# marvinquiet/SpaDOT

Hardware: AMD Instinct MI355X
Metric: training steps/sec + Sinkhorn iters/sec, 50k spots x 3k genes x 5 timepoints (higher is better)
Workload: dtype bf16; 1 GPU; cfg3: 5 time points x 10000 spots x 3000 genes, batch 512, k=30, 1200 inducing points; parallelism=1 GPU, n_sub=9980, E_sub=308893, m_inducing=236, params=16136032, hip_graphs=True, staged_graphs=True, bucketed_grad_exchange=False, units_in_schedule=80

## Files before the change

### include/spadot_model.h

```cpp
#ifndef SPADOT_MODEL_H
#define SPADOT_MODEL_H

#ifdef __cplusplus
extern "C" {
#endif

enum { SPADOT_DT_F32 = 0, SPADOT_DT_BF16 = 1, SPADOT_DT_F64 = 2 };
enum { SPADOT_KERNEL_GAUSSIAN = 0, SPADOT_KERNEL_CAUCHY = 1, SPADOT_KERNEL_QUADRATIC = 2 };

const char *spadot_model_version(void);

int spadot_gat_forward(const void *h, int dtype, const float *s_src, const float *s_dst,
                       const int *rowptr, const int *col, const float *bias, int n, int H, int C,
                       int concat, int act, void *out, float *alpha_out, void *stream);

int spadot_gat_backward_target(const void *g_out, const void *out, const void *h, int dtype,
                               const float *s_src, const float *s_dst, const float *alpha,
                               const int *rowptr, const int *col, int n, int H, int C, int concat,
                               int act, void *g_pre, float *dz, float *ds_dst, void *stream);

int spadot_gat_backward_source(const void *g_pre, int dtype, const float *alpha, const float *dz,
                               const int *rowptr_t, const int *col_t, const int *eid_t, int n, int H,
                               int C, void *dh, float *ds_src, const float *ds_dst, const float *att_src,
                               const float *att_dst, void *stream);
// ... 27 lines not shown
                         void *g_mu, void *g_var, void *g_mv, void *g_tr, void *g_pm, void *g_pv,
                         void *stream);

int spadot_bn_act_forward(const void *x, int x_dtype, const float *lin_bias, const float *gamma, const float *beta,
                          float *running_mean, float *running_var, long long *num_batches_tracked, int b, int F,
                          double momentum, double eps, double slope, float *y, float *save_mean, float *save_invstd,
                          void *stream);
int spadot_bn_act_backward(const float *dy, const float *y, const void *x, int x_dtype, const float *lin_bias,
                           const float *gamma, const float *save_mean, const float *save_invstd, int b, int F,
                           double slope, void *dx, float *dgamma, float *dbeta, void *stream);
int spadot_ln_act_forward(const float *x, const float *gamma, const float *beta, int b, int F, double eps, double slope,
                          float *y, float *save_mean, float *save_invstd, void *stream);
int spadot_ln_act_backward(const float *dy, const float *y, const float *x, const float *gamma, const float *save_mean,
                           const float *save_invstd, int b, int F, double slope, float *dx, float *dgamma, float *dbeta,
                           void *stream);

int spadot_svgp_post_forward(const double *raw, const double *rd, const double *r, const double *Mr, const double *ld,
                             const double *sm, const double *mu, const double *var, const double *ktilde, int b, int L,
                             int m, double c, double kl_const, double b_over_N, double *p_m, double *mv, double *p_v,
                             double *tr, double *out4, float *skl32 , void *stream);
int spadot_svgp_post_backward(const float *g_skl, const double *out4, const double *G_pm, const double *G_pv,
                              const double *mu, const double *var, const double *mv, const double *tr, const double *p_m,
                              const double *p_v, const double *ktilde, const double *Mr, const double *M, int b, int L,
                              int m, double c, double b_over_N, double *g_mu, double *g_var, double *G1, double *G2T,
                              double *g_kl, double *gMr, double *gM, void *stream);
int spadot_svgp_q1t(const double *Ta, const double *Tb, const double *G2T, const double *m0, const double *g_kl, int L, int nh,
                    int b, double *q1, void *stream);
int spadot_svgp_post_pm_pv(const double *raw, const double *rd_a, const double *ktilde, int b, int L, double c, double *p_m,
                           double *p_v, void *stream);
int spadot_svgp_grad_tail(const double *q1, const double *q2, const double *Kdt, const double *p_v, const double *ktilde,
                          const double *p_m, const double *mu, const double *w, const double *g_kl, const double *g_mu,
                          const double *g_var, int b, int L, double c, double *dmu, double *dvar, float *dz,
                          void *stream);
int spadot_svgp_pre(const float *z, int b, int L, double *mu, double *var, double *w, double *muw, void *stream);
int spadot_svgp_pre2(const float *z, const double *Kn, int b, int L, int m, double *mu, double *var, double *w, double *muw,
                     double *A, void *stream);
int spadot_svgp_mid(const double *S, const double *t, const double *M, const double *X2, int L, int m, int rows2,
                    double *r, double *Mr, double *raw, double *sm, double *smpart, int smpart_doubles, void *stream);

int spadot_latent_head_forward(const float *zg, const double *p_m, const double *p_v, float *eps, int b, int Ls,
                               int Lg, float *latent, float *scal2, double *partials, unsigned *counter,
                               unsigned long long *rng_state, void *stream);
int spadot_latent_head_backward(const float *zg, const double *p_v, const float *eps, const float *latent,
                                const float *g_latent, const float *g_kl, const float *g_align, int b, int Ls, int Lg,
                                float *d_zg, double *d_pm, double *d_pv, void *stream);
int spadot_cluster_losses_forward(const float *z, const long long *labels_all, const long long *seed_ids,
                                  const float *centres, const float *prev_centres, const float *gamma,
                                  const long long *cluster_list, int b, int D, int K, int Kp, int Kl, int do_km,
                                  int do_ot, float *out2, float *work, void *stream);
int spadot_cluster_losses_backward(const float *z, const float *centres, const float *prev_centres, const float *gamma,
                                   const long long *cluster_list, const float *work, const float *g_km,
                                   const float *g_ot, int b, int D, int K, int Kp, int Kl, int do_km, int do_ot,
                                   float *dz, void *stream);
int spadot_cluster_losses_fb(const float *z, const long long *labels_all, const long long *seed_ids, const float *centres,
                             const float *prev_centres, const float *gamma, const long long *cluster_list, int b, int D, int K,
                             int Kp, int Kl, int do_km, int do_ot, const float *g_km, const float *g_ot, float *out2,
                             float *work, float *dz, void *stream);
int spadot_mix_losses_forward(const float *const *terms6, const float *w6, float *out7, void *stream);
int spadot_mix_losses_backward(const float *g_elbo, const float *w6, float *g6, void *stream);

int spadot_sqerr_forward(const void *y, const void *yhat, long long count, double inv_scale, int dtype,
                         double *scratch, void *out1, void *stream);
int spadot_sqerr_backward(const void *g1, const void *y, const void *yhat, long long count,
                          double inv_scale, int dtype, void *g_yhat, void *stream);

int spadot_kmeans_assign(const void *x, const void *centers, int n, int k, int d, int dtype, int *labels,
                         void *stream);

int spadot_sgemm_small(int mode, const float *A, int lda, const float *B, int ldb, float *C, int ldc, int M, int N, int K,
                       const float *bias, int batch, long long strideA, long long strideB, long long strideC, void *stream);

int spadot_enc_fused_supported(int b, int F1, int F2, int Q);
long long spadot_enc_fused_workspace(int b, int F1, int F2, int Q);
int spadot_enc_bn_map(const float *h1, const float *lin_bias, const float *gamma, const float *beta, float *running_mean,
                      float *running_var, long long *num_batches_tracked, int b, int F1, double momentum, double eps, double slope,
                      float *y1, float *save_mean, float *save_invstd, const float *W2, int F2, float *part, void *stream);
int spadot_enc_bn_fc(const float *part, int nparts, const float *lin_bias, const float *gamma, const float *beta, float *running_mean,
                     float *running_var, long long *num_batches_tracked, int b, int F2, double momentum, double eps, double slope,
                     float *h2, float *y2, float *save_mean, float *save_invstd, const float *Wfc, int Q, float *pz, void *stream);
int spadot_enc_sum_z(const float *pz, int nparts, const float *bias, int b, int Q, float *z, void *stream);
int spadot_svgp_pre2_partials(const float *pz, int nparts, const float *bias, const double *Kn, int b, int L, int m, float *z,
                              double *mu, double *var, double *w, double *muw, double *A, void *stream);

int spadot_recon_fb_supported(int b, int K, int G);
long long spadot_recon_fb_workspace(int b, int K, int G);
int spadot_recon_fb(const void *h_bf16, const void *W_bf16, const void *WT_bf16, int ldt, const float *bias, const float *y, int b, int K,
                    int G, double inv_scale, const float *grad_weight, void *g_bf16, float *workspace, double *loss_parts, float *dh,
                    void *stream);
int spadot_sum_parts(const double *part, int n, double scale, float *out, void *stream);

int spadot_stamp(unsigned long long *buf, int slot, void *stream);

int spadot_lloyd_step(const double *X, double *C, const int *xoff, const int *npts, int n_max, int R, const int *rgroup,
                      const int *Kr, int K_max, int D, const double *tol, double *part, int *done, double *inertia, int skip_done,
                      void *stream);
int spadot_kmeanspp_seed(const double *X, const int *xoff, const int *npts, int D, int P, const int *pset, const int *pK,
                         const int *pfirst, const int *puoff, const double *U, int K_max, int n_max, double *closest, int *idx,
                         double *centers, void *stream);

int spadot_knn(const double *x, int n, int d, int kk, int *out, void *stream);

int spadot_gat_mfma_supported(int dtype, int H, int C, int max_cols);

int spadot_gat_tail_supported(int dtype, int H, int K);
int spadot_gat_tail_wvec(const float *W, int ldw, const float *att_src, const float *att_dst, int H, int C, int K, float *part,
                         int slices, float *wv, void *whi, void *wlo, void *stream);
int spadot_gat_tail_logits(const void *x, int dtype, int ldx, const float *wv, const void *whi, const void *wlo, int n, int H, int K,
                           float *s, void *stream);
int spadot_gat_tail_aggregate(const void *x, int dtype, int ldx, const float *s, const int *rowptr, const int *col, int n_tgt, int H,
                              int K, void *A, float *alpha, void *stream);
int spadot_gat_tail_headmean(const void *O, int dtype, const float *bias, int n_tgt, int H, int C, void *out, void *stream);
int spadot_gat_tail_colsum_rows(const void *g, int dtype, int rows, int C, float *out, void *stream);
int spadot_gat_tail_scale_colsum(const void *g, int dtype, int rows, int C, double scale, void *gs, float *out, void *stream);
int spadot_gat_tail_edge_backward(const void *x, int dtype, int ldx, const void *dA, const float *s, const float *alpha, const int *rowptr,
                                  const int *col, int n_tgt, int H, int K, float *dz, float *ds_dst, void *stream);
int spadot_gat_tail_source_backward(const void *dA, int dtype, const float *alpha, const float *dz, const float *ds_dst, const float *wv,
                                    const int *rowptr_t, const int *col_t, const int *eid_t, int n, int n_tgt, int rows_out, int H, int K,
                                    void *dx, int lddx, float *ds_src, const void *act_out, int ldm, double slope, void *stream);
int spadot_gat_tail_dwvec_rows(int n);
int spadot_gat_tail_dwvec(const void *x, int dtype, int ldx, const float *ds_src, const float *ds_dst, int n, int n_tgt, int H, int K,
                          float *part, void *stream);
int spadot_gat_tail_wvec_backward(const float *W, int ldw, const float *att_src, const float *att_dst, const float *dwv, int H, int C, int K,
                                  float *dW, int lddw, int accumulate, float *datt_src, float *datt_dst, void *stream);
int spadot_gat_alpha(const float *s_src, const float *s_dst, const int *rowptr, const int *col, const int *cellq, int n_tgt,
                     int H, float *alpha, void *acell, const int *cellq_s, void *acell_s, void *stream);
int spadot_gat_aggregate(const void *x, int dtype, const void *acell, const int *plan_rows, const int *plan_sptr,
                         const int *plan_cols, int nb, int max_cols, int H, int C, int mode, const float *vec_a,
                         const float *vec_b, int act, const float *ds_src, const float *ds_dst, void *out,
                         const void *h_rows, float *att_part, int part_width, int pad_from, int pad_to, const float *dz,
                         const int *rowptr_t, const int *eid_t, float *ds_src_out, void *stream);
int spadot_gat_edge_dot(const void *g_out, const void *out, const void *h, int dtype, const int *plan_rows,
                        const int *plan_sptr, const int *plan_cols, const int *plan_cell, int nb, int max_cols, int H,
                        int C, int act, void *g_pre, float *dz, float *bias_part, int part_width, int part_col, void *stream);
int spadot_gat_softmax_backward(const float *alpha, const float *s_src, const float *s_dst, const int *rowptr,
                                const int *col, const int *cellq_s, int n_tgt, int n_all, int H, float *dz, float *ds_dst,
                                void *acell_s, void *stream);
int spadot_gat_ds_src(const float *dz, const int *rowptr_t, const int *eid_t, int n, int H, float *ds_src, void *stream);

int spadot_gemm_tn_bf16(const void *A, int lda, const void *B, int ldb, void *C, int ldc, int M, int N, int K, void *stream);
int spadot_gemm_nn_bf16(const void *A, int lda, const void *B, int ldb, void *C, int ldc, int M, int N, int K, void *stream);
int spadot_gemm_nn_bf16_masked(const void *A, int lda, const void *B, int ldb, void *C, int ldc, int M, int N, int K,
                               const void *act_out, int ldm, double slope, void *stream);
long long spadot_gemm_bf16_split_workspace(int M, int N, int tail_row_tiles, int slices);
int spadot_gemm_tn_bf16_split(const void *A, int lda, const void *B, int ldb, void *C, int ldc, int M, int N, int K,
                              int tail_row_tiles, int slices, float *workspace, void *stream);


long long spadot_gemm_wgrad_bf16_workspace(int M, int N, int K, int slices);
int spadot_gemm_wgrad_bf16(const void *G, int ldg, const void *X, int ldx, float *dW, int ldw, int M, int N, int K,
                           int slices, float *workspace, const void *zero_row, void *stream);
long long spadot_gemm_wgrad_bf16_workspace_tiled(int M, int N, int K, int slices, int tile_k);
int spadot_gemm_wgrad_bf16_tiled(const void *G, int ldg, const void *X, int ldx, float *dW, int ldw, int M, int N, int K,
                                 int slices, int tile_k, float *workspace, const void *zero_row, void *stream);

int spadot_mlp_chain_supported(int n_layers, const int *dims);
int spadot_mlp_chain_workspace(int b, int n_layers, const int *dims, int *n_rows, int *width);
int spadot_mlp_chain_forward(const float *x, int b, int n_layers, const int *dims, const float *const *W,
                             const float *const *bias, const float *const *gamma, const float *const *beta, const double *eps,
                             const double *slope, float *const *a, float *const *y, float *const *mean, float *const *invstd,
                             void *stream);
int spadot_mlp_chain_forward_bf16(const float *x, int b, int n_layers, const int *dims, const float *const *W,
                                  const float *const *bias, const float *const *gamma, const float *const *beta,
                                  const double *eps, const double *slope, float *const *a, float *const *y, float *const *mean,
                                  float *const *invstd, void *y_last_bf16, void *stream);
int spadot_mlp_chain_backward(const float *dy, const float *x, int b, int n_layers, const int *dims, const float *const *W,
                              const float *const *gamma, const double *slope, float *const *a, float *const *y,
                              float *const *mean, float *const *invstd, float *dx, float *workspace, float *grads, void *stream);
int spadot_mlp_chain_backward_add(const float *dy, const float *x, int b, int n_layers, const int *dims, const float *const *W,
                                  const float *const *gamma, const double *slope, float *const *a, float *const *y,
                                  float *const *mean, float *const *invstd, float *dx, const float *dx_add, float *workspace,
                                  float *grads, void *stream);

int spadot_bias_sqerr_forward(const float *o, const float *bias, const float *y, int b, int G, double inv_scale, double *scratch,
                              float *out, void *stream);
int spadot_bias_sqerr_backward(const float *g1, const float *o, const float *bias, const float *y, int b, int G,
                               double inv_scale, void *g_bf16, float *dbias, void *stream);

int spadot_headfc_backward(const float *g, const void *h_bf16, const float *W, int b, int K, int N, void *dh_bf16,
                           float *workspace , float *grads ,
                           void *stream);

int spadot_cast_rows_multi(const float *const *src, void *const *dst, const int *rows, const int *K, const int *Kp, int n,
                           void *stream);

int spadot_grad_sumsq(const float *grad, long long count, double *scratch, float *sumsq, void *stream);
int spadot_clip_adamw_dev(float *param, const float *grad, float *exp_avg, float *exp_avg_sq, long long count, double lr,
                          double beta1, double beta2, double eps, double weight_decay, double max_norm, double *scratch,
                          float *sumsq, int *step_dev, unsigned *counter, const float *grad_scale_dev, void *stream);
typedef struct spadot_weight_image {
    long long offset;
    int rows, K, Kp, reserved;
    void *image;
} spadot_weight_image;
typedef struct spadot_weight_images {
    int n, reserved;
    spadot_weight_image w[8];
} spadot_weight_images;
int spadot_clip_adamw_images_dev(float *param, const float *grad, float *exp_avg, float *exp_avg_sq, long long count, double lr,
                                 double beta1, double beta2, double eps, double weight_decay, double max_norm, double *scratch,
                                 float *sumsq, int *step_dev, const float *grad_scale_dev, const spadot_weight_images *images,
                                 void *stream);
int spadot_grad_norm_step_dev(const float *grad, long long count, double *scratch, float *sumsq, int *step_dev, void *stream);
int spadot_adamw_range_dev(float *param, const float *grad, float *exp_avg, float *exp_avg_sq, long long offset, long long count,
                           double lr, double beta1, double beta2, double eps, double weight_decay, double max_norm,
                           const float *sumsq, const int *step_dev, const float *grad_scale_dev, const spadot_weight_images *images,
                           void *stream);

int spadot_adamw_step(float *param, const float *grad, float *exp_avg, float *exp_avg_sq,
                      const float *sumsq, long long count, double lr, double beta1, double beta2,
                      double eps, double weight_decay, double max_norm, int step, void *stream);

int spadot_adamw_step_dev(float *param, const float *grad, float *exp_avg, float *exp_avg_sq,
                          const float *sumsq, long long count, double lr, double beta1, double beta2,
                          double eps, double weight_decay, double max_norm, int *step_dev, void *stream);

int spadot_pre_gene_detect(const long long *colptr, const int *ridx, const float *val, const int *tp_off, int T, int G,
                           double thr, int *cnt, double *colsum, void *stream);
int spadot_pre_row_total(const long long *indptr, const int *cidx, const float *val, const int *tp_off, int T, int G,
                         const unsigned char *mask, int nrows, double *total, void *stream);
int spadot_sparkx_moments(const long long *colptr, const int *ridx, const float *val, const int *tp_off, int P,
                          const int *pair_t, const int *pair_g, const int *rowmap, const double *xt, double *mom, void *stream);
int spadot_sparkx_pvals(const double *mom, int P, const int *pair_t, const int *nkeep, const double *inv, const double *lam,
                        int nodes, double *stat, double *pval, double *comb, void *stream);
int spadot_pre_lognorm_stats(const long long *colptr, const int *ridx, const float *val, const int *tp_off, int T, int S,
                             const int *cols, const double *total, double target, double *mean, double *stdv, void *stream);
int spadot_pre_scale_write(const long long *indptr, const int *cidx, const float *val, const int *tp_off, int T, int S,
                           const int *colpos, const double *total, double target, const double *mean, const double *stdv,
                           double clip, int nrows, float *out, void *stream);

int spadot_sct_gene_stats(const long long *colptr, const int *ridx, const float *val, const int *tp_off, int t, int Gk,
                          const int *genes, int N, double *out, void *stream);
int spadot_sct_fit(const long long *colptr, const int *ridx, const float *val, const int *tp_off, int t, int G1,
                   const int *genes, const double *lur, const double *lu, int N, double tol, int maxit, int limit, double eps,
                   double *out, void *stream);
int spadot_sct_resid_stats(const long long *colptr, const int *ridx, const float *val, const int *tp_off, int t, int Gk,
                           const int *genes, const double *lur, const double *lu, int N, const double *pars, double clip_hi,
                           double clip_lo, double *out, void *stream);
int spadot_sct_resid_write(const long long *colptr, const int *ridx, const float *val, const int *tp_off, int t, int S,
                           const int *genes, const double *lur, const double *lu, const int *krow, const int *rowmap, int N,
                           const double *pars, const double *center, double clip_lo, double *out, void *stream);
int spadot_sct_polygamma(const double *x, int n, double *psi, double *psi1, void *stream);

int spadot_mk_lds_capacity(void);
long long spadot_mk_ranksum_scratch_bytes(int T, int G, int nmax);
int spadot_mk_lognorm(const int *ridx, const float *val, const double *total, long long nnz, double target, float *v,
                      void *stream);
int spadot_mk_ranksum(const long long *colptr, const int *ridx, const float *v, const int *tp_off, const int *labels,
                      const int *nk, int T, int G, int K, int nmax, void *scratch, long long scratch_bytes, long long *r2,
                      long long *ties, int *nnz_k, double *vsum, void *stream);
int spadot_mk_finish(const long long *r2, const long long *ties, const int *tp_off, const int *nk, int T, int G, int K,
                     double *u1, double *score, double *pval, void *stream);

int spadot_silhouette(const double *x, int d, int P, const long long *prob, const int *order, const int *coff, int n_max,
                      int k_min, int k_max, double *a, double *b, int *nearest, double *s, void *stream);

int spadot_gmm_em_step(const double *x, int d, int P, const long long *prob, int K_max, int n_max, double *par, double *w,
                       double *cov, double *mom, const double *resp_init, double reg_covar, double tol, int steps, double *part,
                       int *done, int *n_iter, double *lb, void *stream);
int spadot_gmm_estep(const double *x, int d, int P, const long long *prob, int K_max, int n_max, const double *par, double *norm,
                     int *labels, double *resp, double *lp, void *stream);

int spadot_nhood_counts(const int *src, const int *dst, const unsigned char *labels, const long long *desc_host,
                        const long long *desc_dev, int G, int K_max, long long lds_limit, int *out, void *stream);

int spadot_cooccur_counts(const double *xy, const long long *desc_host, const long long *desc_dev, const double *r2_host,
                          const double *r2_dev, int P, int K_max, int B_max, long long *out, void *stream);

int spadot_cooccur_null(const double *xy, const long long *desc_host, const long long *desc_dev, const double *r2_host,
                        const double *r2_dev, int P, int K_max, int B_max, int observed, long long first, int n_perms,
                        long long seed, long long *out, void *stream);

int spadot_ripley_counts(const double *xy, const long long *desc_host, const long long *desc_dev, const double *r2_host,
                         const double *r2_dev, const double *hull_host, const double *hull_dev, const double *cum_host,
                         const double *cum_dev, long long hull_rows, int P, int K_max, int S_max, int B_max, long long seed,
                         long long *out, void *stream);

int spadot_ripley_points(const double *hull_host, const double *hull_dev, const double *cum_host, const double *cum_dev, int V,
                         long long seed, long long g, long long stream_id, long long count, double *out, void *stream);

int spadot_autocorr_sums(const int *src, const int *dst, const long long *colptr, const int *ridx, const float *v, long long nnz,
                         long long ridx_lo, long long ridx_hi, const double *centre, const long long *desc_host,
                         const long long *desc_dev, int T, int G, int g0, int ng, int observed, long long first, long long P,
                         long long seed, long long lds_limit, float *scratch, long long scratch_floats, int threads, int gs,
                         double *N, double *D, void *stream);

int spadot_ligrec_sums(const long long *colptr, const int *ridx, const float *v, long long nnz, long long ridx_lo,
                       long long ridx_hi, const unsigned char *labels, int label_hi, const long long *desc_host,
                       const long long *desc_dev, int T, int G, int K, const int *genes, int ng, int gene_lo, int gene_hi,
                       int observed, long long first, long long P, long long seed, long long lds_limit, int threads, int gc,
                       double *S, int *cnt, void *stream);

int spadot_ligrec_count(const double *S0, const double *S, const double *wk, const int *pairs, int pair_lo, int pair_hi,
                        const unsigned char *mask, int T, int M, int ns, int K, long long L, int skip, int *ge, void *stream);

int spadot_local_lag(const int *rowptr, const int *col, const long long *colptr, const int *ridx, const float *v, long long nnz,
                     long long ridx_lo, long long ridx_hi, const double *centre, const long long *desc_host,
                     const long long *desc_dev, int T, int G, const int *genes, int ng, int gene_lo, int gene_hi, long long first,
                     long long P, long long seed, long long lds_limit, void *scratch, long long scratch_bytes, int threads, int gs,
                     long long perm_chunk, long long rows, double *lag, int *ge, int *le, void *stream);

int spadot_cross_dense(const int *rowptr, const int *col, const long long *colptr, const int *ridx, const float *v, long long nnz,
                       long long ridx_lo, long long ridx_hi, const double *centre, const long long *desc_host,
                       const long long *desc_dev, int T, int G, const int *genes, int ng, int gene_lo, int gene_hi, int GP,
                       long long zrows, double *Z, double *Y, void *stream);
int spadot_cross_sums(const double *Z, const double *Y, long long zrows, int GP, const long long *desc_host,
                      const long long *desc_dev, int T, int ng, int observed, long long first, long long P, long long seed,
                      double *M, void *stream);

int spadot_corr_sums(const double *xy, const int *order, const double *Z, long long zrows, int GP, const long long *desc_host,
                     const long long *desc_dev, const double *r2_host, const double *r2_dev, int T, int ng, int B_max, int observed,
                     long long first, long long P, long long seed, int cull, int cs, double *scratch, long long scratch_doubles,
                     long long *W, long long *S2c, double *N, double *Q, long long *skipped, void *stream);

int spadot_latent_knn(const double *x, int d, int P, const long long *prob_host, const long long *prob_dev, int *idx, double *d2,
                      void *stream);
int spadot_tsne_affinities(const double *d2, int P, const long long *prob_host, const long long *prob_dev, const double *perp_host,
                           const double *perp_dev, double *cond, double *beta, void *stream);
int spadot_tsne_steps(const long long *prob_host, const long long *prob_dev, int P, const long long *rowptr, const int *col,
                      const double *val, double *Y0, double *Y1, double *upd, double *gains, const double *lr, double *part,
                      double *zr, double *att, double *blk, double *grad, double *Z, double *kl, long long kl_stride, long long it0,
                      int steps, long long early, double exaggeration, int two, void *stream);

int spadot_weighted_moments_chunk(void);
int spadot_weighted_moments(const long long *colptr, const int *ridx, const float *v, const int *tp_off, int T, int G,
                            const double *W, long long n, int C, double *S0, double *S1, double *S2, void *stream);

#ifdef __cplusplus
}
#endif
#endif
```

### spadot_amd/_lib.py

```python
import ctypes
import os

_CSRC = os.path.join(os.path.dirname(os.path.abspath(__file__)), "csrc")
_CACHE = {}


class NativeLibraryMissing(RuntimeError):
    pass


def _load(name):
    if name in _CACHE:
        return _CACHE[name]
    import torch

    path = os.path.join(_CSRC, name)
    if not os.path.exists(path):
        raise NativeLibraryMissing(
            f"{path} is missing: build the HIP extension with `python -m spadot_amd.csrc.build` "
            "(needs hipcc; cross-compiles for gfx950 without a GPU). There is no CPU fallback.")
    lib = ctypes.CDLL(path)
    _CACHE[name] = lib
    return lib


class _Checked:
    __slots__ = ("fn", "n", "name")

    def __init__(self, fn, name):
        self.fn, self.n, self.name = fn, len(fn.argtypes), name

    @property
    def argtypes(self):
        return self.fn.argtypes

    @property
    def restype(self):
        return self.fn.restype

    def __call__(self, *args):
        if len(args) != self.n:
            raise TypeError(f"{self.name} takes {self.n} arguments (include/*.h), {len(args)} given")
        return self.fn(*args)


def _seal(lib):
    for name, fn in list(vars(lib).items()):
        if name.startswith("spadot_") and not isinstance(fn, _Checked):
            if fn.argtypes is None and name not in ("spadot_ot_version", "spadot_model_version"):
                raise RuntimeError(f"{name}: no argtypes declared in spadot_amd/_lib.py")
            if fn.argtypes is not None:
                setattr(lib, name, _Checked(fn, name))


class OTConfig(ctypes.Structure):
    _fields_ = [("lambda1", ctypes.c_double), ("lambda2", ctypes.c_double), ("epsilon", ctypes.c_double),
                ("epsilon0", ctypes.c_double), ("tolerance", ctypes.c_double), ("tau", ctypes.c_double),
                ("batch_size", ctypes.c_int), ("max_iter", ctypes.c_int)]


class OTInfo(ctypes.Structure):
    _fields_ = [("gap", ctypes.c_double), ("stage_iters", ctypes.c_int * 6), ("absorbs", ctypes.c_int),
                ("gap_checks", ctypes.c_int)]


class OTSmallProblem(ctypes.Structure):
    _fields_ = [("x_dev", ctypes.c_void_p), ("y_dev", ctypes.c_void_p), ("C_dev", ctypes.c_void_p),
                ("G_dev", ctypes.c_void_p), ("plan_dev", ctypes.c_void_p), ("gamma_rownorm_dev", ctypes.c_void_p),
                ("I", ctypes.c_int), ("J", ctypes.c_int)]


class OTSmallInfo(ctypes.Structure):
    _fields_ = [("gap", ctypes.c_double), ("stage_iters", ctypes.c_int * 6), ("absorbs", ctypes.c_int),
                ("gap_checks", ctypes.c_int), ("status", ctypes.c_int), ("reserved", ctypes.c_int)]


class WeightImage(ctypes.Structure):
    _fields_ = [("offset", ctypes.c_longlong), ("rows", ctypes.c_int), ("K", ctypes.c_int), ("Kp", ctypes.c_int),
                ("reserved", ctypes.c_int), ("image", ctypes.c_void_p)]


class WeightImages(ctypes.Structure):
    _fields_ = [("n", ctypes.c_int), ("reserved", ctypes.c_int), ("w", WeightImage * 8)]


def ot_lib():
    lib = _load("libspadot_ot.so")
    if getattr(lib, "_spadot_ready", False):
        return lib
    vp, ci, cd = ctypes.c_void_p, ctypes.c_int, ctypes.c_double
    lib.spadot_ot_version.restype = ctypes.c_char_p
    lib.spadot_ot_create.argtypes = [ctypes.POINTER(vp), ci, ci, ci, vp]
    lib.spadot_ot_create.restype = ci
    lib.spadot_ot_destroy.argtypes = [vp]
    lib.spadot_ot_destroy.restype = None
    lib.spadot_ot_ld.argtypes = [vp]
    lib.spadot_ot_ld.restype = ci
    lib.spadot_ot_fused_geometry.argtypes = [vp, ctypes.POINTER(ci)]
    lib.spadot_ot_fused_geometry.restype = None
    lib.spadot_ot_matrix_dev.argtypes = [vp, ci]
    lib.spadot_ot_matrix_dev.restype = vp
    lib.spadot_ot_vector_dev.argtypes = [vp, ci]
    lib.spadot_ot_vector_dev.restype = vp
    lib.spadot_ot_vector_host.argtypes = [vp, ci, vp]
    lib.spadot_ot_vector_host.restype = ci
    lib.spadot_ot_matrix_host.argtypes = [vp, ci, vp]
    lib.spadot_ot_matrix_host.restype = ci
    lib.spadot_ot_set_cost_dev.argtypes = [vp, vp, ci, ci]
    lib.spadot_ot_set_cost_dev.restype = ci
    lib.spadot_ot_set_cost_host.argtypes = [vp, vp]
    lib.spadot_ot_set_cost_host.restype = ci
    lib.spadot_ot_set_cost_from_latents_dev.argtypes = [vp, vp, vp, ci, ci]
    lib.spadot_ot_set_cost_from_latents_dev.restype = ci
    lib.spadot_ot_solve.argtypes = [vp, vp, ctypes.POINTER(OTConfig), ctypes.POINTER(OTInfo)]
    lib.spadot_ot_solve.restype = ci
    lib.spadot_ot_plan_dev.argtypes = [vp, vp, ci, ci]
    lib.spadot_ot_plan_dev.restype = ci
    lib.spadot_ot_plan_group_sums_dev.argtypes = [vp, vp, ci, vp]
    lib.spadot_ot_plan_group_sums_dev.restype = ci
    lib.spadot_ot_plan_apply_dev.argtypes = [vp, ci, vp, ci, vp]
    lib.spadot_ot_plan_apply_dev.restype = ci
    lib.spadot_ot_plan_host.argtypes = [vp, vp]
    lib.spadot_ot_plan_host.restype = ci
    lib.spadot_ot_plan_rowsums_host.argtypes = [vp, vp]
    lib.spadot_ot_plan_rowsums_host.restype = ci
    lib.spadot_ot_run_iterations.argtypes = [vp, ctypes.POINTER(OTConfig), cd, ci, ctypes.POINTER(ctypes.c_float)]
    lib.spadot_ot_run_iterations.restype = ci
    lib.spadot_ot_run_tau_flag.argtypes = [vp, ci]
    lib.spadot_ot_run_tau_flag.restype = ci
    lib.spadot_ot_run_checked.argtypes = [vp, ctypes.POINTER(OTConfig), cd, ci, ci, ctypes.POINTER(ci), ctypes.POINTER(ctypes.c_float)]
    lib.spadot_ot_run_checked.restype = ci
    lib.spadot_ot_time_kernels.argtypes = [vp, ctypes.POINTER(OTConfig), cd, ci, ctypes.POINTER(ctypes.c_float)]
    lib.spadot_ot_time_kernels.restype = ci
    lib.spadot_ot_small_max.argtypes = []
    lib.spadot_ot_small_max.restype = ci
    lib.spadot_ot_small_solve.argtypes = [ci, ctypes.POINTER(OTSmallProblem), ci, ci, ctypes.POINTER(OTConfig), vp, vp]
    lib.spadot_ot_small_solve.restype = ci
    _seal(lib)
    lib._spadot_ready = True
    return lib


def model_lib():
    lib = _load("libspadot_model.so")
    if getattr(lib, "_spadot_ready", False):
        return lib
    vp, ci, cd, ll = ctypes.c_void_p, ctypes.c_int, ctypes.c_double, ctypes.c_longlong
    lib.spadot_model_version.restype = ctypes.c_char_p
    sig = {
        "spadot_gat_forward": [vp, ci, vp, vp, vp, vp, vp, ci, ci, ci, ci, ci, vp, vp, vp],
        "spadot_gat_backward_target": [vp, vp, vp, ci, vp, vp, vp, vp, vp, ci, ci, ci, ci, ci, vp, vp, vp, vp],
        "spadot_gat_backward_source": [vp, ci, vp, vp, vp, vp, vp, ci, ci, ci, vp, vp, vp, vp, vp, vp],
        "spadot_gat_logits": [vp, ci, vp, vp, ci, ci, ci, vp, vp, vp],
        "spadot_gat_att_grad": [vp, ci, vp, vp, ci, ci, ci, vp, ci, vp, vp, vp, ci, vp],
        "spadot_gat_alpha": [vp, vp, vp, vp, vp, ci, ci, vp, vp, vp, vp, vp],
        "spadot_gat_softmax_backward": [vp, vp, vp, vp, vp, vp, ci, ci, ci, vp, vp, vp, vp],
        "spadot_gat_ds_src": [vp, vp, vp, ci, ci, vp, vp],
        "spadot_gat_mfma_supported": [ci, ci, ci, ci],
        "spadot_gat_tail_supported": [ci, ci, ci],
        "spadot_gat_tail_wvec": [vp, ci, vp, vp, ci, ci, ci, vp, ci, vp, vp, vp, vp],
        "spadot_gat_tail_logits": [vp, ci, ci, vp, vp, vp, ci, ci, ci, vp, vp],
        "spadot_gat_tail_aggregate": [vp, ci, ci, vp, vp, vp, ci, ci, ci, vp, vp, vp],
        "spadot_gat_tail_headmean": [vp, ci, vp, ci, ci, ci, vp, vp],
        "spadot_gat_tail_colsum_rows": [vp, ci, ci, ci, vp, vp],
        "spadot_gat_tail_scale_colsum": [vp, ci, ci, ci, cd, vp, vp, vp],
        "spadot_gat_tail_edge_backward": [vp, ci, ci, vp, vp, vp, vp, vp, ci, ci, ci, vp, vp, vp],
        "spadot_gat_tail_source_backward": [vp, ci, vp, vp, vp, vp, vp, vp, vp, ci, ci, ci, ci, ci, vp, ci, vp, vp, ci, cd, vp],
        "spadot_gat_tail_dwvec_rows": [ci],
        "spadot_gat_tail_dwvec": [vp, ci, ci, vp, vp, ci, ci, ci, ci, vp, vp],
        "spadot_gat_tail_wvec_backward": [vp, ci, vp, vp, vp, ci, ci, ci, vp, ci, ci, vp, vp, vp],
        "spadot_gat_aggregate": [vp, ci, vp, vp, vp, vp, ci, ci, ci, ci, ci, vp, vp, ci, vp, vp, vp, vp, vp, ci, ci, ci, vp, vp, vp, vp, vp],
        "spadot_gat_edge_dot": [vp, vp, vp, ci, vp, vp, vp, vp, ci, ci, ci, ci, ci, vp, vp, vp, ci, ci, vp],
        "spadot_gemm_tn_bf16": [vp, ci, vp, ci, vp, ci, ci, ci, ci, vp],
        "spadot_gemm_nn_bf16": [vp, ci, vp, ci, vp, ci, ci, ci, ci, vp],
        "spadot_enc_fused_supported": [ci, ci, ci, ci],
        "spadot_recon_fb_supported": [ci, ci, ci],
        "spadot_recon_fb": [vp, vp, vp, ci, vp, vp, ci, ci, ci, cd, vp, vp, vp, vp, vp, vp],
        "spadot_sum_parts": [vp, ci, cd, vp, vp],
        "spadot_enc_bn_map": [vp, vp, vp, vp, vp, vp, vp, ci, ci, cd, cd, cd, vp, vp, vp, vp, ci, vp, vp],
        "spadot_enc_bn_fc": [vp, ci, vp, vp, vp, vp, vp, vp, ci, ci, cd, cd, cd, vp, vp, vp, vp, vp, ci, vp, vp],
        "spadot_enc_sum_z": [vp, ci, vp, ci, ci, vp, vp],
        "spadot_svgp_pre2_partials": [vp, ci, vp, vp, ci, ci, ci, vp, vp, vp, vp, vp, vp, vp],
        "spadot_gemm_nn_bf16_masked": [vp, ci, vp, ci, vp, ci, ci, ci, ci, vp, ci, cd, vp],
        "spadot_gemm_tn_bf16_split": [vp, ci, vp, ci, vp, ci, ci, ci, ci, ci, ci, vp, vp],
        "spadot_gemm_wgrad_bf16": [vp, ci, vp, ci, vp, ci, ci, ci, ci, ci, vp, vp, vp],
        "spadot_gemm_wgrad_bf16_tiled": [vp, ci, vp, ci, vp, ci, ci, ci, ci, ci, ci, vp, vp, vp],
        "spadot_mlp_chain_supported": [ci, vp],
        "spadot_headfc_backward": [vp, vp, vp, ci, ci, ci, vp, vp, vp, vp],
        "spadot_bias_sqerr_forward": [vp, vp, vp, ci, ci, cd, vp, vp, vp],
        "spadot_bias_sqerr_backward": [vp, vp, vp, vp, ci, ci, cd, vp, vp, vp],
        "spadot_mlp_chain_workspace": [ci, ci, vp, vp, vp],
        "spadot_mlp_chain_forward": [vp, ci, ci, vp, vp, vp, vp, vp, vp, vp, vp, vp, vp, vp, vp],
        "spadot_mlp_chain_forward_bf16": [vp, ci, ci, vp, vp, vp, vp, vp, vp, vp, vp, vp, vp, vp, vp, vp],
        "spadot_mlp_chain_backward": [vp, vp, ci, ci, vp, vp, vp, vp, vp, vp, vp, vp, vp, vp, vp, vp],
        "spadot_mlp_chain_backward_add": [vp, vp, ci, ci, vp, vp, vp, vp, vp, vp, vp, vp, vp, vp, vp, vp, vp],
        "spadot_kernel_matrix": [vp, vp, ci, ci, ci, cd, ci, ci, vp, vp],
        "spadot_spd_inverse_logdet": [vp, ci, ci, vp, vp, vp],
        "spadot_rowdot_forward": [vp, vp, ci, ci, ci, ci, vp, vp],
        "spadot_rowdot_backward": [vp, vp, ci, ci, ci, ci, vp, vp],
        "spadot_elbo_forward": [vp, vp, vp, vp, vp, vp, vp, ci, ci, ci, vp, vp],
        "spadot_elbo_backward": [vp, vp, vp, vp, vp, vp, vp, vp, ci, ci, ci, vp, vp, vp, vp, vp, vp, vp],
        "spadot_bn_act_forward": [vp, ci, vp, vp, vp, vp, vp, vp, ci, ci, cd, cd, cd, vp, vp, vp, vp],
        "spadot_bn_act_backward": [vp, vp, vp, ci, vp, vp, vp, vp, ci, ci, cd, vp, vp, vp, vp],
        "spadot_ln_act_forward": [vp, vp, vp, ci, ci, cd, cd, vp, vp, vp, vp],
        "spadot_ln_act_backward": [vp, vp, vp, vp, vp, vp, ci, ci, cd, vp, vp, vp, vp],
        "spadot_svgp_post_forward": [vp] * 9 + [ci, ci, ci, cd, cd, cd] + [vp] * 7,
        "spadot_svgp_post_backward": [vp] * 13 + [ci, ci, ci, cd, cd] + [vp] * 8,
        "spadot_svgp_grad_tail": [vp] * 11 + [ci, ci, cd] + [vp] * 4,
        "spadot_svgp_q1t": [vp, vp, vp, vp, vp, ci, ci, ci, vp, vp],
        "spadot_svgp_post_pm_pv": [vp, vp, vp, ci, ci, cd, vp, vp, vp],
        "spadot_svgp_pre": [vp, ci, ci, vp, vp, vp, vp, vp],
        "spadot_svgp_pre2": [vp, vp, ci, ci, ci, vp, vp, vp, vp, vp, vp],
        "spadot_svgp_mid": [vp, vp, vp, vp, ci, ci, ci, vp, vp, vp, vp, vp, ci, vp],
        "spadot_spd_inverse_logdet2": [vp, ci, ci, ci, vp, vp, vp, vp, vp],
        "spadot_latent_head_forward": [vp, vp, vp, vp, ci, ci, ci, vp, vp, vp, vp, vp, vp],
        "spadot_latent_head_backward": [vp, vp, vp, vp, vp, vp, vp, ci, ci, ci, vp, vp, vp, vp],
        "spadot_cluster_losses_forward": [vp, vp, vp, vp, vp, vp, vp, ci, ci, ci, ci, ci, ci, ci, vp, vp, vp],
        "spadot_cluster_losses_backward": [vp, vp, vp, vp, vp, vp, vp, vp, ci, ci, ci, ci, ci, ci, ci, vp, vp],
        "spadot_cluster_losses_fb": [vp, vp, vp, vp, vp, vp, vp, ci, ci, ci, ci, ci, ci, ci, vp, vp, vp, vp, vp, vp],
        "spadot_mix_losses_forward": [vp, vp, vp, vp],
        "spadot_mix_losses_backward": [vp, vp, vp, vp],
        "spadot_sqerr_forward": [vp, vp, ll, cd, ci, vp, vp, vp],
        "spadot_sqerr_backward": [vp, vp, vp, ll, cd, ci, vp, vp],
        "spadot_kmeans_assign": [vp, vp, ci, ci, ci, ci, vp, vp],
        "spadot_sgemm_small": [ci, vp, ci, vp, ci, vp, ci, ci, ci, ci, vp, ci, ll, ll, ll, vp],
        "spadot_lloyd_step": [vp, vp, vp, vp, ci, ci, vp, vp, ci, ci, vp, vp, vp, vp, ci, vp],
        "spadot_kmeanspp_seed": [vp, vp, vp, ci, ci, vp, vp, vp, vp, vp, ci, ci, vp, vp, vp, vp],
        "spadot_colsum": [vp, ci, ci, vp, vp],
        "spadot_cast_rows_multi": [vp, vp, vp, vp, vp, ci, vp],
        "spadot_knn": [vp, ci, ci, ci, vp, vp],
        "spadot_stamp": [vp, ci, vp],
        "spadot_grad_sumsq": [vp, ll, vp, vp, vp],
        "spadot_clip_adamw_dev": [vp, vp, vp, vp, ll, cd, cd, cd, cd, cd, cd, vp, vp, vp, vp, vp, vp],
        "spadot_clip_adamw_images_dev": [vp, vp, vp, vp, ll, cd, cd, cd, cd, cd, cd, vp, vp, vp, vp, ctypes.POINTER(WeightImages), vp],
        "spadot_grad_norm_step_dev": [vp, ll, vp, vp, vp, vp],
        "spadot_adamw_range_dev": [vp, vp, vp, vp, ll, ll, cd, cd, cd, cd, cd, cd, vp, vp, vp, ctypes.POINTER(WeightImages), vp],
        "spadot_adamw_step": [vp, vp, vp, vp, vp, ll, cd, cd, cd, cd, cd, cd, ci, vp],
        "spadot_adamw_step_dev": [vp, vp, vp, vp, vp, ll, cd, cd, cd, cd, cd, cd, vp, vp],
        "spadot_pre_gene_detect": [vp, vp, vp, vp, ci, ci, cd, vp, vp, vp],
        "spadot_pre_row_total": [vp, vp, vp, vp, ci, ci, vp, ci, vp, vp],
        "spadot_sparkx_moments": [vp, vp, vp, vp, ci, vp, vp, vp, vp, vp, vp],
        "spadot_sparkx_pvals": [vp, ci, vp, vp, vp, vp, ci, vp, vp, vp, vp],
        "spadot_pre_lognorm_stats": [vp, vp, vp, vp, ci, ci, vp, vp, cd, vp, vp, vp],
        "spadot_pre_scale_write": [vp, vp, vp, vp, ci, ci, vp, vp, cd, vp, vp, cd, ci, vp, vp],
        "spadot_sct_gene_stats": [vp, vp, vp, vp, ci, ci, vp, ci, vp, vp],
        "spadot_sct_fit": [vp, vp, vp, vp, ci, ci, vp, vp, vp, ci, cd, ci, ci, cd, vp, vp],
        "spadot_sct_resid_stats": [vp, vp, vp, vp, ci, ci, vp, vp, vp, ci, vp, cd, cd, vp, vp],
        "spadot_sct_resid_write": [vp, vp, vp, vp, ci, ci, vp, vp, vp, vp, vp, ci, vp, vp, cd, vp, vp],
        "spadot_sct_polygamma": [vp, ci, vp, vp, vp],
        "spadot_mk_lognorm": [vp, vp, vp, ll, cd, vp, vp],
        "spadot_mk_ranksum": [vp, vp, vp, vp, vp, vp, ci, ci, ci, ci, vp, ll, vp, vp, vp, vp, vp],
        "spadot_mk_finish": [vp, vp, vp, vp, ci, ci, ci, vp, vp, vp, vp],
        "spadot_silhouette": [vp, ci, ci, vp, vp, vp, ci, ci, ci, vp, vp, vp, vp, vp],
        "spadot_weighted_moments": [vp, vp, vp, vp, ci, ci, vp, ll, ci, vp, vp, vp, vp],
        "spadot_gmm_em_step": [vp, ci, ci, vp, ci, ci, vp, vp, vp, vp, vp, cd, cd, ci, vp, vp, vp, vp, vp],
        "spadot_gmm_estep": [vp, ci, ci, vp, ci, ci, vp, vp, vp, vp, vp, vp],
        "spadot_nhood_counts": [vp, vp, vp, vp, vp, ci, ci, ll, vp, vp],
        "spadot_cooccur_counts": [vp, vp, vp, vp, vp, ci, ci, ci, vp, vp],
        "spadot_cooccur_null": [vp, vp, vp, vp, vp, ci, ci, ci, ci, ll, ci, ll, vp, vp],
        "spadot_ripley_counts": [vp, vp, vp, vp, vp, vp, vp, vp, vp, ll, ci, ci, ci, ci, ll, vp, vp],
        "spadot_ripley_points": [vp, vp, vp, vp, ci, ll, ll, ll, ll, vp, vp],
        "spadot_autocorr_sums": [vp, vp, vp, vp, vp, ll, ll, ll, vp, vp, vp, ci, ci, ci, ci, ci, ll, ll, ll, ll, vp, ll, ci, ci,
                                 vp, vp, vp],
        "spadot_ligrec_sums": [vp, vp, vp, ll, ll, ll, vp, ci, vp, vp, ci, ci, ci, vp, ci, ci, ci, ci, ll, ll, ll, ll, ci, ci, vp, vp,
                               vp],
        "spadot_ligrec_count": [vp, vp, vp, vp, ci, ci, vp, ci, ci, ci, ci, ll, ci, vp, vp],
        "spadot_local_lag": [vp, vp, vp, vp, vp, ll, ll, ll, vp, vp, vp, ci, ci, vp, ci, ci, ci, ll, ll, ll, ll, vp, ll, ci, ci, ll,
                             ll, vp, vp, vp, vp],
        "spadot_cross_dense": [vp, vp, vp, vp, vp, ll, ll, ll, vp, vp, vp, ci, ci, vp, ci, ci, ci, ci, ll, vp, vp, vp],
        "spadot_cross_sums": [vp, vp, ll, ci, vp, vp, ci, ci, ci, ll, ll, ll, vp, vp],
        "spadot_corr_sums": [vp, vp, vp, ll, ci, vp, vp, vp, vp, ci, ci, ci, ci, ll, ll, ll, ci, ci, vp, ll, vp, vp, vp, vp, vp, vp],
        "spadot_latent_knn": [vp, ci, ci, vp, vp, vp, vp, vp],
        "spadot_tsne_affinities": [vp, ci, vp, vp, vp, vp, vp, vp, vp],
        "spadot_tsne_steps": [vp, vp, ci, vp, vp, vp, vp, vp, vp, vp, vp, vp, vp, vp, vp, vp, vp, vp, ll, ll, ci, ll, cd, ci, vp],
    }
    for name, args in sig.items():
        fn = getattr(lib, name)
        fn.argtypes = args
        fn.restype = ci
    lib.spadot_recon_fb_workspace.argtypes = [ci, ci, ci]
    lib.spadot_recon_fb_workspace.restype = ll
    lib.spadot_enc_fused_workspace.argtypes = [ci, ci, ci, ci]
    lib.spadot_enc_fused_workspace.restype = ll
    lib.spadot_gemm_bf16_split_workspace.argtypes = [ci, ci, ci, ci]
    lib.spadot_gemm_bf16_split_workspace.restype = ll
    lib.spadot_gemm_wgrad_bf16_workspace.argtypes = [ci, ci, ci, ci]
    lib.spadot_gemm_wgrad_bf16_workspace.restype = ll
    lib.spadot_gemm_wgrad_bf16_workspace_tiled.argtypes = [ci, ci, ci, ci, ci]
    lib.spadot_gemm_wgrad_bf16_workspace_tiled.restype = ll
    lib.spadot_mk_lds_capacity.argtypes = []
    lib.spadot_mk_lds_capacity.restype = ci
    lib.spadot_mk_ranksum_scratch_bytes.argtypes = [ci, ci, ci]
    lib.spadot_mk_ranksum_scratch_bytes.restype = ll
    lib.spadot_weighted_moments_chunk.argtypes = []
    lib.spadot_weighted_moments_chunk.restype = ci
    _seal(lib)
    lib._spadot_ready = True
    return lib
```

### spadot_amd/csrc/gemm_wgrad_bf16.hip

```cpp
#include <hip/hip_runtime.h>
#include <cstdint>

#include "../../include/spadot_model.h"
#include "per_device.h"

namespace {

typedef __bf16 bf8 __attribute__((ext_vector_type(8)));
typedef short s4v __attribute__((ext_vector_type(4)));
typedef float f16v __attribute__((ext_vector_type(16)));

constexpr int TN = 256, TK = 256, CH = 64, NT = 512;
constexpr int ROWB = 512;
constexpr int OPB = CH * ROWB;
constexpr int STAGEB = 2 * OPB;
constexpr int LDS_BYTES = 2 * STAGEB;
constexpr int PIECES = 8;

template <int WGN, int WGK, int TI, int TJ>
__global__ __launch_bounds__(NT, 1) void k_gemm_wgrad_bf16(const __bf16 *__restrict__ G, int ldg, const __bf16 *__restrict__ X,
                                                          int ldx, float *__restrict__ dW, int ldw, int M, int N, int K,
                                                          int ktiles, int S, int chunks_per_slice,
                                                          const __bf16 *__restrict__ zrow, float *__restrict__ part) {
    extern __shared__ __attribute__((aligned(16))) unsigned char smem[];
// ... 23 lines not shown
        poff[u] = u < 4 ? ((size_t)row * ldg + n0) * 2 + chunk * 16 : ((size_t)row * ldx + k0) * 2 + chunk * 16;
        if (u >= 4 && chunk * 8 >= TKE) pzero = true;
    }
    auto request = [&](int ks) __attribute__((always_inline)) {
#ifdef WGRAD_PROBE_NO_DMA
        return;
#endif
        const int m0 = (c_begin + ks) * CH;
        const unsigned base = lds0 + (unsigned)(ks & 1) * STAGEB + (unsigned)wave * 1024u;
#pragma unroll
        for (int u = 0; u < PIECES; u++) {
            const char *src = (u < 4 ? reinterpret_cast<const char *>(G) + (size_t)m0 * ldg * 2
                                     : reinterpret_cast<const char *>(X) + (size_t)m0 * ldx * 2) + poff[u];
            if (m0 + prow[u] >= M || (u >= 4 && pzero)) src = reinterpret_cast<const char *>(zrow) + (lane & 31) * 16;
            const unsigned dst = __builtin_amdgcn_readfirstlane(base + (unsigned)(u & 3) * 8192u + (u < 4 ? 0u : (unsigned)OPB));
            unsigned keep;
            asm volatile("s_mov_b32 %0, m0\n\ts_mov_b32 m0, %2\n\ts_nop 0\n\tglobal_load_lds_dwordx4 %1, off\n\ts_mov_b32 m0, %0"
                         : "=&s"(keep) : "v"(src), "s"(dst) : "memory");
        }
    };

    f16v acc[TI][TJ];
#pragma unroll
    for (int i = 0; i < TI; i++)
#pragma unroll
        for (int j = 0; j < TJ; j++)
#pragma unroll
            for (int e = 0; e < 16; e++) acc[i][j][e] = 0.f;

    const int hh = lane >> 5, g16 = (lane >> 4) & 1, qq = (lane & 15) >> 2, pp = lane & 3;
    unsigned ga[TI], xb[TJ];
#pragma unroll
    for (int i = 0; i < TI; i++) {
        const int g = wn * TI + i;
        ga[i] = lds0 + (unsigned)((8 * hh + qq) * ROWB + (g & ~3) * 64 + ((g ^ qq) & 3) * 64 + 32 * g16 + 8 * pp);
    }
#pragma unroll
    for (int j = 0; j < TJ; j++) {
        const int g = wk * TJ + j;
        xb[j] = lds0 + (unsigned)OPB + (unsigned)((8 * hh + qq) * ROWB + (g & ~3) * 64 + ((g ^ qq) & 3) * 64 + 32 * g16 + 8 * pp);
    }
    auto read_frags = [&](unsigned stage_off, int ss, s4v (&a)[TI][2], s4v (&b)[TJ][2]) __attribute__((always_inline)) {
        const unsigned so = stage_off + (unsigned)ss * (16 * ROWB);
#ifdef WGRAD_PROBE_NO_READS
#pragma unroll
        for (int j = 0; j < TJ; j++) b[j][0] = b[j][1] = s4v{(short)so, 1, 2, 3};
#pragma unroll
        for (int i = 0; i < TI; i++) a[i][0] = a[i][1] = s4v{(short)so, 1, 2, 3};
        return;
#endif
#pragma unroll
        for (int j = 0; j < TJ; j++) {
            asm volatile("ds_read_b64_tr_b16 %0, %1" : "=v"(b[j][0]) : "v"(xb[j] + so));
            asm volatile("ds_read_b64_tr_b16 %0, %1 offset:2048" : "=v"(b[j][1]) : "v"(xb[j] + so));
        }
#pragma unroll
        for (int i = 0; i < TI; i++) {
            asm volatile("ds_read_b64_tr_b16 %0, %1" : "=v"(a[i][0]) : "v"(ga[i] + so));
            asm volatile("ds_read_b64_tr_b16 %0, %1 offset:2048" : "=v"(a[i][1]) : "v"(ga[i] + so));
        }
    };
    auto mma = [&](const s4v (&a)[TI][2], const s4v (&b)[TJ][2]) __attribute__((always_inline)) {
        __builtin_amdgcn_s_setprio(1);
        bf8 bf[TJ];
#pragma unroll
        for (int j = 0; j < TJ; j++) bf[j] = __builtin_bit_cast(bf8, __builtin_shufflevector(b[j][0], b[j][1], 0, 1, 2, 3, 4, 5, 6, 7));
#pragma unroll
        for (int i = 0; i < TI; i++) {
            const bf8 af = __builtin_bit_cast(bf8, __builtin_shufflevector(a[i][0], a[i][1], 0, 1, 2, 3, 4, 5, 6, 7));
#pragma unroll
            for (int j = 0; j < TJ; j++) {
#ifdef WGRAD_PROBE_NO_MFMA
                asm volatile("" ::"v"(af), "v"(bf[j]));
#else
                acc[i][j] = __builtin_amdgcn_mfma_f32_32x32x16_bf16(af, bf[j], acc[i][j], 0, 0, 0);
#endif
            }
        }
        __builtin_amdgcn_s_setprio(0);
    };
    auto frags_ready = [&]() __attribute__((always_inline)) {
#ifdef WGRAD_PROBE_NO_READS
        return;
#endif
        asm volatile("s_waitcnt lgkmcnt(%0)" ::"n"(RD) : "memory");
        __builtin_amdgcn_sched_barrier(0);
    };

    if (nk > 0) {
        request(0);
        if (1 < nk) {
            request(1);
            asm volatile("s_waitcnt vmcnt(%0)" ::"n"(PIECES) : "memory");
        } else {
            asm volatile("s_waitcnt vmcnt(0)" ::: "memory");
        }
        __builtin_amdgcn_s_barrier();
        s4v a0[TI][2], b0[TJ][2], a1[TI][2], b1[TJ][2];
        read_frags(0u, 0, a0, b0);
        for (int P = 0; P < nk; P++) {
            const unsigned so = (unsigned)(P & 1) * STAGEB;
            read_frags(so, 1, a1, b1);
            frags_ready();
            mma(a0, b0);
            read_frags(so, 2, a0, b0);
            frags_ready();
            mma(a1, b1);
            read_frags(so, 3, a1, b1);
            frags_ready();
            mma(a0, b0);
            if (P + 1 < nk) {
                asm volatile("s_waitcnt vmcnt(0)" ::: "memory");
                asm volatile("s_waitcnt lgkmcnt(0)" ::: "memory");
                __builtin_amdgcn_sched_barrier(0);
                __builtin_amdgcn_s_barrier();
                if (P + 2 < nk) request(P + 2);
                read_frags((unsigned)((P + 1) & 1) * STAGEB, 0, a0, b0);
                asm volatile("s_waitcnt lgkmcnt(%0)" ::"n"(RD) : "memory");
            } else {
                asm volatile("s_waitcnt lgkmcnt(0)" ::: "memory");
            }
            __builtin_amdgcn_sched_barrier(0);
            mma(a1, b1);
        }
    }

    const int lk = (wk * TJ) * 32 + (lane & 31);
    if (S == 1) {
#pragma unroll
        for (int i = 0; i < TI; i++)
#pragma unroll
            for (int j = 0; j < TJ; j++)
#pragma unroll
                for (int e = 0; e < 16; e++) {
                    const int n = n0 + (wn * TI + i) * 32 + (e & 3) + 8 * (e >> 2) + 4 * hh, k = k0 + lk + 32 * j;
                    if (n < N && k < K) dW[(size_t)n * ldw + k] = acc[i][j][e];
                }
        return;
    }
    float *mine = part + ((size_t)slice * gridDim.x / S + tile) * (size_t)(TN * TKE);
#pragma unroll
    for (int i = 0; i < TI; i++)
#pragma unroll
        for (int j = 0; j < TJ; j++)
#pragma unroll
            for (int e = 0; e < 16; e++) {
                const int ln = (wn * TI + i) * 32 + (e & 3) + 8 * (e >> 2) + 4 * hh;
                mine[(size_t)ln * TKE + lk + 32 * j] = acc[i][j][e];
            }
}

template <int TKE>
__global__ __launch_bounds__(256) void k_wgrad_reduce(const float *__restrict__ part, int S, int tiles, int ktiles,
                                                      float *__restrict__ dW, int ldw, int N, int K) {
    constexpr int RP = TKE / 4;
    constexpr int BPT = RP / 4;
    constexpr int Q = 64 * RP;
    typedef float f32x4 __attribute__((ext_vector_type(4)));
    const int tile = blockIdx.x / BPT;
    const int p0 = (blockIdx.x - tile * BPT) * 256 + threadIdx.x;
    const int tn = tile / ktiles, tk = tile - tn * ktiles;
    f32x4 v[8][4];
#pragma unroll
    for (int s_ = 0; s_ < 8; s_++)
        if (s_ < S) {
            const f32x4 *src = reinterpret_cast<const f32x4 *>(part + ((size_t)s_ * tiles + tile) * (size_t)(TN * TKE));
#pragma unroll
            for (int j = 0; j < 4; j++) v[s_][j] = src[p0 + j * Q];
        }
#pragma unroll
    for (int j = 0; j < 4; j++) {
        f32x4 sum = v[0][j];
#pragma unroll
        for (int s_ = 1; s_ < 8; s_++)
            if (s_ < S) sum += v[s_][j];
        const int idx4 = p0 + j * Q, ln = idx4 / RP, c4 = idx4 - ln * RP;
        const int n = tn * TN + ln, k = tk * TKE + 4 * c4;
        if (n < N && k + 3 < K) *reinterpret_cast<f32x4 *>(dW + (size_t)n * ldw + k) = sum;
        else if (n < N) {
            for (int e = 0; e < 4; e++)
                if (k + e < K) dW[(size_t)n * ldw + k + e] = sum[e];
        }
    }
}

static int effective_slices(int M, int slices, int *cps_out) {
    const int nchunk = (M + CH - 1) / CH;
    int S = slices > 0 ? slices : 1;
    if (S > nchunk) S = nchunk;
    if (S > 8) S = 8;
    const int cps = (nchunk + S - 1) / S;
    S = (nchunk + cps - 1) / cps;
    if (cps_out) *cps_out = cps;
    return S;
}

}

extern "C" long long spadot_gemm_wgrad_bf16_workspace_tiled(int M, int N, int K, int slices, int tile_k) {
    if (M <= 0 || N <= 0 || K <= 0 || N % TN != 0 || (tile_k != 256 && tile_k != 192)) return -22;
    const int S = effective_slices(M, slices, nullptr);
    const long long tiles = (long long)(N / TN) * ((K + tile_k - 1) / tile_k);
    return S > 1 ? (long long)S * tiles * TN * tile_k : 0;
}

extern "C" long long spadot_gemm_wgrad_bf16_workspace(int M, int N, int K, int slices) {
    return spadot_gemm_wgrad_bf16_workspace_tiled(M, N, K, slices, 256);
}

template <int WGN, int WGK, int TI, int TJ>
static int launch_wgrad(const void *G, int ldg, const void *X, int ldx, float *dW, int ldw, int M, int N, int K, int ktiles, int ntiles,
                        int S, int cps, float *workspace, const void *zero_row, hipStream_t stream) {
    constexpr int TKE = 32 * WGK * TJ;
    static PerDeviceFlag attr_set;     
    auto kern = k_gemm_wgrad_bf16<WGN, WGK, TI, TJ>;
    if (!attr_set) {
        if (hipFuncSetAttribute((const void *)kern, hipFuncAttributeMaxDynamicSharedMemorySize, LDS_BYTES) != hipSuccess) return -5;
        attr_set = true;
    }
    const int tiles = ntiles * ktiles;
    hipLaunchKernelGGL(kern, dim3((unsigned)(tiles * S)), dim3(NT), LDS_BYTES, stream, (const __bf16 *)G, ldg, (const __bf16 *)X, ldx, dW,
                       ldw, M, N, K, ktiles, S, cps, (const __bf16 *)zero_row, workspace);
    if (S > 1)
        hipLaunchKernelGGL(k_wgrad_reduce<TKE>, dim3((unsigned)tiles * (unsigned)(TKE / 16)), dim3(256), 0, stream, (const float *)workspace, S,
                           tiles, ktiles, dW, ldw, N, K);
    return hipGetLastError() == hipSuccess ? 0 : -5;
}

extern "C" int spadot_gemm_wgrad_bf16_tiled(const void *G, int ldg, const void *X, int ldx, float *dW, int ldw, int M, int N, int K,
                                            int slices, int tile_k, float *workspace, const void *zero_row, void *stream) {
    if (M <= 0 || N <= 0 || K <= 0 || N % TN != 0 || ldg < N || ldx < K || ldw < K || ldg % 8 || ldx % 8) return -22;
    if (tile_k != 256 && tile_k != 192) return -22;
    if (((uintptr_t)G & 15) || ((uintptr_t)X & 15) || ((uintptr_t)dW & 15) || (ldw % 4)) return -22;
    if (!zero_row || ((uintptr_t)zero_row & 15)) return -22;
    const int ktiles = (K + tile_k - 1) / tile_k, ntiles = N / TN;
    if (ldx < ktiles * tile_k) return -22;
    if ((size_t)M * ldg * 2 >= ((size_t)1 << 32) || (size_t)M * ldx * 2 >= ((size_t)1 << 32)) return -22;
    int cps = 0;
    const int S = effective_slices(M, slices, &cps);
    if (ntiles * ktiles > 4096) return -22;
    if (S > 1 && (!workspace || ((uintptr_t)workspace & 15))) return -22;
    if (tile_k == 256)
        return launch_wgrad<2, 4, 4, 2>(G, ldg, X, ldx, dW, ldw, M, N, K, ktiles, ntiles, S, cps, workspace, zero_row, (hipStream_t)stream);
    return launch_wgrad<4, 2, 2, 3>(G, ldg, X, ldx, dW, ldw, M, N, K, ktiles, ntiles, S, cps, workspace, zero_row, (hipStream_t)stream);
}

extern "C" int spadot_gemm_wgrad_bf16(const void *G, int ldg, const void *X, int ldx, float *dW, int ldw, int M, int N, int K,
                                      int slices, float *workspace, const void *zero_row, void *stream) {
    return spadot_gemm_wgrad_bf16_tiled(G, ldg, X, ldx, dW, ldw, M, N, K, slices, 256, workspace, zero_row, stream);
}
```

### spadot_amd/csrc/model_kernels.hip

```cpp
#include <hip/hip_runtime.h>
#include <cmath>
#include <climits>
#include <cstdint>
#include <cstdio>
#include <cstdlib>

#include "../../include/spadot_model.h"
#include "per_device.h"

namespace {

constexpr int WAVE = 64;
constexpr float ATT_SLOPE = 0.2f;
constexpr float ACT_SLOPE = 0.01f;

template <typename T> __device__ __forceinline__ float ld(const T *p);
template <> __device__ __forceinline__ float ld<float>(const float *p) { return *p; }
template <> __device__ __forceinline__ float ld<__bf16>(const __bf16 *p) { return (float)*p; }
template <typename T> __device__ __forceinline__ void st(T *p, float v);
template <> __device__ __forceinline__ void st<float>(float *p, float v) { *p = v; }
template <> __device__ __forceinline__ void st<__bf16>(__bf16 *p, float v) { *p = (__bf16)v; }

__device__ __forceinline__ unsigned bf16_pack2(float lo, float hi) {
    const unsigned short a = __builtin_bit_cast(unsigned short, (__bf16)lo), b = __builtin_bit_cast(unsigned short, (__bf16)hi);
// ... 1174 lines not shown
    for (int c = 1; c < K; c++) {
        if (t < KPP_MAXTR) s_cand[t] = INT_MAX;
        double ssum = 0.0;
        for (int i = lo; i < hi; i++) ssum += cl[i];
        s_scan[t] = ssum;
        __syncthreads();
        for (int off = 1; off < KPP_T; off <<= 1) {
            const double v = t >= off ? s_scan[t - off] : 0.0;
            __syncthreads();
            s_scan[t] += v;
            __syncthreads();
        }
        double run = t > 0 ? s_scan[t - 1] : 0.0;
        double rv[KPP_MAXTR];
        int found[KPP_MAXTR];
#pragma unroll
        for (int j = 0; j < KPP_MAXTR; j++) {
            rv[j] = j < trials ? Up[(size_t)(c - 1) * trials + j] * pot : 0.0;
            found[j] = INT_MAX;
        }
        for (int i = lo; i < hi; i++) {
            run += cl[i];
#pragma unroll
            for (int j = 0; j < KPP_MAXTR; j++)
                if (j < trials && found[j] == INT_MAX && run >= rv[j]) found[j] = i;
        }
#pragma unroll
        for (int j = 0; j < KPP_MAXTR; j++)
            if (j < trials && found[j] != INT_MAX) atomicMin(&s_cand[j], found[j]);
        __syncthreads();
        for (int e = t; e < trials * D; e += KPP_T) {
            const int j = e / D;
            s_c[e] = Xg[(size_t)min(s_cand[j], n - 1) * D + (e - j * D)];
        }
        __syncthreads();
        if (t < trials) {
            double q = 0.0;
            for (int e = 0; e < D; e++) q += s_c[t * D + e] * s_c[t * D + e];
            s_csq[t] = q;
        }
        __syncthreads();
        double lp[KPP_MAXTR];
#pragma unroll
        for (int j = 0; j < KPP_MAXTR; j++) lp[j] = 0.0;
        for (int i = t; i < n; i += KPP_T) {
            const double ci = cl[i];
            const double *xr = Xg + (size_t)i * D;
#pragma unroll
            for (int j = 0; j < KPP_MAXTR; j++)
                if (j < trials) lp[j] += fmin(kpp_d2(xr, s_c + j * D, s_csq[j], D), ci);
        }
        int best = 0;
        double bpot = 0.0;
#pragma unroll
        for (int j = 0; j < KPP_MAXTR; j++) {
            if (j < trials) {
                const double pj = block_sum_d(lp[j], s_red);
                if (j == 0 || pj < bpot) { bpot = pj; best = j; }
            }
        }
        pot = bpot;
        const double *cb = s_c + best * D;
        const double csqb = s_csq[best];
        for (int i = t; i < n; i += KPP_T) cl[i] = fmin(cl[i], kpp_d2(Xg + (size_t)i * D, cb, csqb, D));
        for (int e = t; e < D; e += KPP_T) cp[(size_t)c * D + e] = cb[e];
        if (t == 0) ip[c] = min(s_cand[best], n - 1);
        __syncthreads();
    }
}

__global__ __launch_bounds__(256) void k_sumsq_part(const float *__restrict__ g, long long count,
                                                    double *__restrict__ part) {
    __shared__ double sh[16];
    double acc = 0.0;
    const long long n4 = count / 4;
    const float4 *g4 = reinterpret_cast<const float4 *>(g);
    for (long long k = (long long)blockIdx.x * 256 + threadIdx.x; k < n4; k += (long long)gridDim.x * 256) {
        const float4 v = g4[k];
        acc += (double)v.x * v.x + (double)v.y * v.y + (double)v.z * v.z + (double)v.w * v.w;
    }
    if (blockIdx.x == 0)
        for (long long k = n4 * 4 + threadIdx.x; k < count; k += 256) acc += (double)g[k] * g[k];
    acc = block_sum_d(acc, sh);
    if (threadIdx.x == 0) part[blockIdx.x] = acc;
}

template <int U>
__global__ __launch_bounds__(256) void k_sumsq_last(const float *__restrict__ g, long long count, double *__restrict__ part,
                                                    float *__restrict__ sumsq, int *__restrict__ step_dev,
                                                    unsigned *__restrict__ counter) {
    __shared__ double sh[16];
    __shared__ bool last;
    double acc = 0.0;
    const long long n4 = count / 4;
    const float4 *g4 = reinterpret_cast<const float4 *>(g);
    const long long stride = (long long)gridDim.x * 256;
    for (long long k = (long long)blockIdx.x * 256 + threadIdx.x; k < n4; k += U * stride) {
        float4 v[U];
#pragma unroll
        for (int u = 0; u < U; u++)
            v[u] = (k + u * stride < n4) ? g4[k + u * stride] : make_float4(0.f, 0.f, 0.f, 0.f);
#pragma unroll
        for (int u = 0; u < U; u++)
            acc += ((double)v[u].x * v[u].x + (double)v[u].y * v[u].y) + ((double)v[u].z * v[u].z + (double)v[u].w * v[u].w);
    }
    if (blockIdx.x == 0)
        for (long long k = n4 * 4 + threadIdx.x; k < count; k += 256) acc += (double)g[k] * g[k];
    acc = block_sum_d(acc, sh);
    if (threadIdx.x == 0) {
        part[blockIdx.x] = acc;
        __threadfence();
        last = atomicAdd(counter, 1u) == gridDim.x - 1;
    }
    __syncthreads();
    if (!last) return;
    __threadfence();
    double t = 0.0;
    {
        double q[8];
#pragma unroll
        for (int u = 0; u < 8; u++) {
            const int b = threadIdx.x + u * 256;
            q[u] = b < (int)gridDim.x ? __builtin_nontemporal_load(part + b) : 0.0;
        }
        t = ((q[0] + q[1]) + (q[2] + q[3])) + ((q[4] + q[5]) + (q[6] + q[7]));
    }
    t = block_sum_d(t, sh);
    if (threadIdx.x == 0) { sumsq[0] = (float)t; if (step_dev) step_dev[0] += 1; *counter = 0u; }
}

__global__ void k_step_inc(int *step) { step[0] += 1; }

template <int U>
__global__ __launch_bounds__(256) void k_sumsq_part_u(const float *__restrict__ g, long long count, double *__restrict__ part) {
    __shared__ double sh[16];
    double acc = 0.0;
    const long long n4 = count / 4;
    const float4 *g4 = reinterpret_cast<const float4 *>(g);
    const long long stride = (long long)gridDim.x * 256;
    for (long long k = (long long)blockIdx.x * 256 + threadIdx.x; k < n4; k += U * stride) {
        float4 v[U];
#pragma unroll
        for (int u = 0; u < U; u++)
            v[u] = (k + u * stride < n4) ? g4[k + u * stride] : make_float4(0.f, 0.f, 0.f, 0.f);
#pragma unroll
        for (int u = 0; u < U; u++)
            acc += ((double)v[u].x * v[u].x + (double)v[u].y * v[u].y) + ((double)v[u].z * v[u].z + (double)v[u].w * v[u].w);
    }
    if (blockIdx.x == 0)
        for (long long k = n4 * 4 + threadIdx.x; k < count; k += 256) acc += (double)g[k] * g[k];
    acc = block_sum_d(acc, sh);
    if (threadIdx.x == 0) part[blockIdx.x] = acc;
}
__global__ __launch_bounds__(1024) void k_final_sum_step(const double *__restrict__ part, int nparts, float *__restrict__ out,
                                                         int *__restrict__ step_dev) {
    __shared__ double sh[16];
    double acc = 0.0;
    for (int k = threadIdx.x; k < nparts; k += 1024) acc += part[k];
    acc = block_sum_d(acc, sh);
    if (threadIdx.x == 0) { out[0] = (float)acc; if (step_dev) step_dev[0] += 1; }
}

__device__ __forceinline__ void adamw_element(float g_, float &pp, float &mm, float &vv, float coef, float lr, float wd,
                                              float b1, float b2, float eps, float bc1, float bc2_sqrt) {
#pragma clang fp contract(off)
    const float gg = g_ * coef;
    float pn = pp * (1.f - lr * wd);
    const float mn = mm + (gg - mm) * (1.f - b1);
    const float vn = vv * b2 + gg * gg * (1.f - b2);
    const float denom = sqrtf(vn) / bc2_sqrt + eps;
    pn -= (lr / bc1) * (mn / denom);
    pp = pn; mm = mn; vv = vn;
}

__device__ __forceinline__ float adamw_clip_coef(float sumsq, float gs, float max_norm) {
#pragma clang fp contract(off)
    const float total = sqrtf(sumsq) * gs;
    return fminf(1.f, max_norm / (total + 1e-6f)) * gs;
}

__global__ __launch_bounds__(256) void k_adamw(float *__restrict__ p, const float *__restrict__ g,
                                               float *__restrict__ m, float *__restrict__ v,
                                               const float *__restrict__ sumsq, long long count, float lr,
                                               float b1, float b2, float eps, float wd, float max_norm,
                                               float bc1, float bc2_sqrt, const int *__restrict__ step_dev,
                                               const float *__restrict__ grad_scale) {
    if (step_dev) {
        const double t = (double)step_dev[0];
        bc1 = (float)(1.0 - pow((double)b1, t));
        bc2_sqrt = (float)sqrt(1.0 - pow((double)b2, t));
    }
    const float gs = grad_scale ? grad_scale[0] : 1.f;
    const float coef = adamw_clip_coef(sumsq[0], gs, max_norm);
    for (long long k = (long long)blockIdx.x * 256 + threadIdx.x; k < count; k += (long long)gridDim.x * 256) {
        float pp = p[k], mm = m[k], vv = v[k];
        adamw_element(g[k], pp, mm, vv, coef, lr, wd, b1, b2, eps, bc1, bc2_sqrt);
        p[k] = pp; m[k] = mm; v[k] = vv;
    }
}

__global__ __launch_bounds__(256) void k_adamw_img(float *__restrict__ p, const float *__restrict__ g,
                                                   float *__restrict__ m, float *__restrict__ v,
                                                   const float *__restrict__ sumsq, long long count, float lr,
                                                   float b1, float b2, float eps, float wd, float max_norm,
                                                   const int *__restrict__ step_dev, const float *__restrict__ grad_scale,
                                                   spadot_weight_images imgs, long long base) {
    const double t = (double)step_dev[0];
    const float bc1 = (float)(1.0 - pow((double)b1, t));
    const float bc2_sqrt = (float)sqrt(1.0 - pow((double)b2, t));
    const float gs = grad_scale ? grad_scale[0] : 1.f;
    const float coef = adamw_clip_coef(sumsq[0], gs, max_norm);
    const long long n4 = count >> 2;
    for (long long q = (long long)blockIdx.x * 256 + threadIdx.x; q < n4; q += (long long)gridDim.x * 256) {
        const long long k = q << 2;
        const float4 g4 = *reinterpret_cast<const float4 *>(g + k);
        const float4 p4 = *reinterpret_cast<const float4 *>(p + k);
        const float4 m4 = *reinterpret_cast<const float4 *>(m + k);
        const float4 v4 = *reinterpret_cast<const float4 *>(v + k);
        const float gi[4] = {g4.x, g4.y, g4.z, g4.w}, pi[4] = {p4.x, p4.y, p4.z, p4.w};
        const float mi[4] = {m4.x, m4.y, m4.z, m4.w}, vi[4] = {v4.x, v4.y, v4.z, v4.w};
        float po[4], mo[4], vo[4];
#pragma unroll
        for (int e = 0; e < 4; e++) {
            po[e] = pi[e]; mo[e] = mi[e]; vo[e] = vi[e];
            adamw_element(gi[e], po[e], mo[e], vo[e], coef, lr, wd, b1, b2, eps, bc1, bc2_sqrt);
        }
        *reinterpret_cast<float4 *>(p + k) = make_float4(po[0], po[1], po[2], po[3]);
        *reinterpret_cast<float4 *>(m + k) = make_float4(mo[0], mo[1], mo[2], mo[3]);
        *reinterpret_cast<float4 *>(v + k) = make_float4(vo[0], vo[1], vo[2], vo[3]);
#pragma unroll
        for (int s_ = 0; s_ < 8; s_++) {
            if (s_ >= imgs.n) break;
            const spadot_weight_image W = imgs.w[s_];
            const unsigned long long d = (unsigned long long)(k + base - W.offset);
            if (d < (unsigned long long)W.rows * (unsigned long long)W.K) {
                const unsigned row = (unsigned)d / (unsigned)W.K;
                const unsigned col = (unsigned)d - row * (unsigned)W.K;
                __bf16 *dst = reinterpret_cast<__bf16 *>(W.image) + (size_t)row * W.Kp + col;
                const unsigned lo = (unsigned)__builtin_bit_cast(unsigned short, (__bf16)po[0]) |
                                    ((unsigned)__builtin_bit_cast(unsigned short, (__bf16)po[1]) << 16);
                const unsigned hi = (unsigned)__builtin_bit_cast(unsigned short, (__bf16)po[2]) |
                                    ((unsigned)__builtin_bit_cast(unsigned short, (__bf16)po[3]) << 16);
                *reinterpret_cast<uint2 *>(dst) = make_uint2(lo, hi);
                break;
            }
        }
    }
}

#ifndef BN_RG_DEF
#define BN_RG_DEF 16
#endif
constexpr int BN_RPT = 512 / BN_RG_DEF;
#ifndef BN_COLS_DEF
#define BN_COLS_DEF 16
#endif
constexpr int BN_COLS = BN_COLS_DEF, BN_RG = BN_RG_DEF, BN_NT = BN_COLS * BN_RG;
constexpr int LN_RG = 64, LN_NT = BN_COLS * LN_RG;

template <int RG = BN_RG>
__device__ __forceinline__ float bn_col_sum(float v, float (*sh)[BN_COLS + 1], int cl, int rg) {
    __syncthreads();
    sh[rg][cl] = v;
    __syncthreads();
    float t = 0.f;
#pragma unroll 8
    for (int g = 0; g < RG; g++) t += sh[g][cl];
    return t;
}

template <typename TX>
__global__ __launch_bounds__(BN_NT) void k_bn_act_fwd(const TX *__restrict__ x, const float *__restrict__ lb,
                                                    const float *__restrict__ gamma, const float *__restrict__ beta,
                                                    float *__restrict__ run_mean, float *__restrict__ run_var,
                                                    long long *__restrict__ nbt, int b, int F, float momentum, float eps,
                                                    float slope, float *__restrict__ y, float *__restrict__ save_mean,
                                                    float *__restrict__ save_invstd) {
    __shared__ float sh[BN_RG][BN_COLS + 1];
    const int cl = threadIdx.x & (BN_COLS - 1), rg = threadIdx.x / BN_COLS;
    const int c = blockIdx.x * BN_COLS + cl;
    const bool on = c < F;
    const int c1 = min(c, F - 1);
    const float add_r = (lb ? lb : gamma)[c1];
    const float add = (on && lb) ? add_r : 0.f;
    if (b <= BN_RG * BN_RPT) {
        float v[BN_RPT];
        const int cc = min(c, F - 1);
#pragma unroll
        for (int r = 0; r < BN_RPT; r++) v[r] = ld<TX>(x + (size_t)min(rg + r * BN_RG, b - 1) * F + cc);
        const float gam_r = gamma[cc], bet_r = beta[cc], rm_r = run_mean[cc], rv_r = run_var[cc];
#pragma unroll
        for (int r = 0; r < BN_RPT; r++) v[r] = (on && rg + r * BN_RG < b) ? v[r] + add : 0.f;
        float s = 0.f;
#pragma unroll
        for (int r = 0; r < BN_RPT; r++)
            if (rg + r * BN_RG < b) s += v[r];
        const float mean = bn_col_sum(s, sh, cl, rg) / (float)b;
        float ss = 0.f;
#pragma unroll
        for (int r = 0; r < BN_RPT; r++)
            if (rg + r * BN_RG < b) { const float d = v[r] - mean; ss += d * d; }
        const float var = bn_col_sum(ss, sh, cl, rg) / (float)b;
        const float invstd = rsqrtf(var + eps);
        if (on) {
            const float g = gam_r * invstd, o = bet_r;
#pragma unroll
            for (int r = 0; r < BN_RPT; r++) {
                const int i = rg + r * BN_RG;
                if (i < b) {
                    const float u = (v[r] - mean) * g + o;
                    y[(size_t)i * F + c] = u > 0.f ? u : slope * u;
                }
            }
            if (rg == 0) {
                save_mean[c] = mean; save_invstd[c] = invstd;
                run_mean[c] = (1.f - momentum) * rm_r + momentum * mean;
                run_var[c] = (1.f - momentum) * rv_r + momentum * var * ((float)b / (float)(b > 1 ? b - 1 : 1));
            }
        }
        if (nbt && blockIdx.x == 0 && threadIdx.x == 0) nbt[0] += 1;
        return;
    }
    float s = 0.f;
    if (on)
#pragma unroll 4
        for (int i = rg; i < b; i += BN_RG) s += ld<TX>(x + (size_t)i * F + c) + add;
    const float mean = bn_col_sum(s, sh, cl, rg) / (float)b;
    float ss = 0.f;
    if (on)
#pragma unroll 4
        for (int i = rg; i < b; i += BN_RG) { const float d = ld<TX>(x + (size_t)i * F + c) + add - mean; ss += d * d; }
    const float var = bn_col_sum(ss, sh, cl, rg) / (float)b;
    const float invstd = rsqrtf(var + eps);
    if (on) {
        const float g = gamma[c] * invstd, o = beta[c];
#pragma unroll 4
        for (int i = rg; i < b; i += BN_RG) {
            const float v = (ld<TX>(x + (size_t)i * F + c) + add - mean) * g + o;
            y[(size_t)i * F + c] = v > 0.f ? v : slope * v;
        }
        if (rg == 0) {
            save_mean[c] = mean; save_invstd[c] = invstd;
            run_mean[c] = (1.f - momentum) * run_mean[c] + momentum * mean;
            run_var[c] = (1.f - momentum) * run_var[c] + momentum * var * ((float)b / (float)(b > 1 ? b - 1 : 1));
        }
    }
    if (nbt && blockIdx.x == 0 && threadIdx.x == 0) nbt[0] += 1;
}

template <typename TX>
__global__ __launch_bounds__(BN_NT) void k_bn_act_bwd(const float *__restrict__ dy, const float *__restrict__ y,
                                                    const TX *__restrict__ x, const float *__restrict__ lb,
                                                    const float *__restrict__ gamma, const float *__restrict__ save_mean,
                                                    const float *__restrict__ save_invstd, int b, int F, float slope,
                                                    TX *__restrict__ dx, float *__restrict__ dgamma,
                                                    float *__restrict__ dbeta) {
    __shared__ float sh[BN_RG][BN_COLS + 1];
    const int cl = threadIdx.x & (BN_COLS - 1), rg = threadIdx.x / BN_COLS;
    const int c = blockIdx.x * BN_COLS + cl;
    const bool on = c < F;
    const int c1 = min(c, F - 1);
    const float add_r = (lb ? lb : gamma)[c1], mean_r = save_mean[c1], invstd_r = save_invstd[c1], gamma_r = gamma[c1];
    const float add = (on && lb) ? add_r : 0.f;
    const float mean = on ? mean_r : 0.f, invstd = on ? invstd_r : 0.f;
    if (b <= BN_RG * BN_RPT) {
        float dzv[BN_RPT], xh[BN_RPT];
        const int cc = min(c, F - 1);
#pragma unroll
        for (int r = 0; r < BN_RPT; r++) dzv[r] = dy[(size_t)min(rg + r * BN_RG, b - 1) * F + cc];
#pragma unroll
        for (int r = 0; r < BN_RPT; r++) {
            const float yv = y[(size_t)min(rg + r * BN_RG, b - 1) * F + cc];
            dzv[r] = (on && rg + r * BN_RG < b) ? dzv[r] * (yv > 0.f ? 1.f : slope) : 0.f;
        }
#pragma unroll
        for (int r = 0; r < BN_RPT; r++) {
            const float xv = ld<TX>(x + (size_t)min(rg + r * BN_RG, b - 1) * F + cc);
            xh[r] = (xv + add - mean) * invstd;
        }
        float sb = 0.f, sg = 0.f;
#pragma unroll
        for (int r = 0; r < BN_RPT; r++)
            if (on && rg + r * BN_RG < b) { sb += dzv[r]; sg += dzv[r] * xh[r]; }
        sb = bn_col_sum(sb, sh, cl, rg);
        sg = bn_col_sum(sg, sh, cl, rg);
        if (on) {
            const float g = gamma_r * invstd, mb = sb / (float)b, mg = sg / (float)b;
#pragma unroll
            for (int r = 0; r < BN_RPT; r++) {
                const int i = rg + r * BN_RG;
                if (i < b) st<TX>(dx + (size_t)i * F + c, g * (dzv[r] - mb - xh[r] * mg));
            }
            if (rg == 0) { dgamma[c] = sg; dbeta[c] = sb; }
        }
        return;
    }
// ... 929 lines not shown
    return hipGetLastError() == hipSuccess ? 0 : -5;
}

int spadot_sqerr_forward(const void *y, const void *yhat, long long count, double inv_scale, int dtype,
                         double *scratch, void *out1, void *stream) {
    if (count <= 0 || !scratch) return -22;
    hipStream_t st_ = (hipStream_t)stream;
    const int nb = (int)((count + 255) / 256 < 2048 ? (count + 255) / 256 : 2048);
    FP_DISPATCH(dtype,
                { hipLaunchKernelGGL(k_sqerr_part<float>, dim3(nb), dim3(256), 0, st_, (const float *)y, (const float *)yhat, count, scratch);
                  hipLaunchKernelGGL(k_final_sum<float>, dim3(1), dim3(1024), 0, st_, scratch, nb, inv_scale, (float *)out1); },
                { hipLaunchKernelGGL(k_sqerr_part<double>, dim3(nb), dim3(256), 0, st_, (const double *)y, (const double *)yhat, count, scratch);
                  hipLaunchKernelGGL(k_final_sum<double>, dim3(1), dim3(1024), 0, st_, scratch, nb, inv_scale, (double *)out1); });
    return hipGetLastError() == hipSuccess ? 0 : -5;
}

int spadot_sqerr_backward(const void *g1, const void *y, const void *yhat, long long count, double inv_scale,
                          int dtype, void *g_yhat, void *stream) {
    if (count <= 0) return -22;
    hipStream_t st_ = (hipStream_t)stream;
    const int nb = (int)((count + 255) / 256 < 4096 ? (count + 255) / 256 : 4096);
    FP_DISPATCH(dtype,
                hipLaunchKernelGGL(k_sqerr_bwd<float>, dim3(nb), dim3(256), 0, st_, (const float *)g1, (const float *)y, (const float *)yhat, count, inv_scale, (float *)g_yhat),
                hipLaunchKernelGGL(k_sqerr_bwd<double>, dim3(nb), dim3(256), 0, st_, (const double *)g1, (const double *)y, (const double *)yhat, count, inv_scale, (double *)g_yhat));
    return hipGetLastError() == hipSuccess ? 0 : -5;
}

int spadot_kmeans_assign(const void *x, const void *centers, int n, int k, int d, int dtype, int *labels,
                         void *stream) {
    if (n <= 0 || k <= 0 || d <= 0) return -22;
    hipStream_t st_ = (hipStream_t)stream;
    dim3 g((n + 255) / 256);
    FP_DISPATCH(dtype,
                hipLaunchKernelGGL(k_kmeans_assign<float>, g, dim3(256), 0, st_, (const float *)x, (const float *)centers, n, k, d, labels),
                hipLaunchKernelGGL(k_kmeans_assign<double>, g, dim3(256), 0, st_, (const double *)x, (const double *)centers, n, k, d, labels));
    return hipGetLastError() == hipSuccess ? 0 : -5;
}

int spadot_sgemm_small(int mode, const float *A, int lda, const float *B, int ldb, float *C, int ldc, int M, int N, int K,
                       const float *bias, int batch, long long strideA, long long strideB, long long strideC, void *stream) {
    if (mode < 0 || mode > 2 || !A || !B || !C || M <= 0 || N <= 0 || K <= 0 || ldc < N) return -22;
    if ((mode == 2 ? lda < M : lda < K) || (mode == 1 ? ldb < K : ldb < N)) return -22;
    if (batch < 1 || batch > 65535 || strideA < 0 || strideB < 0 || strideC < 0) return -22;
    const dim3 grid((unsigned)((N + 31) / 32), (unsigned)((M + 31) / 32), (unsigned)batch);
    if (grid.y > 65535u) return -22;
    hipStream_t st_ = (hipStream_t)stream;
    if (mode == 0) hipLaunchKernelGGL(k_sgemm_small<0>, grid, dim3(256), 0, st_, A, lda, B, ldb, C, ldc, M, N, K, bias, strideA, strideB, strideC);
    else if (mode == 1) hipLaunchKernelGGL(k_sgemm_small<1>, grid, dim3(256), 0, st_, A, lda, B, ldb, C, ldc, M, N, K, bias, strideA, strideB, strideC);
    else hipLaunchKernelGGL(k_sgemm_small<2>, grid, dim3(256), 0, st_, A, lda, B, ldb, C, ldc, M, N, K, bias, strideA, strideB, strideC);
    return hipGetLastError() == hipSuccess ? 0 : -5;
}

int spadot_stamp(unsigned long long *buf, int slot, void *stream) {
    if (!buf || slot < 0) return -22;
    hipLaunchKernelGGL(k_stamp, dim3(1), dim3(64), 0, (hipStream_t)stream, buf, slot);
    return hipGetLastError() == hipSuccess ? 0 : -5;
}

int spadot_knn(const double *x, int n, int d, int kk, int *out, void *stream) {
    if (n <= 0 || d <= 0 || d > KNN_MAXD || kk <= 0 || kk > n || kk > 128) return -22;
    const size_t lds = sizeof(double) * KNN_T * KNN_MAXD + (sizeof(double) + sizeof(int)) * (size_t)kk * KNN_T;
    static PerDeviceFlag attr_set;     
    if (!attr_set) { (void)hipFuncSetAttribute((const void *)k_knn, hipFuncAttributeMaxDynamicSharedMemorySize, 160 * 1024); attr_set = true; }
    hipLaunchKernelGGL(k_knn, dim3((n + KNN_T - 1) / KNN_T), dim3(KNN_T), lds, (hipStream_t)stream, x, n, d, kk, out);
    return hipGetLastError() == hipSuccess ? 0 : -5;
}

int spadot_lloyd_step(const double *X, double *C, const int *xoff, const int *npts, int n_max, int R, const int *rgroup,
                      const int *Kr, int K_max, int D, const double *tol, double *part, int *done, double *inertia, int skip_done,
                      void *stream) {
    if (n_max <= 0 || R <= 0 || R > 65535 || D <= 0 || D > LL_MAXD || K_max <= 0 || K_max > LL_MAXK) return -22;
    if (!X || !C || !xoff || !npts || !rgroup || !Kr || !tol || !part || !done || !inertia) return -22;
    if ((size_t)K_max * D + (size_t)LL_PTS * D > 7936) return -22;
    hipStream_t st_ = (hipStream_t)stream;
    const int nchunk = (n_max + LL_PTS - 1) / LL_PTS;
    const size_t lds = sizeof(double) * ((size_t)K_max * D + (size_t)LL_PTS * D);
    hipLaunchKernelGGL(k_lloyd_assign, dim3(nchunk, R), dim3(LL_PTS), lds, st_, X, (const double *)C, D, K_max, part, xoff, npts,
                       skip_done ? (const int *)done : (const int *)nullptr, Kr, rgroup);
    hipLaunchKernelGGL(k_lloyd_update, dim3(R), dim3(256), 0, st_, (const double *)part, nchunk, D, K_max, C, done, inertia, npts,
                       tol, skip_done, Kr, rgroup);
    return hipGetLastError() == hipSuccess ? 0 : -5;
}

int spadot_kmeanspp_seed(const double *X, const int *xoff, const int *npts, int D, int P, const int *pset, const int *pK,
                         const int *pfirst, const int *puoff, const double *U, int K_max, int n_max, double *closest, int *idx,
                         double *centers, void *stream) {
    if (P <= 0 || D <= 0 || D > LL_MAXD || K_max <= 0 || K_max > LL_MAXK || n_max <= 0) return -22;
    if (!X || !xoff || !npts || !pset || !pK || !pfirst || !puoff || !U || !closest || !idx || !centers) return -22;
    hipLaunchKernelGGL(k_kmeanspp_seed, dim3(P), dim3(KPP_T), 0, (hipStream_t)stream, X, xoff, npts, D, pset, pK, pfirst, puoff,
                       U, K_max, n_max, closest, idx, centers);
    return hipGetLastError() == hipSuccess ? 0 : -5;
}

int spadot_grad_sumsq(const float *grad, long long count, double *scratch, float *sumsq, void *stream) {
    if (count <= 0 || !scratch) return -22;
    if (((uintptr_t)grad & 15) != 0) return -22;
    hipStream_t st_ = (hipStream_t)stream;
    const long long want = (count / 4 + 255) / 256;
    const int nb = (int)(want < 1 ? 1 : (want < 2048 ? want : 2048));
    hipLaunchKernelGGL(k_sumsq_part, dim3(nb), dim3(256), 0, st_, grad, count, scratch);
    hipLaunchKernelGGL(k_final_sum<float>, dim3(1), dim3(1024), 0, st_, scratch, nb, 1.0, sumsq);
    return hipGetLastError() == hipSuccess ? 0 : -5;
}

int spadot_adamw_step_dev(float *param, const float *grad, float *exp_avg, float *exp_avg_sq, const float *sumsq,
                          long long count, double lr, double beta1, double beta2, double eps, double weight_decay,
                          double max_norm, int *step_dev, void *stream) {
    if (count <= 0 || !step_dev) return -22;
    hipStream_t st_ = (hipStream_t)stream;
    const long long want = (count + 255) / 256;
    const int nb = (int)(want < 4096 ? want : 4096);
    hipLaunchKernelGGL(k_step_inc, dim3(1), dim3(1), 0, st_, step_dev);
    hipLaunchKernelGGL(k_adamw, dim3(nb), dim3(256), 0, st_, param, grad, exp_avg, exp_avg_sq, sumsq, count,
                       (float)lr, (float)beta1, (float)beta2, (float)eps, (float)weight_decay, (float)max_norm,
                       1.f, 1.f, (const int *)step_dev, (const float *)nullptr);
    return hipGetLastError() == hipSuccess ? 0 : -5;
}

int spadot_clip_adamw_dev(float *param, const float *grad, float *exp_avg, float *exp_avg_sq, long long count, double lr,
                          double beta1, double beta2, double eps, double weight_decay, double max_norm, double *scratch,
                          float *sumsq, int *step_dev, unsigned *counter, const float *grad_scale_dev, void *stream) {
    if (count <= 0 || !step_dev || !scratch || !sumsq || !counter) return -22;
    if (((uintptr_t)grad & 15) != 0) return -22;
    hipStream_t st_ = (hipStream_t)stream;
    const long long want4 = (count / 4 + 255) / 256;
    const int nbs = (int)(want4 < 1 ? 1 : (want4 < 512 ? want4 : 512));
    constexpr int split = 2048;
    if (split > 0) {
        const int nb2 = (int)(want4 < 1 ? 1 : (want4 < split ? want4 : split));
        hipLaunchKernelGGL(k_sumsq_part_u<4>, dim3(nb2), dim3(256), 0, st_, grad, count, scratch);
        hipLaunchKernelGGL(k_final_sum_step, dim3(1), dim3(1024), 0, st_, (const double *)scratch, nb2, sumsq, step_dev);
    } else
        hipLaunchKernelGGL(k_sumsq_last<4>, dim3(nbs), dim3(256), 0, st_, grad, count, scratch, sumsq, step_dev, counter);
    const long long want = (count + 255) / 256;
    const int nb = (int)(want < 4096 ? want : 4096);
    hipLaunchKernelGGL(k_adamw, dim3(nb), dim3(256), 0, st_, param, grad, exp_avg, exp_avg_sq, (const float *)sumsq, count,
                       (float)lr, (float)beta1, (float)beta2, (float)eps, (float)weight_decay, (float)max_norm,
                       1.f, 1.f, (const int *)step_dev, grad_scale_dev);
    return hipGetLastError() == hipSuccess ? 0 : -5;
}

int spadot_clip_adamw_images_dev(float *param, const float *grad, float *exp_avg, float *exp_avg_sq, long long count, double lr,
                                 double beta1, double beta2, double eps, double weight_decay, double max_norm, double *scratch,
                                 float *sumsq, int *step_dev, const float *grad_scale_dev, const spadot_weight_images *images,
                                 void *stream) {
    if (count <= 0 || (count & 3) || !step_dev || !scratch || !sumsq || !images) return -22;
    if (((uintptr_t)grad & 15) || ((uintptr_t)param & 15) || ((uintptr_t)exp_avg & 15) || ((uintptr_t)exp_avg_sq & 15)) return -22;
    if (images->n < 0 || images->n > 8) return -22;
    for (int s_ = 0; s_ < images->n; s_++) {
        const spadot_weight_image &W = images->w[s_];
        if (!W.image || ((uintptr_t)W.image & 7) || W.rows <= 0 || W.K <= 0 || (W.K & 3) || W.Kp < W.K || (W.Kp & 3) || (W.offset & 3) ||
            W.offset < 0 || W.offset + (long long)W.rows * W.K > count || (long long)W.rows * W.K >= (1ll << 31))
            return -22;
    }
    hipStream_t st_ = (hipStream_t)stream;
    const long long want4 = (count / 4 + 255) / 256;
    const int nb2 = (int)(want4 < 1 ? 1 : (want4 < 2048 ? want4 : 2048));
    hipLaunchKernelGGL(k_sumsq_part_u<4>, dim3(nb2), dim3(256), 0, st_, grad, count, scratch);
    hipLaunchKernelGGL(k_final_sum_step, dim3(1), dim3(1024), 0, st_, (const double *)scratch, nb2, sumsq, step_dev);
    const int nb = (int)(want4 < 4096 ? want4 : 4096);
    hipLaunchKernelGGL(k_adamw_img, dim3(nb), dim3(256), 0, st_, param, grad, exp_avg, exp_avg_sq, (const float *)sumsq, count,
                       (float)lr, (float)beta1, (float)beta2, (float)eps, (float)weight_decay, (float)max_norm,
                       (const int *)step_dev, grad_scale_dev, *images, 0ll);
    return hipGetLastError() == hipSuccess ? 0 : -5;
}

int spadot_grad_norm_step_dev(const float *grad, long long count, double *scratch, float *sumsq, int *step_dev, void *stream) {
    if (count <= 0 || !scratch || !sumsq || !step_dev || ((uintptr_t)grad & 15)) return -22;
    hipStream_t st_ = (hipStream_t)stream;
    const long long want4 = (count / 4 + 255) / 256;
    const int nb2 = (int)(want4 < 1 ? 1 : (want4 < 2048 ? want4 : 2048));
    hipLaunchKernelGGL(k_sumsq_part_u<4>, dim3(nb2), dim3(256), 0, st_, grad, count, scratch);
    hipLaunchKernelGGL(k_final_sum_step, dim3(1), dim3(1024), 0, st_, (const double *)scratch, nb2, sumsq, step_dev);
    return hipGetLastError() == hipSuccess ? 0 : -5;
}

int spadot_adamw_range_dev(float *param, const float *grad, float *exp_avg, float *exp_avg_sq, long long offset, long long count,
                           double lr, double beta1, double beta2, double eps, double weight_decay, double max_norm,
                           const float *sumsq, const int *step_dev, const float *grad_scale_dev, const spadot_weight_images *images,
                           void *stream) {
    if (offset < 0 || count <= 0 || (offset & 3) || (count & 3) || !step_dev || !sumsq) return -22;
    if (((uintptr_t)grad & 15) || ((uintptr_t)param & 15) || ((uintptr_t)exp_avg & 15) || ((uintptr_t)exp_avg_sq & 15)) return -22;
    spadot_weight_images none;
    none.n = 0;
    const spadot_weight_images *tab = images ? images : &none;
    if (tab->n < 0 || tab->n > 8) return -22;
    for (int s_ = 0; s_ < tab->n; s_++) {
        const spadot_weight_image &W = tab->w[s_];
        if (!W.image || ((uintptr_t)W.image & 7) || W.rows <= 0 || W.K <= 0 || (W.K & 3) || W.Kp < W.K || (W.Kp & 3) || (W.offset & 3) ||
            W.offset < 0 || (long long)W.rows * W.K >= (1ll << 31))
            return -22;
    }
    hipStream_t st_ = (hipStream_t)stream;
    constexpr long long max_wgs = 512;
    const long long want4 = (count / 4 + 255) / 256;
    const int nb = (int)(want4 < max_wgs ? want4 : max_wgs);
    hipLaunchKernelGGL(k_adamw_img, dim3(nb), dim3(256), 0, st_, param + offset, grad + offset, exp_avg + offset, exp_avg_sq + offset,
                       sumsq, count, (float)lr, (float)beta1, (float)beta2, (float)eps, (float)weight_decay, (float)max_norm,
                       step_dev, grad_scale_dev, *tab, offset);
    return hipGetLastError() == hipSuccess ? 0 : -5;
}

int spadot_adamw_step(float *param, const float *grad, float *exp_avg, float *exp_avg_sq, const float *sumsq,
                      long long count, double lr, double beta1, double beta2, double eps, double weight_decay,
                      double max_norm, int step, void *stream) {
    if (count <= 0 || step < 1) return -22;
    hipStream_t st_ = (hipStream_t)stream;
    const long long want = (count + 255) / 256;
    const int nb = (int)(want < 4096 ? want : 4096);
    const double bc1 = 1.0 - pow(beta1, (double)step);
    const double bc2 = 1.0 - pow(beta2, (double)step);
    hipLaunchKernelGGL(k_adamw, dim3(nb), dim3(256), 0, st_, param, grad, exp_avg, exp_avg_sq, sumsq, count,
                       (float)lr, (float)beta1, (float)beta2, (float)eps, (float)weight_decay, (float)max_norm,
                       (float)bc1, (float)sqrt(bc2), (const int *)nullptr, (const float *)nullptr);
    return hipGetLastError() == hipSuccess ? 0 : -5;
}

}
```

### spadot_amd/model/decoder.py

```python
import torch
import torch.nn as nn
import torch.nn.functional as F

from ..ops import (grad_bias, linear_bias, ln_act, mlp_chain, mlp_chain_ok, recon_fb_ok, recon_sqerr, recon_sqerr_fb, recon_sqerr_ok,
                   sqerr_sum, weight_image)


def _hidden_stage(fan_in, fan_out):
    dense = nn.Linear(fan_in, fan_out)
    nn.init.xavier_uniform_(dense.weight)
    return dense, nn.LayerNorm(fan_out), nn.LeakyReLU()


class Decoder(nn.Module):
    def __init__(self, input_dim, z_dim, decoder_layers, compute_dtype=torch.float32):
        super().__init__()
        self.compute_dtype = compute_dtype
        widths = [z_dim, *decoder_layers]
        stages = []
        for fan_in, fan_out in zip(widths[:-1], widths[1:]):
            stages.extend(_hidden_stage(fan_in, fan_out))
        stages.append(nn.Linear(widths[-1], input_dim))
        self.decoder_net = nn.Sequential(*stages)

    def forward(self, latent_sample):
        h, last, _ = self._hidden(latent_sample)
        return linear_bias(h, last.weight, last.bias, self.compute_dtype)

    def recon_loss(self, latent_sample, y, inv_scale, dz_extra=None, grad_weight=None):
        bf = self.compute_dtype == torch.bfloat16
        nocast = bf
        h, last, hb = self._hidden(latent_sample, bf16_out=nocast, dx_add=dz_extra)
        if bf and grad_weight is not None:
            wim = self._output_image(last.weight)
            wimT = self._output_image_T(wim) if wim is not None else None
            if recon_fb_ok(h, last.weight, last.bias, y, hb, wim, wimT, grad_weight):
                return recon_sqerr_fb(h, last.weight, last.bias, y, inv_scale, hb, wim, wimT, grad_weight)
        if bf and recon_sqerr_ok(h, last.weight, last.bias, y):
            return recon_sqerr(h, last.weight, last.bias, y, inv_scale, hb, self._output_image(last.weight) if nocast else None)
        return sqerr_sum(y, linear_bias(h, last.weight, last.bias, self.compute_dtype), inv_scale)

    def _output_image(self, W):
        opt = getattr(self, "_image_optimizer", None)
        if opt is None or not self.training or not W.is_cuda:
            return None
        if not opt.owns(W):
            object.__setattr__(self, "_image_optimizer", None)
            return None
        im = weight_image(W, W.shape[1], torch.bfloat16, self, tag="_wout")
        if not opt.maintain_image(W, im):
            return None
        opt.sync_images()
        return im

    def _output_image_T(self, wim, refresh=None):
        G, K = wim.shape
        Gp = (G + 127) // 128 * 128
        t = getattr(self, "_wout_T", None)
        if t is None or t.shape != (K, Gp) or t.device != wim.device:
            t = torch.zeros((K, Gp), dtype=torch.bfloat16, device=wim.device)
            object.__setattr__(self, "_wout_T", t)
            object.__setattr__(self, "_wout_T_fresh", False)
        if refresh is True or (refresh is None and not getattr(self, "_wout_T_fresh", False)):
            with torch.no_grad():
                t[:, :G].copy_(wim.t())
        object.__setattr__(self, "_wout_T_fresh", bool(refresh))
        return t

    def step_begin(self):
        if self.compute_dtype != torch.bfloat16 or not self.training:
            return
        wim = self._output_image(list(self.decoder_net)[-1].weight)
        if wim is not None:
            self._output_image_T(wim, refresh=True)

    def _hidden(self, latent_sample, bf16_out=False, dx_add=None):
        stages = list(self.decoder_net)
        h, hb = latent_sample, None
        hidden = [(stages[i], stages[i + 1], stages[i + 2].negative_slope) for i in range(0, len(stages) - 1, 3)]
        if hidden and mlp_chain_ok(h, hidden):
            if bf16_out:
                h, hb = mlp_chain(h, hidden, bf16_out=True, dx_add=dx_add)
            else:
                h = mlp_chain(h, hidden, dx_add=dx_add)
        else:
            if dx_add is not None:
                h = grad_bias(h, dx_add)
            for dense, norm, slope in hidden:
                h = ln_act(linear_bias(h, dense.weight, dense.bias), norm, slope)
        return h, stages[-1], hb
```

### spadot_amd/ops.py

```python
import ctypes

import torch

from ._call import launched as _check, need_cuda as _need_cuda, ptr as _p, stream as _stream
from ._lib import model_lib

DT_F32, DT_BF16, DT_F64 = 0, 1, 2
_DT = {torch.float32: DT_F32, torch.bfloat16: DT_BF16, torch.float64: DT_F64}
KERNEL_KINDS = {"Gaussian": 0, "Cauchy": 1, "Quadratic": 2}



class BatchGraph:

    def __init__(self, n, rowptr, col, rowptr_t, col_t, eid_t, n_tgt=None):
        self.n = int(n)
        self.n_tgt = self.n if n_tgt is None else int(n_tgt)
        self.rowptr, self.col = rowptr, col
        self.rowptr_t, self.col_t, self.eid_t = rowptr_t, col_t, eid_t
        self.E = int(col.numel())
        assert rowptr.numel() == self.n_tgt + 1 and rowptr_t.numel() == self.n + 1
        self.seed_graph = None
        self.layer_graphs = None
        self.plan_t = None
# ... 293 lines not shown
        dev = x.device
        g = g.contiguous()
        dbias = torch.empty(C, dtype=torch.float32, device=dev)
        if g.dtype == x.dtype:
            gs = torch.empty_like(g)
            _check(lib.spadot_gat_tail_scale_colsum(_p(g), dt, nt, C, 1.0 / H, _p(gs), _p(dbias), _stream()), "spadot_gat_tail_scale_colsum")
        else:
            _check(lib.spadot_gat_tail_colsum_rows(_p(g), _DT[g.dtype], nt, C, _p(dbias), _stream()), "spadot_gat_tail_colsum_rows")
            gs = (g * (1.0 / H)).to(x.dtype)
        dA = torch.bmm(gs.unsqueeze(0).expand(H, nt, C), Wg)
        direct = ctx.wgrad is not None and _DIRECT_GRAD[0]
        dW = ctx.wgrad if direct else torch.empty((H * C, K), dtype=torch.float32, device=dev)
        defer = direct and _deferring() and ctx.agrad[0] is not None and ctx.agrad[1] is not None
        if not defer:
            _bmm_f32(gs.t().unsqueeze(0).expand(H, C, nt), A, out=dW.view(H, C, K))
        dz = torch.empty((graph.E, H), dtype=torch.float32, device=dev)
        ds_dst = torch.empty((nt, H), dtype=torch.float32, device=dev)
        _check(lib.spadot_gat_tail_edge_backward(_p(x), dt, Kp, _p(dA), _p(s), _p(alpha), _p(graph.rowptr), _p(graph.col), nt, H, K,
                                                 _p(dz), _p(ds_dst), _stream()), "spadot_gat_tail_edge_backward")
        dx = torch.empty_like(x) if Kp == K else torch.zeros_like(x)
        ds_src = torch.empty((n, H), dtype=torch.float32, device=dev)
        _check(lib.spadot_gat_tail_source_backward(_p(dA), dt, _p(alpha), _p(dz), _p(ds_dst), _p(wv), _p(graph.rowptr_t), _p(graph.col_t),
                                                   _p(graph.eid_t), n, nt, x.shape[0], H, K, _p(dx), Kp, _p(ds_src),
                                                   _p(x) if ctx.in_cell is not None else None, Kp,
                                                   float(ctx.in_cell["slope"]) if ctx.in_cell is not None else 1.0, _stream()),
               "spadot_gat_tail_source_backward")
        if ctx.in_cell is not None:
            ctx.in_cell["premasked"] = True
        R = int(lib.spadot_gat_tail_dwvec_rows(n))

        def weight_side(datt_src_ptr, datt_dst_ptr, with_dw):
            if with_dw:
                _bmm_f32(gs.t().unsqueeze(0).expand(H, C, nt), A, out=dW.view(H, C, K))
            part = torch.empty((R, 2 * H * K), dtype=torch.float32, device=dev)
            _check(lib.spadot_gat_tail_dwvec(_p(x), dt, Kp, _p(ds_src), _p(ds_dst), n, nt, H, K, _p(part), _stream()), "spadot_gat_tail_dwvec")
            dwv = torch.empty(2 * H * K, dtype=torch.float32, device=dev)
            _check(lib.spadot_colsum(_p(part), R, 2 * H * K, _p(dwv), _stream()), "spadot_colsum")
            _check(lib.spadot_gat_tail_wvec_backward(_p(Wd), K, _p(a_s), _p(a_d), _p(dwv), H, C, K, _p(dW), K, 1, datt_src_ptr, datt_dst_ptr,
                                                     _stream()), "spadot_gat_tail_wvec_backward")

        if defer:
            ga_s, ga_d = ctx.agrad
            DEFERRED[0].append(lambda: weight_side(_p(ga_s), _p(ga_d), True))
            return dx, dW, None, ga_s, ga_d, dbias.to(ctx.bias_dtype), None, None, None, None
        datt = torch.empty((2, H * C), dtype=torch.float32, device=dev)
        weight_side(_p(datt), ctypes.c_void_p(datt.data_ptr() + 4 * H * C), False)
        return (dx, dW, None, datt[0].view(ctx.att_shape).to(ctx.att_dtype), datt[1].view(ctx.att_shape).to(ctx.att_dtype),
                dbias.to(ctx.bias_dtype), None, None, None, None)


def gat_tail(x, W, wimg, att_src, att_dst, bias, graph, heads, channels, in_cell=None):
    return _GATTail.apply(x, W, wimg, att_src, att_dst, bias, graph, heads, channels, in_cell)



_DIRECT_GRAD = [False]

DEFERRED = [None]
POST_CHAIN = [None]
_UNIT_SEEDS = set()
_UNIT_ONES = {}


def unit_seed(device):
    key = (device.type, device.index if device.index is not None else torch.cuda.current_device())
    one = _UNIT_ONES.get(key)
    if one is None:
        one = _UNIT_ONES[key] = torch.ones((), dtype=torch.float32, device=device)
        _UNIT_SEEDS.add(one.data_ptr())
    return one


def _deferring():
    return DEFERRED[0] is not None and _DIRECT_GRAD[0]


def cast_rows(pairs):
    ok = all(s_.dtype == torch.float32 and d_.dtype == torch.bfloat16 and s_.is_contiguous() and d_.is_contiguous()
             and s_.dim() == 2 and s_.shape[1] % 4 == 0 and d_.shape[1] % 4 == 0 and s_.is_cuda
             and s_.data_ptr() % 16 == 0 and d_.data_ptr() % 8 == 0 for s_, d_ in pairs)
    if not ok:
        for s_, d_ in pairs:
            d_[:, :s_.shape[1]].copy_(s_)
        return
    lib = model_lib()
    for k0 in range(0, len(pairs), 4):
        grp = pairs[k0:k0 + 4]
        n = len(grp)
        src = (ctypes.c_void_p * n)(*(s_.data_ptr() for s_, _ in grp))
        dst = (ctypes.c_void_p * n)(*(d_.data_ptr() for _, d_ in grp))
        rows = (ctypes.c_int * n)(*(s_.shape[0] for s_, _ in grp))
        K = (ctypes.c_int * n)(*(s_.shape[1] for s_, _ in grp))
        Kp = (ctypes.c_int * n)(*(d_.shape[1] for _, d_ in grp))
        _check(lib.spadot_cast_rows_multi(src, dst, rows, K, Kp, n, _stream()), "spadot_cast_rows_multi")


GEMM_DGRAD_MIN_WGS = 240
GEMM_MAX_WGS = 256
GEMM_OWN = [True]
GEMM_BUSY_CUS = 40
GEMM_FWD_SHAPES = ((2048, 9000),)


def _own_forward(M, Kp):
    return any(t[0] == Kp and M >= t[1] for t in GEMM_FWD_SHAPES)


def gemm_tn(x, w):
    M, K = x.shape
    N = w.shape[0]
    if (GEMM_OWN[0] and x.is_cuda and x.dtype == torch.bfloat16 and w.dtype == torch.bfloat16 and x.is_contiguous()
            and w.is_contiguous() and N % 256 == 0 and K % 64 == 0 and w.shape[1] == K and M >= 2560 and N >= 1024
            and ((M + 319) // 320) * (N // 256) <= GEMM_MAX_WGS):
        out = torch.empty((M, N), dtype=torch.bfloat16, device=x.device)
        lib = model_lib()
        mt, nt_ = (M + 319) // 320, N // 256
        tail = mt - (256 - GEMM_BUSY_CUS) // nt_ if GEMM_BUSY_CUS > 0 else 0
        if 0 < tail < mt and mt * nt_ > 256 - GEMM_BUSY_CUS and K >= 4 * 64:
            need = int(lib.spadot_gemm_bf16_split_workspace(M, N, tail, 4))
            if need > 0:
                ws = torch.empty(need, dtype=torch.float32, device=x.device)
                rc = lib.spadot_gemm_tn_bf16_split(x.data_ptr(), K, w.data_ptr(), K, out.data_ptr(), N, M, N, K, tail, 4,
                                                   ws.data_ptr(), _stream())
                if rc == 0:
                    return out
                if rc != -22:
                    _check(rc, "spadot_gemm_tn_bf16_split")
        rc = lib.spadot_gemm_tn_bf16(x.data_ptr(), K, w.data_ptr(), K, out.data_ptr(), N, M, N, K, _stream())
        if rc == 0:
            return out
        if rc != -22:
            _check(rc, "spadot_gemm_tn_bf16")
    return torch.nn.functional.linear(x, w)


WGRAD_MIN_WGS = 200


_ZERO_ROWS = {}


def _zero_row(device):
    key = (device.type, device.index)
    z = _ZERO_ROWS.get(key)
    if z is None:
        z = torch.zeros(256, dtype=torch.bfloat16, device=device)
        if not torch.cuda.is_current_stream_capturing():
            _ZERO_ROWS[key] = z
    return z




def wgrad_plan(N, K, Kp):
    best = None
    for tk in (256, 192):
        kt = (K + tk - 1) // tk
        if Kp < kt * tk:
            continue
        tiles = (N // 256) * kt
        if tiles == 0 or tiles > 256:
            wgs, slices = tiles, 1
        else:
            slices = min(8, max(1, 256 // tiles))
            wgs = tiles * slices
        fill = wgs / (256.0 * ((wgs + 255) // 256)) if wgs else 0.0
        score = fill * (1.0 if tk == 256 else 0.85)
        if best is None or score > best[0]:
            best = (score, tk, slices, wgs)
    if best is None or best[3] < WGRAD_MIN_WGS:
        return None
    return best[1], best[2], best[3]


def wgrad_bf16(g, x, K, out=None):
    M, N = g.shape
    Kp = x.shape[1]
    if (g.is_cuda and g.dtype == torch.bfloat16 and x.dtype == torch.bfloat16 and g.is_contiguous()
            and x.is_contiguous() and N % 256 == 0 and Kp % 8 == 0 and M >= 1024 and N >= 1024 and K >= 1024):
        if out is None:
            out = torch.empty((N, K), dtype=torch.float32, device=g.device)
        plan = wgrad_plan(N, K, Kp) if (out.is_contiguous() and out.dtype == torch.float32 and out.shape == (N, K)) else None
        if plan is not None:
            tile_k, slices, _ = plan
            lib = model_lib()
            need = int(lib.spadot_gemm_wgrad_bf16_workspace_tiled(M, N, K, slices, tile_k))
            ws = torch.empty(max(need, 4), dtype=torch.float32, device=g.device) if need >= 0 else None
            rc = -22 if ws is None else lib.spadot_gemm_wgrad_bf16_tiled(g.data_ptr(), N, x.data_ptr(), Kp, out.data_ptr(), K, M, N, K,
                                                                        slices, tile_k, ws.data_ptr(), _zero_row(g.device).data_ptr(),
                                                                        _stream())
            if rc == 0:
                return out
            if rc != -22:
                _check(rc, "spadot_gemm_wgrad_bf16_tiled")
    if out is not None:
        return torch.mm(g.t(), x[:, :K], out_dtype=torch.float32, out=out)
    return torch.mm(g.t(), x[:, :K], out_dtype=torch.float32)


class _DenseCD(torch.autograd.Function):

    @staticmethod
    def forward(ctx, x, W, wbuf, fresh, defer=False, in_cell=None):
        N, K = W.shape
        Kp = x.shape[1]
        ctx.defer = bool(defer)
        ctx.in_cell = in_cell if (in_cell is not None and in_cell.get("armed") and in_cell.get("rows") == x.shape[0]
                                  and x.dtype == torch.bfloat16 and x.is_contiguous()) else None
        assert Kp >= K and wbuf.shape == (N, Kp) and wbuf.dtype == x.dtype
        if not fresh:
            wbuf[:, :K].copy_(W)
        ctx.save_for_backward(x, wbuf)
        ctx.K = K
        g = W.grad
        ctx.wgrad = g if (g is not None and g.dtype == torch.float32 and g.is_contiguous() and g.shape == W.shape) else None
        return gemm_tn(x, wbuf) if _own_forward(x.shape[0], Kp) else torch.nn.functional.linear(x, wbuf)

    @staticmethod
    def backward(ctx, g):
        x, wbuf = ctx.saved_tensors
        g_final = g.is_contiguous() and g.dtype == x.dtype
        g = g.contiguous()
        dx = None
        if ctx.needs_input_grad[0]:
            dx = None
            M_, Kp_ = g.shape[0], wbuf.shape[1]
            if (GEMM_OWN[0] and g.is_cuda and g.dtype == torch.bfloat16 and M_ >= 2560 and Kp_ % 256 == 0
                    and wbuf.shape[0] % 64 == 0 and wbuf.is_contiguous() and ((M_ + 319) // 320) * (Kp_ // 256) >= GEMM_DGRAD_MIN_WGS):
                dx = torch.empty((M_, Kp_), dtype=torch.bfloat16, device=g.device)
                if ctx.in_cell is not None and x.shape == (M_, Kp_):
                    rc = model_lib().spadot_gemm_nn_bf16_masked(g.data_ptr(), g.shape[1], wbuf.data_ptr(), Kp_, dx.data_ptr(), Kp_, M_,
                                                                Kp_, g.shape[1], x.data_ptr(), Kp_, float(ctx.in_cell["slope"]), _stream())
                    if rc == 0:
                        ctx.in_cell["premasked"] = True
                else:
                    rc = model_lib().spadot_gemm_nn_bf16(g.data_ptr(), g.shape[1], wbuf.data_ptr(), Kp_, dx.data_ptr(), Kp_, M_, Kp_,
                                                         g.shape[1], _stream())
                if rc == -22:
                    dx = None
                elif rc != 0:
                    _check(rc, "spadot_gemm_nn_bf16")
            if dx is None:
                dx = g @ wbuf
        dW = None
        if ctx.needs_input_grad[1]:
            if ctx.defer and ctx.wgrad is not None and _deferring() and g_final:
                DEFERRED[0].append(lambda g=g, x=x, K=ctx.K, out=ctx.wgrad: wgrad_bf16(g, x, K, out))
                dW = ctx.wgrad
            else:
                dW = wgrad_bf16(g, x, ctx.K, ctx.wgrad if (ctx.wgrad is not None and _DIRECT_GRAD[0]) else None)
        return dx, dW, None, None, None, None


class _FirstMapSeeds(torch.autograd.Function):

    @staticmethod
    def forward(ctx, x32, W, xbf):
        K = W.shape[1]
        ctx.save_for_backward(x32, xbf)
        ctx.K = K
        g = W.grad
        ctx.wgrad = g if (g is not None and g.dtype == torch.float32 and g.is_contiguous() and g.shape == W.shape) else None
        return torch.nn.functional.linear(x32[:, :K], W)

    @staticmethod
    def backward(ctx, g):
        x32, xbf = ctx.saved_tensors
        K = ctx.K
        M, N = g.shape
        lib = model_lib()
        gb = g.contiguous().to(torch.bfloat16)
        out = ctx.wgrad if (ctx.wgrad is not None and _DIRECT_GRAD[0]) else torch.empty((N, K), dtype=torch.float32, device=g.device)
        S_ = 1
        need = int(lib.spadot_gemm_wgrad_bf16_workspace(M, N, K, S_))
        rc = -22
        if need >= 0:
            ws = torch.empty(max(need, 4), dtype=torch.float32, device=g.device)
            rc = lib.spadot_gemm_wgrad_bf16(gb.data_ptr(), N, xbf.data_ptr(), xbf.shape[1], out.data_ptr(), K, M, N, K, S_,
                                            ws.data_ptr(), _zero_row(g.device).data_ptr(), _stream())
        if rc == -22:
            return None, torch.mm(g.t(), x32[:, :K]), None
        _check(rc, "spadot_gemm_wgrad_bf16")
        return None, out, None


def first_map_seeds_ok(x32, W, xbf):
    if xbf is None or not (x32.is_cuda and x32.dtype == torch.float32 and xbf.dtype == torch.bfloat16 and xbf.is_contiguous()):
        return False
    N, K = W.shape
    return (N % 256 == 0 and K % 4 == 0 and xbf.shape[0] == x32.shape[0] and xbf.shape[1] >= (K + 255) // 256 * 256
            and xbf.shape[1] % 8 == 0 and xbf.data_ptr() % 16 == 0 and x32.shape[0] >= 64 and not x32.requires_grad)


def first_map_seeds(x32, W, xbf):
    return _FirstMapSeeds.apply(x32, W, xbf)


def _small_weight_grad(g, x):
    M, N = g.shape
    K = x.shape[1]
    if M >= 256 and M % 8 == 0 and min(N, K) >= 64 and N * K <= 65536:
        return torch.bmm(g.view(8, M // 8, N).transpose(1, 2), x.view(8, M // 8, K)).sum(0)
    return g.t() @ x


def sgemm_small_ok(*ts):
    return all(t.is_cuda and t.dtype == torch.float32 and t.dim() == 2 and t.is_contiguous() for t in ts)


def sgemm_small(mode, A, B, bias=None):
    _need_cuda(A, B, bias)
    if mode == 0:
        (M, K), N = A.shape, B.shape[1]
    elif mode == 1:
        (M, K), N = A.shape, B.shape[0]
    else:
        (K, M), N = A.shape, B.shape[1]
    C = torch.empty((M, N), dtype=torch.float32, device=A.device)
    _check(model_lib().spadot_sgemm_small(mode, _p(A), A.shape[1], _p(B), B.shape[1], _p(C), N, M, N, K,
                                          _p(bias) if bias is not None else None, 1, 0, 0, 0, _stream()), "spadot_sgemm_small")
    return C


def wgrad_small(g, x, slices=8):
    _need_cuda(g, x)
    M, N = g.shape
    K = x.shape[1]
    S = slices if (M % slices == 0 and M // slices >= 32) else 1
    Ms = M // S
    part = torch.empty((S, N, K), dtype=torch.float32, device=g.device)
    _check(model_lib().spadot_sgemm_small(2, _p(g), N, _p(x), K, _p(part), K, N, K, Ms, None, S, Ms * N, Ms * K, N * K, _stream()),
           "spadot_sgemm_small")
    return part.sum(0) if S > 1 else part[0]


_SMALL_WORK = 1 << 27


class _HiddenMap(torch.autograd.Function):

    @staticmethod
    def forward(ctx, x, W):
        ctx.save_for_backward(x, W)
        return torch.nn.functional.linear(x, W)

    @staticmethod
    def backward(ctx, g):
        x, W = ctx.saved_tensors
# ... 793 lines not shown
        db = ctx.bgrad if (direct and ctx.bgrad is not None) else torch.empty(G, dtype=torch.float32, device=y.device)
        _check(model_lib().spadot_bias_sqerr_backward(_p(g1), _p(o), _p(bias), _p(y), b, G, ctx.inv_scale, _p(gc), _p(db),
                                                      _stream()), "spadot_bias_sqerr_backward")
        dh = torch.mm(gc, Wc, out_dtype=torch.float32) if ctx.needs_input_grad[0] else None
        if direct and ctx.wgrad is not None and _deferring():
            DEFERRED[0].append(lambda gc=gc, hc=hc, out=ctx.wgrad: torch.mm(gc.t(), hc, out_dtype=torch.float32, out=out))
            dW = ctx.wgrad
        elif direct and ctx.wgrad is not None:
            dW = torch.mm(gc.t(), hc, out_dtype=torch.float32, out=ctx.wgrad)
        else:
            dW = torch.mm(gc.t(), hc, out_dtype=torch.float32)
        return dh, dW, db, None, None, None, None


class _ReconFB(torch.autograd.Function):

    @staticmethod
    def forward(ctx, h, W, bias, y, inv_scale, hc, Wc, WcT, gw):
        lib = model_lib()
        b, K = h.shape
        G = W.shape[0]
        dev = h.device
        nfl = int(lib.spadot_recon_fb_workspace(b, K, G))
        GB, RB = (G + 127) // 128, (b + 63) // 64
        ws = torch.empty(nfl, dtype=torch.float32, device=dev)
        lossp = torch.empty(GB * RB, dtype=torch.float64, device=dev)
        gc = torch.empty((b, G), dtype=torch.bfloat16, device=dev)
        dh = torch.empty((b, K), dtype=torch.float32, device=dev)
        _check(lib.spadot_recon_fb(_p(hc), _p(Wc), _p(WcT), WcT.shape[1], _p(bias), _p(y), b, K, G, float(inv_scale), _p(gw), _p(gc), _p(ws),
                                   _p(lossp), _p(dh), _stream()), "spadot_recon_fb")
        out = torch.empty(1, dtype=torch.float32, device=dev)

        def value(lossp=lossp, out=out):
            _check(lib.spadot_sum_parts(_p(lossp), GB * RB, float(inv_scale), _p(out), _stream()), "spadot_sum_parts")

        if DEFERRED[0] is not None:
            DEFERRED[0].append(value)
        else:
            value()
        ctx.save_for_backward(hc, gc, dh)
        ctx.dbp = ws[GB * b * K:].view(RB, G)
        ctx.seed = gw.data_ptr()
        ok = lambda g_, p_: g_ if (g_ is not None and g_.dtype == torch.float32 and g_.is_contiguous() and g_.shape == p_.shape) else None
        ctx.wgrad, ctx.bgrad = ok(W.grad, W), ok(bias.grad, bias)
        return out[0]

    @staticmethod
    def backward(ctx, g):
        if g is None or g.data_ptr() != ctx.seed:
            raise RuntimeError("recon_sqerr_fb: backward seeded with something other than the weight its gradient was formed for "
                               "(the forward launch already holds d loss / d h for THAT seed)")
        hc, gc, dh = ctx.saved_tensors
        lib = model_lib()
        dbp = ctx.dbp
        direct = _DIRECT_GRAD[0]
        db = ctx.bgrad if (direct and ctx.bgrad is not None) else torch.empty(dbp.shape[1], dtype=torch.float32, device=dh.device)
        dW = ctx.wgrad if (direct and ctx.wgrad is not None) else torch.empty((gc.shape[1], hc.shape[1]), dtype=torch.float32, device=dh.device)

        def rest(dbp=dbp, db=db, dW=dW, gc=gc, hc=hc):
            _check(lib.spadot_colsum(_p(dbp), dbp.shape[0], dbp.shape[1], _p(db), _stream()), "spadot_colsum")
            torch.mm(gc.t(), hc, out_dtype=torch.float32, out=dW)

        if direct and ctx.wgrad is not None and ctx.bgrad is not None and _deferring():
            DEFERRED[0].append(rest)
        else:
            with torch.no_grad():
                rest()
        return dh, dW, db, None, None, None, None, None, None


def recon_fb_ok(h, W, bias, y, hc, Wc, WcT, gw):
    ok = lambda t_, like: (t_ is not None and t_.dtype == torch.bfloat16 and t_.is_contiguous() and t_.shape == like.shape)
    okT = (WcT is not None and WcT.dtype == torch.bfloat16 and WcT.is_contiguous() and WcT.dim() == 2 and WcT.shape[0] == W.shape[1]
           and WcT.shape[1] >= (W.shape[0] + 127) // 128 * 128 and WcT.shape[1] % 8 == 0 and WcT.data_ptr() % 16 == 0)
    return bool(okT and gw is not None and gw.is_cuda and gw.dtype == torch.float32 and h.is_cuda and h.dtype == torch.float32 and h.dim() == 2
                and y.dtype == torch.float32 and y.is_contiguous() and y.shape == (h.shape[0], W.shape[0]) and bias is not None
                and bias.dtype == torch.float32 and bias.is_contiguous() and bias.data_ptr() % 16 == 0 and y.data_ptr() % 16 == 0
                and ok(hc, h) and ok(Wc, W) and model_lib().spadot_recon_fb_supported(h.shape[0], h.shape[1], W.shape[0]))


def recon_sqerr_fb(h, W, bias, y, inv_scale, h_bf16, W_image, W_image_T, grad_weight):
    return _ReconFB.apply(h, W, bias, y, inv_scale, h_bf16, W_image, W_image_T, grad_weight)


def recon_sqerr_ok(h, W, bias, y):
    return bool(h.is_cuda and h.dtype == torch.float32 and y.dtype == torch.float32 and h.dim() == 2
                and y.dim() == 2 and h.shape[1] % 4 == 0 and W.shape[1] % 4 == 0 and y.shape == (h.shape[0], W.shape[0])
                and h.shape[0] <= 4096
                and bias is not None)


def recon_sqerr(h, W, bias, y, inv_scale, h_bf16=None, W_image=None):
    ok = lambda t_, like: (t_ is not None and t_.dtype == torch.bfloat16 and t_.is_contiguous() and t_.shape == like.shape)
    return _LinearSqErr.apply(h.contiguous(), W, bias, y.contiguous(), inv_scale, h_bf16 if ok(h_bf16, h) else None,
                              W_image if ok(W_image, W) else None)



def kmeans_assign(x, centers):
    _need_cuda(x, centers)
    x = x.contiguous()
    centers = centers.contiguous().to(x.dtype)
    labels = torch.empty(x.shape[0], dtype=torch.int32, device=x.device)
    _check(model_lib().spadot_kmeans_assign(_p(x), _p(centers), x.shape[0], centers.shape[0], x.shape[1],
                                            _DT[x.dtype], _p(labels), _stream()), "spadot_kmeans_assign")
    return labels


def lloyd_steps(X, C, xoff, npts, n_max, rgroup, Kr, tol, done, inertia, part, steps, skip_done=False):
    D = X.shape[1]
    R, K_max = C.shape[0], C.shape[1]
    lib = model_lib()
    for _ in range(steps):
        _check(lib.spadot_lloyd_step(_p(X), _p(C), _p(xoff), _p(npts), int(n_max), R, _p(rgroup), _p(Kr), K_max, D, _p(tol),
                                     _p(part), _p(done), _p(inertia), 1 if skip_done else 0, _stream()), "spadot_lloyd_step")


def kmeanspp_seed(X, xoff, npts, n_max, pset, pK, pfirst, puoff, U, K_max, out=None):
    _need_cuda(X)
    P, D = int(pset.shape[0]), int(X.shape[1])
    dev = X.device
    idx, centers, closest = out if out is not None else (
        torch.empty((P, K_max), dtype=torch.int32, device=dev), torch.empty((P, K_max, D), dtype=torch.float64, device=dev),
        torch.empty((P, int(n_max)), dtype=torch.float64, device=dev))
    _check(model_lib().spadot_kmeanspp_seed(_p(X), _p(xoff), _p(npts), D, P, _p(pset), _p(pK), _p(pfirst), _p(puoff), _p(U),
                                            int(K_max), int(n_max), _p(closest), _p(idx), _p(centers), _stream()),
           "spadot_kmeanspp_seed")
    return idx, centers


def knn(coords, kk):
    _need_cuda(coords)
    x = coords.contiguous().double()
    n, d = x.shape
    out = torch.empty((n, kk), dtype=torch.int32, device=x.device)
    _check(model_lib().spadot_knn(_p(x), n, d, int(kk), _p(out), _stream()), "spadot_knn")
    return out



STAMP_BUF = [None]


def stamp_if(slot):
    if STAMP_BUF[0] is not None:
        stamp(STAMP_BUF[0], slot)


def stamp(buf, slot):
    _check(model_lib().spadot_stamp(_p(buf), int(slot), _stream()), "spadot_stamp")



class FlatAdamW:

    def __init__(self, params, lr=3e-4, betas=(0.9, 0.999), eps=1e-8, weight_decay=1e-2, max_norm=0.3, last=None, first=None):
        params = [p for p in params if p.requires_grad]
        tail_ids = {id(p) for p in (last or [])}
        head_ids = {id(p) for p in (first or [])} - tail_ids
        params = ([p for p in params if id(p) in head_ids] + [p for p in params if id(p) not in tail_ids and id(p) not in head_ids]
                  + [p for p in params if id(p) in tail_ids])
        n_tail = sum(1 for p in params if id(p) in tail_ids)
        n_head = sum(1 for p in params if id(p) in head_ids)
        assert params and all(p.is_cuda and p.dtype == torch.float32 for p in params), \
            "FlatAdamW needs fp32 parameters on the MI355X"
        dev = params[0].device
        sizes = [p.numel() for p in params]
        offs, tot = [], 0
        for s in sizes:
            offs.append(tot)
            tot += (s + 3) // 4 * 4
        self.flat_param = torch.zeros(tot, dtype=torch.float32, device=dev)
        self.flat_grad = torch.zeros(tot, dtype=torch.float32, device=dev)
        self.exp_avg = torch.zeros(tot, dtype=torch.float32, device=dev)
        self.exp_avg_sq = torch.zeros(tot, dtype=torch.float32, device=dev)
        self.sumsq = torch.zeros(1, dtype=torch.float32, device=dev)
        self.scratch = torch.empty(4096, dtype=torch.float64, device=dev)
        for p, o, s in zip(params, offs, sizes):
            self.flat_param[o:o + s].copy_(p.data.reshape(-1))
            p.data = self.flat_param[o:o + s].view_as(p.data)
            p.grad = self.flat_grad[o:o + s].view_as(p.data)
        self.params, self.count = params, tot
        self.tail_offset = offs[len(params) - n_tail] if n_tail else None
        self.tail_params = params[len(params) - n_tail:] if n_tail else []
        self.head_count = (offs[n_head] if n_head < len(params) else tot) if n_head else 0
        self.lr, self.betas, self.eps, self.weight_decay, self.max_norm = lr, betas, eps, weight_decay, max_norm
        self.t = 0
        self.step_dev = torch.zeros(1, dtype=torch.int32, device=dev)
        self.grad_scale = torch.ones(1, dtype=torch.float32, device=dev)
        self._counter = torch.zeros(1, dtype=torch.int32, device=dev)
        self._images, self._image_table, self.images_version = [], None, 0
        self._image_stamps = {}

    def owns(self, param):
        lo = self.flat_param.data_ptr()
        return param.is_cuda and lo <= param.data_ptr() < lo + 4 * self.count

    def _stamp(self, param):
        return (self.flat_param._version, param._version)

    def maintain_image(self, param, image):
        if not self.owns(param):
            return False
        if any(im.data_ptr() == image.data_ptr() and p is param for p, im in self._images):
            return True
        idx = next((i for i, p in enumerate(self.params) if p is param), None)
        rows, K = (int(param.shape[0]), int(param.shape[1])) if param.dim() == 2 else (0, 0)
        ok = (idx is not None and param.dim() == 2 and image.dtype == torch.bfloat16 and image.is_contiguous()
              and image.dim() == 2 and image.shape[0] == rows and image.shape[1] >= K and K % 4 == 0 and image.shape[1] % 4 == 0
              and rows * K < 2 ** 31 and image.data_ptr() % 8 == 0 and len(self._images) < 8 and self.count % 4 == 0
              and not any(im.data_ptr() == image.data_ptr() for _, im in self._images))
        if not ok:
            return False
        self._images.append((param, image))
        self._image_table = None
        self.images_version += 1
        self.refresh_images([image])
        return True

    def maintains(self, image):
        return any(im.data_ptr() == image.data_ptr() for _, im in self._images)

    def refresh_images(self, only=None):
        pairs = [(p.detach(), im) for p, im in self._images if only is None or any(im is o for o in only)]
        if pairs:
            with torch.no_grad():
                cast_rows(pairs)
        for p, im in self._images:
            if only is None or any(im is o for o in only):
                self._image_stamps[im.data_ptr()] = self._stamp(p)

    def sync_images(self):
        stale = [im for p, im in self._images if self._image_stamps.get(im.data_ptr()) != self._stamp(p)]
        if stale:
            self.refresh_images(stale)
        return len(stale)

    def _images_struct(self):
        if self._image_table is None:
            from ._lib import WeightImages
            tab = WeightImages()
            tab.n = len(self._images)
            for k, (p, im) in enumerate(self._images):
                off = (p.data_ptr() - self.flat_param.data_ptr()) // 4
                tab.w[k].offset, tab.w[k].rows, tab.w[k].K, tab.w[k].Kp = off, p.shape[0], p.shape[1], im.shape[1]
                tab.w[k].image = im.data_ptr()
            self._image_table = tab
        return self._image_table

    def zero_grad(self):
        self.flat_grad.zero_()

    def backward(self, loss):
        _DIRECT_GRAD[0] = True
        post = POST_CHAIN[0] = []
        try:
            grads = torch.autograd.grad(loss, self.params, allow_unused=True)
        finally:
            _DIRECT_GRAD[0] = False
            POST_CHAIN[0] = None
        with torch.no_grad():
            for job in post:
                job()
        pairs = [(p.grad, g) for p, g in zip(self.params, grads) if g is not None and g.data_ptr() != p.grad.data_ptr()]
        dst = [d for d, _ in pairs]
        src = [s for _, s in pairs]
        self._zero_unreached(self.params, grads)
        torch._foreach_copy_(dst, src)

    def backward_partial(self, outputs, grad_outputs, params, extra_inputs=()):
        ins = list(params) + list(extra_inputs)
        if grad_outputs is None and torch.is_tensor(outputs) and outputs.dim() == 0 and outputs.dtype == torch.float32:
            grad_outputs = unit_seed(outputs.device)
        _DIRECT_GRAD[0] = True
        post = POST_CHAIN[0] = []
        try:
            grads = torch.autograd.grad(outputs, ins, grad_outputs=grad_outputs, allow_unused=True)
        finally:
            _DIRECT_GRAD[0] = False
            POST_CHAIN[0] = None
        with torch.no_grad():
            for job in post:
                job()
        pg = grads[:len(params)]
        pairs = [(p.grad, g) for p, g in zip(params, pg) if g is not None and g.data_ptr() != p.grad.data_ptr()]
        self._zero_unreached(params, pg)
        if pairs:
            try:
                torch._foreach_copy_([d for d, _ in pairs], [s for _, s in pairs])
            except RuntimeError as ex:
                bad = [(tuple(d.shape), d.requires_grad, d.is_leaf, d.data_ptr() - self.flat_grad.data_ptr()) for d, _ in pairs
                       if d.requires_grad or not (0 <= d.data_ptr() - self.flat_grad.data_ptr() < 4 * self.count)]
                raise RuntimeError(f"{ex}; offending gradient slots (shape, requires_grad, is_leaf, byte offset in flat_grad): {bad}") from ex
        return grads[len(params):]

    def _zero_unreached(self, params, grads):
        for p, g in zip(params, grads):
            if g is None:
                p.grad.zero_()

    def grad_norm_sq(self):
        _check(model_lib().spadot_grad_sumsq(_p(self.flat_grad), self.count, _p(self.scratch), _p(self.sumsq),
                                             _stream()), "spadot_grad_sumsq")
        return self.sumsq

    def step(self):
        self.t += 1
        if self._images:
            _check(model_lib().spadot_clip_adamw_images_dev(_p(self.flat_param), _p(self.flat_grad), _p(self.exp_avg),
                                                            _p(self.exp_avg_sq), self.count, self.lr, self.betas[0], self.betas[1],
                                                            self.eps, self.weight_decay, self.max_norm, _p(self.scratch),
                                                            _p(self.sumsq), _p(self.step_dev), _p(self.grad_scale),
                                                            ctypes.byref(self._images_struct()), _stream()),
                   "spadot_clip_adamw_images_dev")
            return
        _check(model_lib().spadot_clip_adamw_dev(_p(self.flat_param), _p(self.flat_grad), _p(self.exp_avg),
                                                 _p(self.exp_avg_sq), self.count, self.lr, self.betas[0], self.betas[1],
                                                 self.eps, self.weight_decay, self.max_norm, _p(self.scratch), _p(self.sumsq),
                                                 _p(self.step_dev), _p(self._counter), _p(self.grad_scale), _stream()),
               "spadot_clip_adamw_dev")

    def _update_range(self, lo, hi):
        tab = ctypes.byref(self._images_struct()) if self._images else None
        _check(model_lib().spadot_adamw_range_dev(_p(self.flat_param), _p(self.flat_grad), _p(self.exp_avg), _p(self.exp_avg_sq),
                                                  lo, hi - lo, self.lr, self.betas[0], self.betas[1], self.eps, self.weight_decay,
                                                  self.max_norm, _p(self.sumsq), _p(self.step_dev), _p(self.grad_scale), tab,
                                                  _stream()), "spadot_adamw_range_dev")

    def step_sharded(self, group=None):
        from . import parallel as _par
        assert self.count % 4 == 0
        self.t += 1

        def local_sumsq(lo, hi):
            if hi <= lo:
                self.sumsq.zero_()
                self.step_dev += 1
                return self.sumsq
            _check(model_lib().spadot_grad_norm_step_dev(self.flat_grad[lo:hi].data_ptr(), hi - lo, _p(self.scratch), _p(self.sumsq),
                                                         _p(self.step_dev), _stream()), "spadot_grad_norm_step_dev")
            return self.sumsq

        def update_range(lo, hi, sumsq):
            if sumsq.data_ptr() != self.sumsq.data_ptr():
                self.sumsq.copy_(sumsq)
            self._update_range(lo, hi)

        _par.sharded_update(self.flat_grad, self.flat_param, local_sumsq, update_range, group=group)
        if self._images:
            self.refresh_images()

    def step_head(self):
        assert self.head_count > 0 and self.count % 4 == 0
        self.t += 1
        _check(model_lib().spadot_grad_norm_step_dev(_p(self.flat_grad), self.count, _p(self.scratch), _p(self.sumsq),
                                                     _p(self.step_dev), _stream()), "spadot_grad_norm_step_dev")
        self._update_range(0, self.head_count)

    def step_rest(self):
        if self.head_count < self.count:
            self._update_range(self.head_count, self.count)
```

### spadot_amd/utils/_train_utils.py

```python
import contextlib
import os
import random
from collections import OrderedDict
from collections.abc import Mapping
from time import time

import numpy as np
import torch

from ..graph import build_batch_graph, knn_graph, precompute_batches
from ..model import SpaDOT
from ..ops import FlatAdamW, cluster_losses, cluster_losses_fb, mix_losses
from .OT_loss.ot_solvers import compute_transport_map, compute_transport_maps

LOSS_NAMES = ["elbo", "Recon", "SVGP_KL", "GAT_KL", "alignment", "KMeans", "OT"]


def _obtain_tp_loc_info(adata):
    tps = np.asarray(adata.obs["timepoint"])
    uniq = sorted(set(tps.tolist()))
    code = np.array([uniq.index(t) for t in tps.tolist()], dtype=int)
    tp_mat = np.zeros((code.size, len(uniq)))
    tp_mat[np.arange(code.size), code] = 1
    loc = np.asarray(adata.obsm["spatial"], dtype=np.float64)
# ... 177 lines not shown
    with torch.no_grad():
        if backend == "device":
            from ..kmeans import fit_many
            lat = []
            for tp in tps:
                loc, Y, ix = dataloader_dict["datasets"][tp]
                lat.append(model.all_latent_samples(loc, Y, dataloader_dict["graphs"][tp], tp, as_numpy=False))
            fits = fit_many(lat, model_config["n_clusters"], random_state=model_config["seed"], n_init=10) if lat else []
            for tp, km in zip(tps, fits):
                _set_kmeans_state(model, tp, km.cluster_centers_, km.labels_, dataloader_dict["datasets"][tp][2], device)
            return
        for tp in tps:
            loc, Y, ix = dataloader_dict["datasets"][tp]
            from sklearn.cluster import KMeans
            latent = model.all_latent_samples(loc, Y, dataloader_dict["graphs"][tp], tp)
            km = KMeans(n_clusters=model_config["n_clusters"], random_state=model_config["seed"], n_init=10).fit(latent)
            _set_kmeans_state(model, tp, km.cluster_centers_, km.labels_, ix, device)


def _set_gamma(model, key, gamma, device):
    model.gammas[key] = gamma
    with np.errstate(divide="ignore", invalid="ignore"):
        g = gamma / gamma.sum(axis=1, keepdims=True)
    g = np.nan_to_num(g, nan=0.0, posinf=0.0, neginf=0.0)
    if _assign_or_copy(model._gamma_dev, key, torch.as_tensor(g, dtype=torch.float32).to(device)):
        model._state_version = getattr(model, "_state_version", 0) + 1


def _update_OT_matrix(model, model_config):
    model.eval()
    device = torch.device(model_config["device"])
    timepoints = model_config["timepoints"]
    keys, pairs = [], []
    for tp_i, tp in enumerate(timepoints[:-1]):
        nxt = timepoints[tp_i + 1]
        if tp not in model.kmeans_center_dict or nxt not in model.kmeans_center_dict:
            continue
        keys.append(f"{tp}_{nxt}")
        pairs.append((np.asarray(model.kmeans_center_dict[tp]), np.asarray(model.kmeans_center_dict[nxt])))
    if not pairs:
        return
    if not hasattr(model, "_gamma_dev"):
        model._kmeans_dev, model._gamma_dev = getattr(model, "_kmeans_dev", {}), {}
    outs = []
    for key, (a, b) in zip(keys, pairs):
        cur = model._gamma_dev.get(key)
        if cur is None or tuple(cur.shape) != (a.shape[0], b.shape[0]):
            if cur is not None:
                model._state_version = getattr(model, "_state_version", 0) + 1
            cur = model._gamma_dev[key] = torch.zeros((a.shape[0], b.shape[0]), dtype=torch.float32, device=device)
        outs.append(cur)
    plans = compute_transport_maps(pairs, model_config["ot_config"], gamma_out=outs, device=device)
    if plans is not None:
        for key, gamma in zip(keys, plans):
            model.gammas[key] = gamma
        return
    for key, (a, b) in zip(keys, pairs):
        gamma = compute_transport_map(a, b, model_config["ot_config"], G=None, device=device, skip_small=True)
        _set_gamma(model, key, gamma, device)



def _cluster_terms(model, model_config, tp, tp_i, seed_ids, z, do_km, do_ot, weights=None):
    if not (do_km or do_ot):
        zero = torch.zeros((), dtype=torch.float32, device=z.device)
        return zero, zero
    st = _device_state(model, tp)
    prev = gamma = None
    if do_ot:
        prev_tp = model_config["timepoints"][tp_i - 1]
        prev = _device_state(model, prev_tp)["centers"]
        gamma = model._gamma_dev[f"{prev_tp}_{tp}"]
    if weights is not None:
        return cluster_losses_fb(z, st["labels"], seed_ids, st["centers"], prev, gamma, st["cluster_list"], do_km, do_ot,
                                 weights[4], weights[5])
    return cluster_losses(z, st["labels"], seed_ids, st["centers"], prev, gamma, st["cluster_list"], do_km, do_ot)


def _loss_weights(model, model_config, beta1):
    if isinstance(beta1, torch.Tensor) and beta1.numel() == 6:
        return beta1
    return torch.tensor([model_config["lambda1"], -float(beta1), model_config["beta2"], model_config["omiga1"],
                         model_config["omiga2"], model_config["omiga3"]], dtype=torch.float32,
                        device=next(model.parameters()).device)


def forward_backward(model, model_config, dataloader_dict, tp_i, tp, bi, epoch, beta1, optimizer=None, noise=None,
                     latent_out=None):
    batch = dataloader_dict["dataloaders"][tp][bi]
    loc, Y, _ = dataloader_dict["datasets"][tp]
    if batch.y is not None:
        x_b, y_b = batch.x, batch.y
    else:
        x_b, y_b = loc[batch.n_id], Y[batch.n_id]
    seeds = batch.n_id[:batch.batch_size]
    recon, svgp_kl, gat_kl, align, z = model.forward(x=x_b, y=y_b, edge_index=batch.graph, tp=tp,
                                                     batch_size=batch.batch_size, batch_key=(tp, bi), noise=noise,
                                                     y_seed32=batch.y_seed32 if batch.y is not None else None)
    if latent_out is not None:
        latent_out.append(z.detach())
    do_km = epoch >= 1
    do_ot = bool(epoch >= model_config["ot_epoch"] and tp_i != 0)
    km, ot = _cluster_terms(model, model_config, tp, tp_i, seeds, z, do_km, do_ot)
    elbo, losses = mix_losses(_loss_weights(model, model_config, beta1), (recon, svgp_kl, gat_kl, align, km, ot))
    if optimizer is not None and hasattr(optimizer, "backward"):
        optimizer.backward(elbo)
    else:
        elbo.backward()
    return losses


def _ranks_share_a_device(device):
    import socket
    import torch.distributed as dist
    if not (dist.is_available() and dist.is_initialized()) or dist.get_world_size() < 2:
        return False
    idx = device.index if device.index is not None else torch.cuda.current_device()
    prop = torch.cuda.get_device_properties(idx)
    me = (socket.gethostname(), getattr(prop, "pci_domain_id", 0), getattr(prop, "pci_bus_id", idx), getattr(prop, "pci_device_id", 0))
    everyone = [None] * dist.get_world_size()
    dist.all_gather_object(everyone, me)
    return len(set(everyone)) < len(everyone)


class GraphedStepper:

    STAGES = ("gat_fwd", "svgp_fwd", "tail", "svgp_bwd", "gat_bwd_a", "gat_bwd_b", "late", "svgp_pre")
    SIDE_STAGES = (1, 3, 6, 7)

    def __init__(self, model, optimizer, model_config, dataloader_dict, grad_sync=None, grad_sync_async=None):
        self.model, self.opt, self.cfg, self.dd = model, optimizer, model_config, dataloader_dict
        self.grad_sync, self.grad_sync_async = grad_sync, grad_sync_async
        self.beta1_t = _loss_weights(model, model_config, 0.0)
        self.graphs, self.seen = {}, set()
        self.opt_graph = None
        self.pool = self.pool_side = None
        self._groups = None
        import torch.distributed as dist
        multi = grad_sync is not None or (dist.is_available() and dist.is_initialized() and dist.get_world_size() > 1)
        shared = multi and _ranks_share_a_device(torch.device(model_config["device"]))
        self.staged = bool(model_config.get("staged_graphs", not shared))
        first = {id(p) for p in model.GATEncoder.first_layer_parameters()}
        self.overlap = bool(self.staged and grad_sync_async is not None and optimizer.tail_offset is not None
                            and {id(p) for p in optimizer.tail_params} == first
                            and model_config.get("overlap_grad_sync", True))
        self.capturable = True
        self._beta1 = None
        self.clone_output = True
        self.version = getattr(model, "_state_version", 0)
        self.keep_latents, self.latents = False, {}
        if model_config.get("optimizer_weight_images", True) and hasattr(optimizer, "maintain_image"):
            object.__setattr__(model.GATEncoder, "_image_optimizer", optimizer)
            object.__setattr__(model.decoder, "_image_optimizer", optimizer)
            if not getattr(model, "_image_refresh_hook", False):
                def _refresh(mod, incompatible):
                    o = getattr(mod.GATEncoder, "_image_optimizer", None)
                    if o is not None:
                        o.refresh_images()
                model.register_load_state_dict_post_hook(_refresh)
                object.__setattr__(model, "_image_refresh_hook", True)
        self._images_version = getattr(optimizer, "images_version", 0)
        self._head_event, self._head_ready, self._chain = None, False, False
        if self.staged:
            object.__setattr__(model.GATEncoder.gat2, "defer_wgrad", True)
        self._late_event = None
        self.stamps = (torch.zeros(32, dtype=torch.int64, device=next(model.parameters()).device)
                       if os.environ.get("SPADOT_STAMPS") == "1" else None)
        if self.stamps is not None:
            from .. import ops as _ops
            _ops.STAMP_BUF[0] = self.stamps
        import weakref
        reg = getattr(model, "_steppers", None)
        if reg is None:
            reg = weakref.WeakSet()
            object.__setattr__(model, "_steppers", reg)
        reg.add(self)

    def _body(self, tp_i, tp, bi, epoch, with_update=True):
        losses = forward_backward(self.model, self.cfg, self.dd, tp_i, tp, bi, epoch, self.beta1_t,
                                  optimizer=self.opt)
        if with_update:
            self.opt.step()
        return losses

    def _capture(self, fn):
        torch.cuda.synchronize()
        g = torch.cuda.CUDAGraph()
        if self.pool is None:
            self.pool = torch.cuda.graph_pool_handle()
        with torch.cuda.graph(g, pool=self.pool, capture_error_mode="thread_local"):
            out = fn()
        return g, out

    def update(self):
        if getattr(self.opt, "images_version", 0) != self._images_version:
            self._images_version = self.opt.images_version
            self.opt_graph = None if self.opt_graph in (None, False) else False
        if getattr(self.opt, "head_count", 0) <= 0:
            if self.opt_graph is None:
                self.opt.step()
                self.opt_graph = False
            elif self.opt_graph is False:
                self.opt_graph, _ = self._capture(self.opt.step)
                self.opt_graph.replay()
            else:
                self.opt_graph.replay()
            return
        if self._head_event is None:
            self._head_event = torch.cuda.Event()
        main = torch.cuda.current_stream()
        if self.opt_graph is None:
            self.opt.step_head()
            self._head_event.record(main)
            self.opt.step_rest()
            self.opt_graph = False
        else:
            if self.opt_graph is False:
                head, rest = self.opt.step_head, self.opt.step_rest
                if self.stamps is not None:
                    from ..ops import stamp

                    def head():
                        stamp(self.stamps, 24)
                        self.opt.step_head()
                        stamp(self.stamps, 25)

                    def rest():
                        stamp(self.stamps, 26)
                        self.opt.step_rest()
                        stamp(self.stamps, 27)
                ga, _ = self._capture(head)
                gb, _ = self._capture(rest)
                self.opt_graph = (ga, gb)
            self.opt_graph[0].replay()
            self._head_event.record(main)
            self.opt_graph[1].replay()
        self._head_ready = True

    @contextlib.contextmanager
    def chained(self):
        prev = self._chain
        self._chain, self._head_ready = True, False
        try:
            yield self
        finally:
            self._chain, self._head_ready = prev, False

    def barrier(self):
        self._head_ready = False

    def _run(self, tp_i, tp, bi, epoch, beta1, with_update):
        if getattr(self.model.GATEncoder, "_image_optimizer", None) is self.opt:
            self.opt.sync_images()
        if getattr(self.model, "_state_version", 0) != self.version:
            self.graphs.clear()
            self.version = getattr(self.model, "_state_version", 0)
        if self._beta1 != float(beta1):
            self.beta1_t[1].fill_(-float(beta1))
            self._beta1 = float(beta1)
        if self.staged:
            return self._run_staged(tp_i, tp, bi, epoch, with_update)
        key = (tp, bi, epoch >= 1, epoch >= self.cfg["ot_epoch"] and tp_i != 0, with_update)
        if key in self.graphs:
            g, out = self.graphs[key]
            g.replay()
            return out.clone() if self.clone_output else out
        if key not in self.seen:
            self.seen.add(key)
            return self._body(tp_i, tp, bi, epoch, with_update=with_update)
        g, out = self._capture(lambda: self._body(tp_i, tp, bi, epoch, with_update=with_update))
        self.graphs[key] = (g, out)
        g.replay()
        return out.clone() if self.clone_output else out

    def _stages(self, tp_i, tp, bi, epoch):
        model, cfg, dd, opt = self.model, self.cfg, self.dd, self.opt
        batch = dd["dataloaders"][tp][bi]
        b = batch.batch_size
        seeds = batch.n_id[:b]
        cached = batch.y is not None
        loc, Y, _ = dd["datasets"][tp]
        do_km = epoch >= 1
        do_ot = bool(epoch >= cfg["ot_epoch"] and tp_i != 0)
        P = self._param_groups()
        st = {}
        from .. import ops as _ops
        from ..model import svgp as _svgp

        def gat_fwd():
            model.decoder.step_begin()
            y_all = batch.y if cached else Y[batch.n_id]
            st["zg"] = model.branch_gat(y_all, batch.graph, b, taps=st)

        def svgp_fwd():
            st["xs"] = batch.x[:b] if cached else loc[seeds]
            st["ys"] = batch.y[:b] if cached else Y[seeds]
            _svgp.ELBO_LATE[0] = st.setdefault("svgp_late", [])
            try:
                st["pm"], st["pv"], st["skl"] = model.branch_svgp(st["xs"], st["ys"], tp, b, batch_key=(tp, bi),
                                                                  y_seed32=getattr(batch, "y_seed32", None) if cached else None)
            finally:
                _svgp.ELBO_LATE[0] = None
            st["svgp_holder"] = _svgp.holder_of(st["pm"])

        def svgp_pre():
            with torch.no_grad():
                for job in st.pop("svgp_late", []):
                    job()
            _svgp.precompute_backward(st["svgp_holder"])

        def tail():
            leaves = [st[k].detach().requires_grad_(True) for k in ("zg", "pm", "pv", "skl")]
            box = {}

            def hook(z):
                if not (do_km or do_ot):
                    return None
                res = _cluster_terms(model, cfg, tp, tp_i, seeds, z, do_km, do_ot, weights=self.beta1_t)
                if res is None:
                    return None
                box["km"], box["ot"] = res[0], res[1]
                return res[2]

            recon, gkl, align, z = model.tail(leaves[0], leaves[1], leaves[2], st["ys"], b,
                                              y_seed32=getattr(batch, "y_seed32", None) if cached else None, z_hook=hook,
                                              recon_weight=self.beta1_t[0])
            km, ot = (box["km"], box["ot"]) if "km" in box else _cluster_terms(model, cfg, tp, tp_i, seeds, z, do_km, do_ot)
            elbo, losses = mix_losses(self.beta1_t, (recon, leaves[3], gkl, align, km, ot))
            st["g"] = opt.backward_partial(elbo, None, P["tail"], extra_inputs=leaves)
            if self.keep_latents:
                self.latents[(tp, bi)] = z.detach()
            return losses

        def svgp_bwd():
            g = st["g"]
            opt.backward_partial([st["pm"], st["pv"], st["skl"]], [g[1], g[2], g[3]], P["svgp"])

        def gat_bwd_a():
            st["gd2"] = opt.backward_partial([st["zg"]], [st["g"][0]], P["gat_above_d2"], extra_inputs=[st["d2"]])[0]

        def gat_bwd_b():
            opt.backward_partial([st["d2"]], [st["gd2"]], P["gat_below_d2"])

        def late():
            with torch.no_grad():
                for job in st.pop("late", []):
                    job()

        def queued(fn):
            def run():
                _ops.DEFERRED[0] = st.setdefault("late", [])
                try:
                    return fn()
                finally:
                    _ops.DEFERRED[0] = None
            return run

        fns = (gat_fwd, svgp_fwd, queued(tail), svgp_bwd, queued(gat_bwd_a), queued(gat_bwd_b), late, svgp_pre)
        if self.stamps is not None:
            from ..ops import stamp

            def stamped(k, fn):
                def run():
                    stamp(self.stamps, 2 * k)
                    r = fn()
                    stamp(self.stamps, 2 * k + 1)
                    return r
                return run
            fns = tuple(stamped(k, fn) for k, fn in enumerate(fns))
        return fns

    def _param_groups(self):
        if self._groups is None:
            own = {id(p) for p in self.opt.params}
            gat = [p for p in self.model.GATEncoder.parameters() if id(p) in own]
            svgp = [p for p in self.model.SVGPEncoder.parameters() if id(p) in own]
            taken = {id(p) for p in gat + svgp}
            above = {id(p) for p in self.model.GATEncoder.above_second_dense()}
            self._groups = {"svgp": svgp, "tail": [p for p in self.opt.params if id(p) not in taken],
                            "gat_above_d2": [p for p in gat if id(p) in above],
                            "gat_below_d2": [p for p in gat if id(p) not in above]}
        return self._groups

    def _issue_staged(self, fns, two_streams=True):
        gat_fwd, svgp_fwd, tail, svgp_bwd, gat_bwd_a, gat_bwd_b, late, svgp_pre = fns
        main = torch.cuda.current_stream()
        if not two_streams:
            gat_fwd(); svgp_fwd(); svgp_pre()
            res = tail()
            svgp_bwd(); gat_bwd_a(); gat_bwd_b(); late()
            if self.overlap:
                self._exchange_buckets(main, main)
            return res
        side = self.model._side_stream()
        if self._chain and self._head_ready and self._head_event is not None:
            side.wait_event(self._head_event)
        else:
            side.wait_stream(main)
        self._head_ready = False
        gat_fwd()
        with torch.cuda.stream(side):
            svgp_fwd()
        main.wait_stream(side)
        res = tail()
        with torch.cuda.stream(side):
            svgp_pre()
        side.wait_stream(main)
        gat_bwd_a()
        if self._late_event is None:
            self._late_event = torch.cuda.Event()
        self._late_event.record(main)
        with torch.cuda.stream(side):
            svgp_bwd()
        gat_bwd_b()
        with torch.cuda.stream(side):
            side.wait_event(self._late_event)
            late()
        if self.overlap:
            self._exchange_buckets(main, side)
        main.wait_stream(side)
        return res

    def _exchange_buckets(self, main, side):
        cut = self.opt.tail_offset
        with torch.cuda.stream(side):
            w1 = self.grad_sync_async(self.opt.flat_grad[:cut])
        w2 = self.grad_sync_async(self.opt.flat_grad[cut:])
        w1.wait()
        w2.wait()

    def exchange_idle(self):
        main = torch.cuda.current_stream()
        self._exchange_buckets(main, main)

    def _run_staged(self, tp_i, tp, bi, epoch, with_update):
        key = (tp, bi, epoch >= 1, epoch >= self.cfg["ot_epoch"] and tp_i != 0, "staged")
        if key in self.graphs:
            graphs, out = self.graphs[key]
            self._issue_staged([g.replay for g in graphs])
            res = out.clone() if self.clone_output else out
        elif key not in self.seen:
            self.seen.add(key)
            res = self._issue_staged(list(self._stages(tp_i, tp, bi, epoch)), two_streams=False)
        else:
            fns = self._stages(tp_i, tp, bi, epoch)
            if self.pool is None:
                self.pool, self.pool_side = torch.cuda.graph_pool_handle(), torch.cuda.graph_pool_handle()
            torch.cuda.synchronize()
            out = None
            graphs = [None] * len(fns)
            for k in (0, 1, 7, 2, 3, 4, 5, 6):
                g = torch.cuda.CUDAGraph()
                pool = self.pool_side if k in self.SIDE_STAGES else self.pool
                with torch.cuda.graph(g, pool=pool, capture_error_mode="thread_local"):
                    r = fns[k]()
                if k == 2:
                    out = r
                graphs[k] = g
            self.graphs[key] = (graphs, out)
            self._issue_staged([g.replay for g in graphs])
            res = out.clone() if self.clone_output else out
        if with_update:
            self.update()
        return res

    def fb(self, tp_i, tp, bi, epoch, beta1):
        return self._run(tp_i, tp, bi, epoch, beta1, False)

    def step(self, tp_i, tp, bi, epoch, beta1):
        if self.grad_sync is None:
            return self._run(tp_i, tp, bi, epoch, beta1, True)
        res = self.fb(tp_i, tp, bi, epoch, beta1)
        if not self.overlap:
            self.grad_sync(self.opt.flat_grad)
        self.update()
        return res


def training_step(model, optimizer, model_config, dataloader_dict, tp_i, tp, bi, epoch, beta1, grad_sync=None):
    losses = forward_backward(model, model_config, dataloader_dict, tp_i, tp, bi, epoch, beta1,
                              optimizer=optimizer)
    if grad_sync is not None:
        grad_sync(optimizer.flat_grad)
    optimizer.step()
    return losses


def train_SpaDOT(dataloader_dict, model_config, verbose=True, epoch_seconds=None):
    import pandas as pd
    device = torch.device(model_config["device"])
    model = SpaDOT.SpaDOT(model_config, dataloader_dict).to(device)
    optimizer = FlatAdamW(model.parameters(), lr=model_config["lr"], first=model.SVGPEncoder.parameters())
    stepper = GraphedStepper(model, optimizer, model_config, dataloader_dict) if model_config.get("use_hip_graphs", True) else None
    if stepper is not None:
        stepper.clone_output = False
    beta1s = _beta_cycle_linear(model_config["maxiter"], stop=model_config["beta1"])
    tp_indexed_list = list(enumerate(model_config["timepoints"]))
    loss_dict = OrderedDict((e, OrderedDict((n, 0.0) for n in LOSS_NAMES)) for e in range(model_config["maxiter"]))
    if verbose:
        print("Training SpaDOT model...")
        print("K-means backend: %s" % model_config.get("kmeans_backend", "device"))
    t_start = time()
    for epoch in range(model_config["maxiter"]):
        beta1 = float(beta1s[epoch])
        model.train()
        ep_start = time()
        random.shuffle(tp_indexed_list)
        acc = {}
        with (stepper.chained() if stepper is not None else contextlib.nullcontext()):
            for tp_i, tp in tp_indexed_list:
                if tp not in dataloader_dict["dataloaders"]:
                    continue
                nb = len(dataloader_dict["dataloaders"][tp])
                tot = torch.zeros(len(LOSS_NAMES), dtype=torch.float32, device=device)
                for bi in range(nb):
                    if stepper is not None:
                        tot += stepper.step(tp_i, tp, bi, epoch, beta1).float()
                    else:
                        tot += training_step(model, optimizer, model_config, dataloader_dict, tp_i, tp, bi, epoch, beta1).float()
                acc[tp] = tot / nb
        for tp, v in acc.items():
            for name, val in zip(LOSS_NAMES, v.cpu().tolist()):
                loss_dict[epoch][name] += val
        if verbose and epoch % 10 == 0:
            print(f"Epoch {epoch + 1}: Training time: {int(time() - ep_start)} seconds, "
                  + ", ".join(f"{n}: {loss_dict[epoch][n]:.8f}" for n in LOSS_NAMES))
        _update_Kmeans(model, model_config, dataloader_dict)
        if (epoch + 1) % model_config["ot_config"]["ot_epochs"] == 0:
            _update_OT_matrix(model, model_config)
        if epoch_seconds is not None:
            torch.cuda.synchronize(device)
            epoch_seconds.append(time() - ep_start)
    if verbose:
        print("Training finished...")
        print("Training time: %d seconds." % int(time() - t_start))
    return model, pd.DataFrame.from_dict(loss_dict)
```

Before: 668.7 training steps/s.

## Fuse grad-norm partials into wgrad reduce and hand optimizer head to side stream

The split-K wgrad reduce kernel now writes per-block squared-norm partials into slots. The optimizer then sums those slots plus a ranged sum-of-squares over the remaining gradient ranges, so the gradient buffer is not read twice for clipping. The AdamW kernel also keeps a transposed bf16 weight image up to date. The optimizer head step is moved to the side stream without joining main first, so the update can overlap the tail of the backward pass. This adds per-key skip bookkeeping and more captured graph variants, and risks ordering bugs between streams.

```diff
diff --git a/include/spadot_model.h b/include/spadot_model.h
--- a/include/spadot_model.h
+++ b/include/spadot_model.h
@@ -203,6 +203,9 @@
 long long spadot_gemm_wgrad_bf16_workspace_tiled(int M, int N, int K, int slices, int tile_k);
 int spadot_gemm_wgrad_bf16_tiled(const void *G, int ldg, const void *X, int ldx, float *dW, int ldw, int M, int N, int K,
                                  int slices, int tile_k, float *workspace, const void *zero_row, void *stream);
+long long spadot_gemm_wgrad_bf16_slots(int M, int N, int K, int slices, int tile_k);
+int spadot_gemm_wgrad_bf16_tiled_sq(const void *G, int ldg, const void *X, int ldx, float *dW, int ldw, int M, int N, int K,
+                                    int slices, int tile_k, float *workspace, const void *zero_row, double *slots, void *stream);
 
 int spadot_mlp_chain_supported(int n_layers, const int *dims);
 int spadot_mlp_chain_workspace(int b, int n_layers, const int *dims, int *n_rows, int *width);
@@ -240,8 +243,9 @@
                           float *sumsq, int *step_dev, unsigned *counter, const float *grad_scale_dev, void *stream);
 typedef struct spadot_weight_image {
     long long offset;
-    int rows, K, Kp, reserved;
+    int rows, K, Kp, ldt;
     void *image;
+    void *image_t;
 } spadot_weight_image;
 typedef struct spadot_weight_images {
     int n, reserved;
@@ -257,6 +261,13 @@
                            const float *sumsq, const int *step_dev, const float *grad_scale_dev, const spadot_weight_images *images,
                            void *stream);
 
+int spadot_grad_norm_ranged_dev(const float *grad, long long count, int nskip, const long long *skip_off, const long long *skip_len,
+                                double *slots, int nslots, int *step_dev, void *stream);
+int spadot_adamw_range_slots_dev(float *param, const float *grad, float *exp_avg, float *exp_avg_sq, long long offset, long long count,
+                                 double lr, double beta1, double beta2, double eps, double weight_decay, double max_norm,
+                                 const double *slots, int nslots, float *sumsq_out, const int *step_dev, const float *grad_scale_dev,
+                                 const spadot_weight_images *images, void *stream);
+
 int spadot_adamw_step(float *param, const float *grad, float *exp_avg, float *exp_avg_sq,
                       const float *sumsq, long long count, double lr, double beta1, double beta2,
                       double eps, double weight_decay, double max_norm, int step, void *stream);
diff --git a/spadot_amd/_lib.py b/spadot_amd/_lib.py
--- a/spadot_amd/_lib.py
+++ b/spadot_amd/_lib.py
@@ -77,7 +77,7 @@
 
 class WeightImage(ctypes.Structure):
     _fields_ = [("offset", ctypes.c_longlong), ("rows", ctypes.c_int), ("K", ctypes.c_int), ("Kp", ctypes.c_int),
-                ("reserved", ctypes.c_int), ("image", ctypes.c_void_p)]
+                ("ldt", ctypes.c_int), ("image", ctypes.c_void_p), ("image_t", ctypes.c_void_p)]
 
 
 class WeightImages(ctypes.Structure):
@@ -185,6 +185,7 @@
         "spadot_gemm_tn_bf16_split": [vp, ci, vp, ci, vp, ci, ci, ci, ci, ci, ci, vp, vp],
         "spadot_gemm_wgrad_bf16": [vp, ci, vp, ci, vp, ci, ci, ci, ci, ci, vp, vp, vp],
         "spadot_gemm_wgrad_bf16_tiled": [vp, ci, vp, ci, vp, ci, ci, ci, ci, ci, ci, vp, vp, vp],
+        "spadot_gemm_wgrad_bf16_tiled_sq": [vp, ci, vp, ci, vp, ci, ci, ci, ci, ci, ci, vp, vp, vp, vp],
         "spadot_mlp_chain_supported": [ci, vp],
         "spadot_headfc_backward": [vp, vp, vp, ci, ci, ci, vp, vp, vp, vp],
         "spadot_bias_sqerr_forward": [vp, vp, vp, ci, ci, cd, vp, vp, vp],
@@ -234,6 +235,9 @@
         "spadot_clip_adamw_dev": [vp, vp, vp, vp, ll, cd, cd, cd, cd, cd, cd, vp, vp, vp, vp, vp, vp],
         "spadot_clip_adamw_images_dev": [vp, vp, vp, vp, ll, cd, cd, cd, cd, cd, cd, vp, vp, vp, vp, ctypes.POINTER(WeightImages), vp],
         "spadot_grad_norm_step_dev": [vp, ll, vp, vp, vp, vp],
+        "spadot_grad_norm_ranged_dev": [vp, ll, ci, ctypes.POINTER(ll), ctypes.POINTER(ll), vp, ci, vp, vp],
+        "spadot_adamw_range_slots_dev": [vp, vp, vp, vp, ll, ll, cd, cd, cd, cd, cd, cd, vp, ci, vp, vp, vp,
+                                         ctypes.POINTER(WeightImages), vp],
         "spadot_adamw_range_dev": [vp, vp, vp, vp, ll, ll, cd, cd, cd, cd, cd, cd, vp, vp, vp, ctypes.POINTER(WeightImages), vp],
         "spadot_adamw_step": [vp, vp, vp, vp, vp, ll, cd, cd, cd, cd, cd, cd, ci, vp],
         "spadot_adamw_step_dev": [vp, vp, vp, vp, vp, ll, cd, cd, cd, cd, cd, cd, vp, vp],
@@ -288,6 +292,8 @@
     lib.spadot_gemm_wgrad_bf16_workspace.restype = ll
     lib.spadot_gemm_wgrad_bf16_workspace_tiled.argtypes = [ci, ci, ci, ci, ci]
     lib.spadot_gemm_wgrad_bf16_workspace_tiled.restype = ll
+    lib.spadot_gemm_wgrad_bf16_slots.argtypes = [ci, ci, ci, ci, ci]
+    lib.spadot_gemm_wgrad_bf16_slots.restype = ll
     lib.spadot_mk_lds_capacity.argtypes = []
     lib.spadot_mk_lds_capacity.restype = ci
     lib.spadot_mk_ranksum_scratch_bytes.argtypes = [ci, ci, ci]
diff --git a/spadot_amd/csrc/gemm_wgrad_bf16.hip b/spadot_amd/csrc/gemm_wgrad_bf16.hip
--- a/spadot_amd/csrc/gemm_wgrad_bf16.hip
+++ b/spadot_amd/csrc/gemm_wgrad_bf16.hip
@@ -199,7 +199,7 @@
 
 template <int TKE>
 __global__ __launch_bounds__(256) void k_wgrad_reduce(const float *__restrict__ part, int S, int tiles, int ktiles,
-                                                      float *__restrict__ dW, int ldw, int N, int K) {
+                                                      float *__restrict__ dW, int ldw, int N, int K, double *__restrict__ slots) {
     constexpr int RP = TKE / 4;
     constexpr int BPT = RP / 4;
     constexpr int Q = 64 * RP;
@@ -208,6 +208,7 @@
     const int p0 = (blockIdx.x - tile * BPT) * 256 + threadIdx.x;
     const int tn = tile / ktiles, tk = tile - tn * ktiles;
     f32x4 v[8][4];
+    double sq = 0.0;
 #pragma unroll
     for (int s_ = 0; s_ < 8; s_++)
         if (s_ < S) {
@@ -223,11 +224,24 @@
             if (s_ < S) sum += v[s_][j];
         const int idx4 = p0 + j * Q, ln = idx4 / RP, c4 = idx4 - ln * RP;
         const int n = tn * TN + ln, k = tk * TKE + 4 * c4;
-        if (n < N && k + 3 < K) *reinterpret_cast<f32x4 *>(dW + (size_t)n * ldw + k) = sum;
-        else if (n < N) {
+        if (n < N && k + 3 < K) {
+            *reinterpret_cast<f32x4 *>(dW + (size_t)n * ldw + k) = sum;
+            sq += ((double)sum[0] * sum[0] + (double)sum[1] * sum[1]) + ((double)sum[2] * sum[2] + (double)sum[3] * sum[3]);
+        } else if (n < N) {
             for (int e = 0; e < 4; e++)
-                if (k + e < K) dW[(size_t)n * ldw + k + e] = sum[e];
-        }
+                if (k + e < K) {
+                    dW[(size_t)n * ldw + k + e] = sum[e];
+                    sq += (double)sum[e] * sum[e];
+                }
+        }
+    }
+    if (slots) {
+        __shared__ double sh[4];
+#pragma unroll
+        for (int off = 32; off > 0; off >>= 1) sq += __shfl_xor(sq, off, 64);
+        if ((threadIdx.x & 63) == 0) sh[threadIdx.x >> 6] = sq;
+        __syncthreads();
+        if (threadIdx.x == 0) slots[blockIdx.x] = ((sh[0] + sh[1]) + sh[2]) + sh[3];
     }
 }
 
@@ -257,7 +271,7 @@
 
 template <int WGN, int WGK, int TI, int TJ>
 static int launch_wgrad(const void *G, int ldg, const void *X, int ldx, float *dW, int ldw, int M, int N, int K, int ktiles, int ntiles,
-                        int S, int cps, float *workspace, const void *zero_row, hipStream_t stream) {
+                        int S, int cps, float *workspace, const void *zero_row, double *slots, hipStream_t stream) {
     constexpr int TKE = 32 * WGK * TJ;
     static PerDeviceFlag attr_set;     
     auto kern = k_gemm_wgrad_bf16<WGN, WGK, TI, TJ>;
@@ -270,12 +284,19 @@
                        ldw, M, N, K, ktiles, S, cps, (const __bf16 *)zero_row, workspace);
     if (S > 1)
         hipLaunchKernelGGL(k_wgrad_reduce<TKE>, dim3((unsigned)tiles * (unsigned)(TKE / 16)), dim3(256), 0, stream, (const float *)workspace, S,
-                           tiles, ktiles, dW, ldw, N, K);
+                           tiles, ktiles, dW, ldw, N, K, slots);
     return hipGetLastError() == hipSuccess ? 0 : -5;
 }
 
-extern "C" int spadot_gemm_wgrad_bf16_tiled(const void *G, int ldg, const void *X, int ldx, float *dW, int ldw, int M, int N, int K,
-                                            int slices, int tile_k, float *workspace, const void *zero_row, void *stream) {
+extern "C" long long spadot_gemm_wgrad_bf16_slots(int M, int N, int K, int slices, int tile_k) {
+    if (M <= 0 || N <= 0 || K <= 0 || N % TN != 0 || (tile_k != 256 && tile_k != 192)) return -22;
+    const int S = effective_slices(M, slices, nullptr);
+    const long long tiles = (long long)(N / TN) * ((K + tile_k - 1) / tile_k);
+    return S > 1 ? tiles * (tile_k / 16) : 0;
+}
+
+static int wgrad_tiled(const void *G, int ldg, const void *X, int ldx, float *dW, int ldw, int M, int N, int K, int slices, int tile_k,
+                       float *workspace, const void *zero_row, double *slots, void *stream) {
     if (M <= 0 || N <= 0 || K <= 0 || N % TN != 0 || ldg < N || ldx < K || ldw < K || ldg % 8 || ldx % 8) return -22;
     if (tile_k != 256 && tile_k != 192) return -22;
     if (((uintptr_t)G & 15) || ((uintptr_t)X & 15) || ((uintptr_t)dW & 15) || (ldw % 4)) return -22;
@@ -287,9 +308,24 @@
     const int S = effective_slices(M, slices, &cps);
     if (ntiles * ktiles > 4096) return -22;
     if (S > 1 && (!workspace || ((uintptr_t)workspace & 15))) return -22;
+    if (slots && (S <= 1 || ((uintptr_t)slots & 7))) return -22;
     if (tile_k == 256)
-        return launch_wgrad<2, 4, 4, 2>(G, ldg, X, ldx, dW, ldw, M, N, K, ktiles, ntiles, S, cps, workspace, zero_row, (hipStream_t)stream);
-    return launch_wgrad<4, 2, 2, 3>(G, ldg, X, ldx, dW, ldw, M, N, K, ktiles, ntiles, S, cps, workspace, zero_row, (hipStream_t)stream);
+        return launch_wgrad<2, 4, 4, 2>(G, ldg, X, ldx, dW, ldw, M, N, K, ktiles, ntiles, S, cps, workspace, zero_row, slots,
+                                        (hipStream_t)stream);
+    return launch_wgrad<4, 2, 2, 3>(G, ldg, X, ldx, dW, ldw, M, N, K, ktiles, ntiles, S, cps, workspace, zero_row, slots,
+                                    (hipStream_t)stream);
+}
+
+extern "C" int spadot_gemm_wgrad_bf16_tiled(const void *G, int ldg, const void *X, int ldx, float *dW, int ldw, int M, int N, int K,
+                                            int slices, int tile_k, float *workspace, const void *zero_row, void *stream) {
+    return wgrad_tiled(G, ldg, X, ldx, dW, ldw, M, N, K, slices, tile_k, workspace, zero_row, nullptr, stream);
+}
+
+extern "C" int spadot_gemm_wgrad_bf16_tiled_sq(const void *G, int ldg, const void *X, int ldx, float *dW, int ldw, int M, int N, int K,
+                                               int slices, int tile_k, float *workspace, const void *zero_row, double *slots,
+                                               void *stream) {
+    if (!slots) return -22;
+    return wgrad_tiled(G, ldg, X, ldx, dW, ldw, M, N, K, slices, tile_k, workspace, zero_row, slots, stream);
 }
 
 extern "C" int spadot_gemm_wgrad_bf16(const void *G, int ldg, const void *X, int ldx, float *dW, int ldw, int M, int N, int K,
diff --git a/spadot_amd/csrc/model_kernels.hip b/spadot_amd/csrc/model_kernels.hip
--- a/spadot_amd/csrc/model_kernels.hip
+++ b/spadot_amd/csrc/model_kernels.hip
@@ -1350,6 +1350,44 @@
     acc = block_sum_d(acc, sh);
     if (threadIdx.x == 0) part[blockIdx.x] = acc;
 }
+struct sumsq_kept {
+    int n;
+    long long start4[5];
+    long long cum4[5];
+    long long total4;
+};
+template <int U>
+__global__ __launch_bounds__(256) void k_sumsq_ranged(const float *__restrict__ g, sumsq_kept kept, double *__restrict__ part,
+                                                      int *__restrict__ step_dev) {
+    __shared__ double sh[16];
+    double acc = 0.0;
+    const long long n4 = kept.total4;
+    const float4 *g4 = reinterpret_cast<const float4 *>(g);
+    const long long stride = (long long)gridDim.x * 256;
+    for (long long k = (long long)blockIdx.x * 256 + threadIdx.x; k < n4; k += U * stride) {
+        float4 v[U];
+#pragma unroll
+        for (int u = 0; u < U; u++) {
+            const long long q = k + u * stride;
+            v[u] = make_float4(0.f, 0.f, 0.f, 0.f);
+            if (q < n4) {
+                long long at = kept.start4[0] + q;
+#pragma unroll
+                for (int c = 1; c < 5; c++)
+                    if (c < kept.n && q >= kept.cum4[c]) at = kept.start4[c] + (q - kept.cum4[c]);
+                v[u] = g4[at];
+            }
+        }
+#pragma unroll
+        for (int u = 0; u < U; u++)
+            acc += ((double)v[u].x * v[u].x + (double)v[u].y * v[u].y) + ((double)v[u].z * v[u].z + (double)v[u].w * v[u].w);
+    }
+    acc = block_sum_d(acc, sh);
+    if (threadIdx.x == 0) {
+        part[blockIdx.x] = acc;
+        if (blockIdx.x == 0) step_dev[0] += 1;
+    }
+}
 __global__ __launch_bounds__(1024) void k_final_sum_step(const double *__restrict__ part, int nparts, float *__restrict__ out,
                                                          int *__restrict__ step_dev) {
     __shared__ double sh[16];
@@ -1402,12 +1440,29 @@
                                                    const float *__restrict__ sumsq, long long count, float lr,
                                                    float b1, float b2, float eps, float wd, float max_norm,
                                                    const int *__restrict__ step_dev, const float *__restrict__ grad_scale,
-                                                   spadot_weight_images imgs, long long base) {
+                                                   spadot_weight_images imgs, long long base,
+                                                   const double *__restrict__ slots, int nslots, float *__restrict__ sumsq_out) {
+    float ss;
+    if (slots) {
+        __shared__ double sh[16];
+        double acc = 0.0;
+        for (int k0 = threadIdx.x; k0 < nslots; k0 += 16 * 256) {
+            double q[16];
+#pragma unroll
+            for (int u = 0; u < 16; u++) q[u] = k0 + u * 256 < nslots ? slots[k0 + u * 256] : 0.0;
+#pragma unroll
+            for (int u = 0; u < 16; u++) acc += q[u];
+        }
+        acc = block_sum_d(acc, sh);
+        ss = (float)acc;
+        if (blockIdx.x == 0 && threadIdx.x == 0 && sumsq_out) sumsq_out[0] = ss;
+    } else
+        ss = sumsq[0];
     const double t = (double)step_dev[0];
     const float bc1 = (float)(1.0 - pow((double)b1, t));
     const float bc2_sqrt = (float)sqrt(1.0 - pow((double)b2, t));
     const float gs = grad_scale ? grad_scale[0] : 1.f;
-    const float coef = adamw_clip_coef(sumsq[0], gs, max_norm);
+    const float coef = adamw_clip_coef(ss, gs, max_norm);
     const long long n4 = count >> 2;
     for (long long q = (long long)blockIdx.x * 256 + threadIdx.x; q < n4; q += (long long)gridDim.x * 256) {
         const long long k = q << 2;
@@ -1440,6 +1495,11 @@
                 const unsigned hi = (unsigned)__builtin_bit_cast(unsigned short, (__bf16)po[2]) |
                                     ((unsigned)__builtin_bit_cast(unsigned short, (__bf16)po[3]) << 16);
                 *reinterpret_cast<uint2 *>(dst) = make_uint2(lo, hi);
+                if (W.image_t) {
+                    __bf16 *dt = reinterpret_cast<__bf16 *>(W.image_t) + (size_t)col * (unsigned)W.ldt + row;
+#pragma unroll
+                    for (int e = 0; e < 4; e++) dt[(size_t)e * (unsigned)W.ldt] = (__bf16)po[e];
+                }
                 break;
             }
         }
@@ -2675,6 +2735,7 @@
         if (!W.image || ((uintptr_t)W.image & 7) || W.rows <= 0 || W.K <= 0 || (W.K & 3) || W.Kp < W.K || (W.Kp & 3) || (W.offset & 3) ||
             W.offset < 0 || W.offset + (long long)W.rows * W.K > count || (long long)W.rows * W.K >= (1ll << 31))
             return -22;
+        if (W.image_t && (W.ldt < W.rows || (long long)W.K * W.ldt >= (1ll << 31))) return -22;
     }
     hipStream_t st_ = (hipStream_t)stream;
     const long long want4 = (count / 4 + 255) / 256;
@@ -2684,7 +2745,7 @@
     const int nb = (int)(want4 < 4096 ? want4 : 4096);
     hipLaunchKernelGGL(k_adamw_img, dim3(nb), dim3(256), 0, st_, param, grad, exp_avg, exp_avg_sq, (const float *)sumsq, count,
                        (float)lr, (float)beta1, (float)beta2, (float)eps, (float)weight_decay, (float)max_norm,
-                       (const int *)step_dev, grad_scale_dev, *images, 0ll);
+                       (const int *)step_dev, grad_scale_dev, *images, 0ll, (const double *)nullptr, 0, (float *)nullptr);
     return hipGetLastError() == hipSuccess ? 0 : -5;
 }
 
@@ -2698,11 +2759,38 @@
     return hipGetLastError() == hipSuccess ? 0 : -5;
 }
 
-int spadot_adamw_range_dev(float *param, const float *grad, float *exp_avg, float *exp_avg_sq, long long offset, long long count,
-                           double lr, double beta1, double beta2, double eps, double weight_decay, double max_norm,
-                           const float *sumsq, const int *step_dev, const float *grad_scale_dev, const spadot_weight_images *images,
-                           void *stream) {
-    if (offset < 0 || count <= 0 || (offset & 3) || (count & 3) || !step_dev || !sumsq) return -22;
+int spadot_grad_norm_ranged_dev(const float *grad, long long count, int nskip, const long long *skip_off, const long long *skip_len,
+                                double *slots, int nslots, int *step_dev, void *stream) {
+    if (count <= 0 || (count & 3) || nskip < 0 || nskip > 4 || !slots || nslots < 1 || nslots > 2048 || !step_dev) return -22;
+    if (((uintptr_t)grad & 15) || ((uintptr_t)slots & 7) || (nskip > 0 && (!skip_off || !skip_len))) return -22;
+    sumsq_kept kept;
+    kept.n = 0;
+    for (int c = 0; c < 5; c++) kept.start4[c] = kept.cum4[c] = 0;
+    long long at = 0, cum = 0;
+    for (int i = 0; i <= nskip; i++) {
+        const long long end = i < nskip ? skip_off[i] : count;
+        if (i < nskip && (skip_off[i] < at || skip_len[i] <= 0 || (skip_off[i] & 3) || (skip_len[i] & 3) || skip_off[i] + skip_len[i] > count))
+            return -22;
+        if (end > at) {
+            kept.start4[kept.n] = at >> 2;
+            kept.cum4[kept.n] = cum;
+            kept.n++;
+            cum += (end - at) >> 2;
+        }
+        if (i < nskip) at = skip_off[i] + skip_len[i];
+    }
+    kept.total4 = cum;
+    if (kept.n == 0) kept.n = 1;
+    hipLaunchKernelGGL(k_sumsq_ranged<4>, dim3(nslots), dim3(256), 0, (hipStream_t)stream, grad, kept, slots, step_dev);
+    return hipGetLastError() == hipSuccess ? 0 : -5;
+}
+
+static int adamw_range(float *param, const float *grad, float *exp_avg, float *exp_avg_sq, long long offset, long long count,
+                       double lr, double beta1, double beta2, double eps, double weight_decay, double max_norm,
+                       const float *sumsq, const double *slots, int nslots, float *sumsq_out, const int *step_dev,
+                       const float *grad_scale_dev, const spadot_weight_images *images, void *stream) {
+    if (offset < 0 || count <= 0 || (offset & 3) || (count & 3) || !step_dev || (!sumsq && !slots)) return -22;
+    if (slots && (nslots < 1 || ((uintptr_t)slots & 7))) return -22;
     if (((uintptr_t)grad & 15) || ((uintptr_t)param & 15) || ((uintptr_t)exp_avg & 15) || ((uintptr_t)exp_avg_sq & 15)) return -22;
     spadot_weight_images none;
     none.n = 0;
@@ -2713,6 +2801,7 @@
         if (!W.image || ((uintptr_t)W.image & 7) || W.rows <= 0 || W.K <= 0 || (W.K & 3) || W.Kp < W.K || (W.Kp & 3) || (W.offset & 3) ||
             W.offset < 0 || (long long)W.rows * W.K >= (1ll << 31))
             return -22;
+        if (W.image_t && (W.ldt < W.rows || (long long)W.K * W.ldt >= (1ll << 31))) return -22;
     }
     hipStream_t st_ = (hipStream_t)stream;
     constexpr long long max_wgs = 512;
@@ -2720,8 +2809,26 @@
     const int nb = (int)(want4 < max_wgs ? want4 : max_wgs);
     hipLaunchKernelGGL(k_adamw_img, dim3(nb), dim3(256), 0, st_, param + offset, grad + offset, exp_avg + offset, exp_avg_sq + offset,
                        sumsq, count, (float)lr, (float)beta1, (float)beta2, (float)eps, (float)weight_decay, (float)max_norm,
-                       step_dev, grad_scale_dev, *tab, offset);
-    return hipGetLastError() == hipSuccess ? 0 : -5;
+                       step_dev, grad_scale_dev, *tab, offset, slots, nslots, sumsq_out);
+    return hipGetLastError() == hipSuccess ? 0 : -5;
+}
+
+int spadot_adamw_range_dev(float *param, const float *grad, float *exp_avg, float *exp_avg_sq, long long offset, long long count,
+                           double lr, double beta1, double beta2, double eps, double weight_decay, double max_norm,
+                           const float *sumsq, const int *step_dev, const float *grad_scale_dev, const spadot_weight_images *images,
+                           void *stream) {
+    if (!sumsq) return -22;
+    return adamw_range(param, grad, exp_avg, exp_avg_sq, offset, count, lr, beta1, beta2, eps, weight_decay, max_norm, sumsq, nullptr, 0,
+                       nullptr, step_dev, grad_scale_dev, images, stream);
+}
+
+int spadot_adamw_range_slots_dev(float *param, const float *grad, float *exp_avg, float *exp_avg_sq, long long offset, long long count,
+                                 double lr, double beta1, double beta2, double eps, double weight_decay, double max_norm,
+                                 const double *slots, int nslots, float *sumsq_out, const int *step_dev, const float *grad_scale_dev,
+                                 const spadot_weight_images *images, void *stream) {
+    if (!slots) return -22;
+    return adamw_range(param, grad, exp_avg, exp_avg_sq, offset, count, lr, beta1, beta2, eps, weight_decay, max_norm, nullptr, slots,
+                       nslots, sumsq_out, step_dev, grad_scale_dev, images, stream);
 }
 
 int spadot_adamw_step(float *param, const float *grad, float *exp_avg, float *exp_avg_sq, const float *sumsq,
diff --git a/spadot_amd/model/decoder.py b/spadot_amd/model/decoder.py
--- a/spadot_amd/model/decoder.py
+++ b/spadot_amd/model/decoder.py
@@ -48,12 +48,12 @@
             object.__setattr__(self, "_image_optimizer", None)
             return None
         im = weight_image(W, W.shape[1], torch.bfloat16, self, tag="_wout")
-        if not opt.maintain_image(W, im):
+        if not opt.maintain_image(W, im, image_t=self._wout_T_buffer(im) if getattr(self, "_maintain_T", True) else None):
             return None
         opt.sync_images()
         return im
 
-    def _output_image_T(self, wim, refresh=None):
+    def _wout_T_buffer(self, wim):
         G, K = wim.shape
         Gp = (G + 127) // 128 * 128
         t = getattr(self, "_wout_T", None)
@@ -61,6 +61,14 @@
             t = torch.zeros((K, Gp), dtype=torch.bfloat16, device=wim.device)
             object.__setattr__(self, "_wout_T", t)
             object.__setattr__(self, "_wout_T_fresh", False)
+        return t
+
+    def _output_image_T(self, wim, refresh=None):
+        G, K = wim.shape
+        t = self._wout_T_buffer(wim)
+        opt = getattr(self, "_image_optimizer", None)
+        if opt is not None and opt.maintains(wim) and opt.maintains_t(t):
+            return t
         if refresh is True or (refresh is None and not getattr(self, "_wout_T_fresh", False)):
             with torch.no_grad():
                 t[:, :G].copy_(wim.t())
diff --git a/spadot_amd/ops.py b/spadot_amd/ops.py
--- a/spadot_amd/ops.py
+++ b/spadot_amd/ops.py
@@ -469,6 +469,9 @@
 
 
 
+SLOT_SINK = [None]
+
+
 def wgrad_plan(N, K, Kp):
     best = None
     for tk in (256, 192):
@@ -503,14 +506,27 @@
             lib = model_lib()
             need = int(lib.spadot_gemm_wgrad_bf16_workspace_tiled(M, N, K, slices, tile_k))
             ws = torch.empty(max(need, 4), dtype=torch.float32, device=g.device) if need >= 0 else None
-            rc = -22 if ws is None else lib.spadot_gemm_wgrad_bf16_tiled(g.data_ptr(), N, x.data_ptr(), Kp, out.data_ptr(), K, M, N, K,
-                                                                        slices, tile_k, ws.data_ptr(), _zero_row(g.device).data_ptr(),
-                                                                        _stream())
+            sink, slots = SLOT_SINK[0], None
+            if sink is not None and ws is not None:
+                ns = int(lib.spadot_gemm_wgrad_bf16_slots(M, N, K, slices, tile_k))
+                slots = sink.request(out, ns) if ns > 0 else None
+            if ws is None:
+                rc = -22
+            elif slots is not None:
+                rc = lib.spadot_gemm_wgrad_bf16_tiled_sq(g.data_ptr(), N, x.data_ptr(), Kp, out.data_ptr(), K, M, N, K, slices, tile_k,
+                                                         ws.data_ptr(), _zero_row(g.device).data_ptr(), slots.data_ptr(), _stream())
+            else:
+                rc = lib.spadot_gemm_wgrad_bf16_tiled(g.data_ptr(), N, x.data_ptr(), Kp, out.data_ptr(), K, M, N, K, slices, tile_k,
+                                                      ws.data_ptr(), _zero_row(g.device).data_ptr(), _stream())
             if rc == 0:
+                if sink is not None:
+                    sink.wrote(out, slots is not None)
                 return out
             if rc != -22:
                 _check(rc, "spadot_gemm_wgrad_bf16_tiled")
     if out is not None:
+        if SLOT_SINK[0] is not None:
+            SLOT_SINK[0].wrote(out, False)
         return torch.mm(g.t(), x[:, :K], out_dtype=torch.float32, out=out)
     return torch.mm(g.t(), x[:, :K], out_dtype=torch.float32)
 
@@ -1610,6 +1626,35 @@
 
 
 
+class _SlotSink:
+
+    def __init__(self, opt):
+        self.opt, self.last = opt, {}
+
+    def request(self, out, nslots):
+        rng = self.opt._grad_range(out)
+        got = self.opt._slot_range(rng, int(nslots)) if rng is not None else None
+        return None if got is None else self.opt._slots[got[0]:got[0] + got[1]]
+
+    def wrote(self, out, emitted):
+        rng = self.opt._grad_range(out)
+        if rng is None:
+            return
+        for key in list(self.last):
+            if key != rng and key[0] < rng[0] + rng[1] and rng[0] < key[0] + key[1]:
+                self.last[key] = False
+        self.last[rng] = bool(emitted)
+
+    def skipped(self):
+        out = []
+        for off, cnt, _, _ in self.opt._slot_ranges:
+            if not self.last.get((off, cnt), False):
+                break
+            out.append((off, cnt))
+        return tuple(out)
+
+
+
 class FlatAdamW:
 
     def __init__(self, params, lr=3e-4, betas=(0.9, 0.999), eps=1e-8, weight_decay=1e-2, max_norm=0.3, last=None, first=None):
@@ -1649,6 +1694,8 @@
         self._counter = torch.zeros(1, dtype=torch.int32, device=dev)
         self._images, self._image_table, self.images_version = [], None, 0
         self._image_stamps = {}
+        self._images_t = {}
+        self._slots, self._slot_ranges = None, []
 
     def owns(self, param):
         lo = self.flat_param.data_ptr()
@@ -1657,7 +1704,7 @@
     def _stamp(self, param):
         return (self.flat_param._version, param._version)
 
-    def maintain_image(self, param, image):
+    def maintain_image(self, param, image, image_t=None):
         if not self.owns(param):
             return False
         if any(im.data_ptr() == image.data_ptr() and p is param for p, im in self._images):
@@ -1670,6 +1717,9 @@
               and not any(im.data_ptr() == image.data_ptr() for _, im in self._images))
         if not ok:
             return False
+        if (image_t is not None and image_t.dtype == torch.bfloat16 and image_t.is_contiguous() and image_t.dim() == 2
+                and image_t.is_cuda and image_t.shape[0] == K and image_t.shape[1] >= rows and K * image_t.shape[1] < 2 ** 31):
+            self._images_t[image.data_ptr()] = image_t
         self._images.append((param, image))
         self._image_table = None
         self.images_version += 1
@@ -1679,11 +1729,21 @@
     def maintains(self, image):
         return any(im.data_ptr() == image.data_ptr() for _, im in self._images)
 
+    def maintains_t(self, image_t):
+        return any(t.data_ptr() == image_t.data_ptr() and self.maintains_ptr(a) for a, t in self._images_t.items())
+
+    def maintains_ptr(self, addr):
+        return any(im.data_ptr() == addr for _, im in self._images)
+
     def refresh_images(self, only=None):
         pairs = [(p.detach(), im) for p, im in self._images if only is None or any(im is o for o in only)]
         if pairs:
             with torch.no_grad():
                 cast_rows(pairs)
+                for p, im in pairs:
+                    t = self._images_t.get(im.data_ptr())
+                    if t is not None:
+                        t[:, :im.shape[0]].copy_(im[:, :p.shape[1]].t())
         for p, im in self._images:
             if only is None or any(im is o for o in only):
                 self._image_stamps[im.data_ptr()] = self._stamp(p)
@@ -1703,8 +1763,44 @@
                 off = (p.data_ptr() - self.flat_param.data_ptr()) // 4
                 tab.w[k].offset, tab.w[k].rows, tab.w[k].K, tab.w[k].Kp = off, p.shape[0], p.shape[1], im.shape[1]
                 tab.w[k].image = im.data_ptr()
+                t = self._images_t.get(im.data_ptr())
+                tab.w[k].image_t, tab.w[k].ldt = (t.data_ptr(), t.shape[1]) if t is not None else (None, 0)
             self._image_table = tab
         return self._image_table
+
+    NORM_SLOTS, MAX_SLOT_RANGES, MAX_RANGE_SLOTS = 1024, 4, 4096
+
+    def slot_sink(self):
+        return _SlotSink(self)
+
+    def _grad_range(self, t):
+        if not (torch.is_tensor(t) and t.is_cuda and t.is_contiguous() and t.dtype == torch.float32):
+            return None
+        d = t.data_ptr() - self.flat_grad.data_ptr()
+        if d < 0 or d % 16 or d // 4 + t.numel() > self.count or t.numel() % 4 or t.numel() == 0:
+            return None
+        return d // 4, t.numel()
+
+    def _slot_range(self, rng, nslots):
+        for off, cnt, first, ns in self._slot_ranges:
+            if (off, cnt) == rng:
+                return (first, ns) if ns == nslots else None
+            if off < rng[0] + rng[1] and rng[0] < off + cnt:
+                return None
+        if len(self._slot_ranges) >= self.MAX_SLOT_RANGES or not (0 < nslots <= self.MAX_RANGE_SLOTS) or self.count % 4:
+            return None
+        if self._slots is None:
+            self._slots = torch.zeros(self.NORM_SLOTS + self.MAX_SLOT_RANGES * self.MAX_RANGE_SLOTS, dtype=torch.float64,
+                                      device=self.flat_grad.device)
+        first = self.NORM_SLOTS + sum(r[3] for r in self._slot_ranges)
+        self._slot_ranges.append((rng[0], rng[1], first, nslots))
+        return first, nslots
+
+    def _skip_args(self, skip):
+        n = len(skip)
+        assert n <= len(self._slot_ranges) and tuple(skip) == tuple((r[0], r[1]) for r in self._slot_ranges[:n]), \
+            "skip must be slot_sink().skipped() of this optimizer"
+        return sorted(skip), self.NORM_SLOTS + sum(r[3] for r in self._slot_ranges[:n])
 
     def zero_grad(self):
         self.flat_grad.zero_()
@@ -1742,6 +1838,10 @@
                 job()
         pg = grads[:len(params)]
         pairs = [(p.grad, g) for p, g in zip(params, pg) if g is not None and g.data_ptr() != p.grad.data_ptr()]
+        if SLOT_SINK[0] is not None:
+            for p, g in zip(params, pg):
+                if g is None or g.data_ptr() != p.grad.data_ptr():
+                    SLOT_SINK[0].wrote(p.grad, False)
         self._zero_unreached(params, pg)
         if pairs:
             try:
@@ -1778,8 +1878,15 @@
                                                  _p(self.step_dev), _p(self._counter), _p(self.grad_scale), _stream()),
                "spadot_clip_adamw_dev")
 
-    def _update_range(self, lo, hi):
+    def _update_range(self, lo, hi, nslots=0):
         tab = ctypes.byref(self._images_struct()) if self._images else None
+        if nslots:
+            _check(model_lib().spadot_adamw_range_slots_dev(_p(self.flat_param), _p(self.flat_grad), _p(self.exp_avg),
+                                                            _p(self.exp_avg_sq), lo, hi - lo, self.lr, self.betas[0], self.betas[1],
+                                                            self.eps, self.weight_decay, self.max_norm, _p(self._slots), nslots,
+                                                            _p(self.sumsq), _p(self.step_dev), _p(self.grad_scale), tab, _stream()),
+                   "spadot_adamw_range_slots_dev")
+            return
         _check(model_lib().spadot_adamw_range_dev(_p(self.flat_param), _p(self.flat_grad), _p(self.exp_avg), _p(self.exp_avg_sq),
                                                   lo, hi - lo, self.lr, self.betas[0], self.betas[1], self.eps, self.weight_decay,
                                                   self.max_norm, _p(self.sumsq), _p(self.step_dev), _p(self.grad_scale), tab,
@@ -1808,13 +1915,24 @@
         if self._images:
             self.refresh_images()
 
-    def step_head(self):
+    def step_head(self, skip=None):
         assert self.head_count > 0 and self.count % 4 == 0
         self.t += 1
-        _check(model_lib().spadot_grad_norm_step_dev(_p(self.flat_grad), self.count, _p(self.scratch), _p(self.sumsq),
-                                                     _p(self.step_dev), _stream()), "spadot_grad_norm_step_dev")
-        self._update_range(0, self.head_count)
-
-    def step_rest(self):
+        if skip is None:
+            _check(model_lib().spadot_grad_norm_step_dev(_p(self.flat_grad), self.count, _p(self.scratch), _p(self.sumsq),
+                                                         _p(self.step_dev), _stream()), "spadot_grad_norm_step_dev")
+            self._update_range(0, self.head_count)
+            return
+        if self._slots is None:
+            self._slots = torch.zeros(self.NORM_SLOTS + self.MAX_SLOT_RANGES * self.MAX_RANGE_SLOTS, dtype=torch.float64,
+                                      device=self.flat_grad.device)
+        ranges, nslots = self._skip_args(skip)
+        ll4 = ctypes.c_longlong * 4
+        offs, lens = ll4(*([r[0] for r in ranges] + [0] * (4 - len(ranges)))), ll4(*([r[1] for r in ranges] + [0] * (4 - len(ranges))))
+        _check(model_lib().spadot_grad_norm_ranged_dev(_p(self.flat_grad), self.count, len(ranges), offs, lens, _p(self._slots),
+                                                       self.NORM_SLOTS, _p(self.step_dev), _stream()), "spadot_grad_norm_ranged_dev")
+        self._update_range(0, self.head_count, nslots)
+
+    def step_rest(self, skip=None):
         if self.head_count < self.count:
-            self._update_range(self.head_count, self.count)
+            self._update_range(self.head_count, self.count, 0 if skip is None else self._skip_args(skip)[1])
diff --git a/spadot_amd/utils/_train_utils.py b/spadot_amd/utils/_train_utils.py
--- a/spadot_amd/utils/_train_utils.py
+++ b/spadot_amd/utils/_train_utils.py
@@ -353,6 +353,7 @@
         if model_config.get("optimizer_weight_images", True) and hasattr(optimizer, "maintain_image"):
             object.__setattr__(model.GATEncoder, "_image_optimizer", optimizer)
             object.__setattr__(model.decoder, "_image_optimizer", optimizer)
+            object.__setattr__(model.decoder, "_maintain_T", bool(model_config.get("optimizer_transposed_image", True)))
             if not getattr(model, "_image_refresh_hook", False):
                 def _refresh(mod, incompatible):
                     o = getattr(mod.GATEncoder, "_image_optimizer", None)
@@ -365,6 +366,11 @@
         if self.staged:
             object.__setattr__(model.GATEncoder.gat2, "defer_wgrad", True)
         self._late_event = None
+        single = (self.staged and not multi and grad_sync_async is None and getattr(optimizer, "head_count", 0) > 0
+                  and hasattr(optimizer, "slot_sink") and optimizer.count % 4 == 0)
+        self.norm_slots = single and bool(model_config.get("clip_norm_slots", True))
+        self.handover = single and bool(model_config.get("update_handover", True))
+        self._skips, self._slot_graphs = {}, {}
         self.stamps = (torch.zeros(32, dtype=torch.int64, device=next(model.parameters()).device)
                        if os.environ.get("SPADOT_STAMPS") == "1" else None)
         if self.stamps is not None:
@@ -384,19 +390,22 @@
             self.opt.step()
         return losses
 
-    def _capture(self, fn):
+    def _capture(self, fn, side=False):
         torch.cuda.synchronize()
         g = torch.cuda.CUDAGraph()
         if self.pool is None:
             self.pool = torch.cuda.graph_pool_handle()
-        with torch.cuda.graph(g, pool=self.pool, capture_error_mode="thread_local"):
+        if side and self.pool_side is None:
+            self.pool_side = torch.cuda.graph_pool_handle()
+        with torch.cuda.graph(g, pool=self.pool_side if side else self.pool, capture_error_mode="thread_local"):
             out = fn()
         return g, out
 
-    def update(self):
+    def update(self, skip=None, side=None):
         if getattr(self.opt, "images_version", 0) != self._images_version:
             self._images_version = self.opt.images_version
             self.opt_graph = None if self.opt_graph in (None, False) else False
+            self._slot_graphs = {k: (None if v in (None, False) else False) for k, v in self._slot_graphs.items()}
         if getattr(self.opt, "head_count", 0) <= 0:
             if self.opt_graph is None:
                 self.opt.step()
@@ -410,32 +419,49 @@
         if self._head_event is None:
             self._head_event = torch.cuda.Event()
         main = torch.cuda.current_stream()
-        if self.opt_graph is None:
-            self.opt.step_head()
-            self._head_event.record(main)
-            self.opt.step_rest()
-            self.opt_graph = False
+        plain = skip is None and side is None
+        state = self.opt_graph if plain else self._slot_graphs.get((skip, side is not None))
+        step_head = self.opt.step_head if skip is None else (lambda: self.opt.step_head(skip))
+        step_rest = self.opt.step_rest if skip is None else (lambda: self.opt.step_rest(skip))
+        first = main if side is None else side
+        if side is not None:
+            side.wait_stream(main)
+        if state is None:
+            with torch.cuda.stream(first):
+                step_head()
+                self._head_event.record(first)
+            main.wait_event(self._head_event)
+            step_rest()
+            state = False
         else:
-            if self.opt_graph is False:
-                head, rest = self.opt.step_head, self.opt.step_rest
+            if state is False:
+                head, rest = step_head, step_rest
                 if self.stamps is not None:
                     from ..ops import stamp
 
                     def head():
                         stamp(self.stamps, 24)
-                        self.opt.step_head()
+                        step_head()
                         stamp(self.stamps, 25)
 
                     def rest():
                         stamp(self.stamps, 26)
-                        self.opt.step_rest()
+                        step_rest()
                         stamp(self.stamps, 27)
-                ga, _ = self._capture(head)
+                ga, _ = self._capture(head, side=side is not None)
                 gb, _ = self._capture(rest)
-                self.opt_graph = (ga, gb)
-            self.opt_graph[0].replay()
-            self._head_event.record(main)
-            self.opt_graph[1].replay()
+                state = (ga, gb)
+                if side is not None:
+                    side.wait_stream(main)
+            with torch.cuda.stream(first):
+                state[0].replay()
+                self._head_event.record(first)
+            main.wait_event(self._head_event)
+            state[1].replay()
+        if plain:
+            self.opt_graph = state
+        else:
+            self._slot_graphs[(skip, side is not None)] = state
         self._head_ready = True
 
     @contextlib.contextmanager
@@ -455,6 +481,7 @@
             self.opt.sync_images()
         if getattr(self.model, "_state_version", 0) != self.version:
             self.graphs.clear()
+            self._skips.clear()
             self.version = getattr(self.model, "_state_version", 0)
         if self._beta1 != float(beta1):
             self.beta1_t[1].fill_(-float(beta1))
@@ -583,7 +610,7 @@
                             "gat_below_d2": [p for p in gat if id(p) not in above]}
         return self._groups
 
-    def _issue_staged(self, fns, two_streams=True):
+    def _issue_staged(self, fns, two_streams=True, join=True):
         gat_fwd, svgp_fwd, tail, svgp_bwd, gat_bwd_a, gat_bwd_b, late, svgp_pre = fns
         main = torch.cuda.current_stream()
         if not two_streams:
@@ -619,7 +646,8 @@
             late()
         if self.overlap:
             self._exchange_buckets(main, side)
-        main.wait_stream(side)
+        if join:
+            main.wait_stream(side)
         return res
 
     def _exchange_buckets(self, main, side):
@@ -636,9 +664,10 @@
 
     def _run_staged(self, tp_i, tp, bi, epoch, with_update):
         key = (tp, bi, epoch >= 1, epoch >= self.cfg["ot_epoch"] and tp_i != 0, "staged")
+        side = self.model._side_stream() if (with_update and self.handover and key in self.seen) else None
         if key in self.graphs:
             graphs, out = self.graphs[key]
-            self._issue_staged([g.replay for g in graphs])
+            self._issue_staged([g.replay for g in graphs], join=side is None)
             res = out.clone() if self.clone_output else out
         elif key not in self.seen:
             self.seen.add(key)
@@ -650,19 +679,26 @@
             torch.cuda.synchronize()
             out = None
             graphs = [None] * len(fns)
-            for k in (0, 1, 7, 2, 3, 4, 5, 6):
-                g = torch.cuda.CUDAGraph()
-                pool = self.pool_side if k in self.SIDE_STAGES else self.pool
-                with torch.cuda.graph(g, pool=pool, capture_error_mode="thread_local"):
-                    r = fns[k]()
-                if k == 2:
-                    out = r
-                graphs[k] = g
+            from .. import ops as _ops
+            sink = _ops.SLOT_SINK[0] = self.opt.slot_sink() if self.norm_slots else None
+            try:
+                for k in (0, 1, 7, 2, 3, 4, 5, 6):
+                    g = torch.cuda.CUDAGraph()
+                    pool = self.pool_side if k in self.SIDE_STAGES else self.pool
+                    with torch.cuda.graph(g, pool=pool, capture_error_mode="thread_local"):
+                        r = fns[k]()
+                    if k == 2:
+                        out = r
+                    graphs[k] = g
+            finally:
+                _ops.SLOT_SINK[0] = None
             self.graphs[key] = (graphs, out)
-            self._issue_staged([g.replay for g in graphs])
+            if sink is not None:
+                self._skips[key] = sink.skipped()
+            self._issue_staged([g.replay for g in graphs], join=side is None)
             res = out.clone() if self.clone_output else out
         if with_update:
-            self.update()
+            self.update(skip=self._skips.get(key) if key in self.graphs else None, side=side)
         return res
 
     def fb(self, tp_i, tp, bi, epoch, beta1):
```

Measured after the change: 672.8 training steps/s (median of 6 runs). About the same (+0.6%).
